# nikisalli/nightmare_rl

Measured on AMD Instinct MI355X. Metric: env-steps/sec at N parallel Nightmare-v3 envs, 1/2/4/8 MI355X, higher is better.
Workload: dtype f32; 1 GPU; 4096 Nightmare-v3 envs per GPU, random-action rollout U(-1,1)^18, full step(): 2 x 8 ms substeps (18-DoF dynamics + floor contact, PGS x3 + noslip x4) + obs/reward/termination/reset; envs_per_gpu=4096, decimation=2

## Files before the change

nightmare_rl_amd/csrc/nm_core.h:

```cpp
#pragma once
#include <type_traits>
#include <stddef.h>

#include "simt.h"

#ifdef NM_MEASURE
#define NM_ABLATE(mask) (mask)
#else
#define NM_ABLATE(mask) 0
#endif
namespace nm {
using namespace simt;

constexpr int kNQ = 25, kNV = 24, kNU = 18, kNLEG = 6, kNCOL = 7, kNSENS = 13, kNOBS = 66, kNREW = 16;
constexpr int kLinkN = 25;
constexpr int kLegN = 3 * kLinkN;
constexpr int kBaseN = 10;
constexpr int kColN = 24;
constexpr int kMaxCon = 16;
constexpr int kMaxRow = 4 * kMaxCon;
constexpr int kMaxConBig = 44;
constexpr int kBigSlots = (4 * kMaxConBig + NM_WAVE - 1) / NM_WAVE;
constexpr int kJRow = 16;
enum { R_ACTION_RATE, R_ANG_VEL_XY, R_BASE_HEIGHT, R_BODY_CONTACT, R_DEFAULT_POS, R_DOF_ACC, R_DOF_VEL, R_FEET_AIR_TIME, R_FEET_CONTACT,
       R_LIN_VEL_Z, R_ORIENTATION, R_STAND_STILL, R_TORQUES, R_TRACK_ANG, R_TRACK_LIN, R_TERMINATION };

template <class real> struct Model {
  const real* hullv;
  const real* hullnv;
  real legc[kNLEG * kLegN];
  real basec[kBaseN];
  real colc[kNCOL * kColN];
  real footc[kNLEG * 4];
  real qpos0[kNQ];
  int maxnbr;
  int link_rot_id[3];
  real total_mass;
  real h, kv, ctrl_max, grav, mu;
  real solref_K, solref_B, si_d0, si_dmax, si_width, si_mid, si_power;
  real pgs_scale, pgs_tol, noslip_tol, tol_planemesh;
  int pgs_iters, noslip_iters, mpr_iters;
  real mpr_tol;
  real dt, p_gain, clip_obs, obs_lin, obs_ang, obs_dofpos, obs_dofvel, max_lin_x, max_ang, term_force, sigma, max_ep_len, default_pos[3];
  float action_scale, clip_actions;
  int resample_every;
  real rew_scale[kNREW];
  real ep_len_s;
  int rew_extra;
  int tibia_mode, body_mode;
  int collide_batch_min;
  real tibia_max, body_max, base_h_target, max_contact_force;
};

template <class real> struct Args {
  int N;
  uint64_t seed;
  int64_t env_offset;
  real *qpos, *qvel, *qwarm;
  real *dofpos, *dofvel, *act, *cmd, *epsum;
  real* feetair;
  int* feetflags;
  int64_t* eplen;
  uint32_t* rngctr;
  int* hullcache;
  const float* actions;
  const real* cmd_u;
  float *obs, *rew, *timeout_now;
  float* ret_acc;
  int64_t* done;
  real* stat_sum;
  int* stat_cnt;
  int* wave_done;
  int *nto, *to_list;
  int *nprev, *to_prev;
  unsigned long long* to_owner;
  float *ep_stats, *time_outs;
  long long* counters;
  real* dbg;
  int nsub;
  int nxcd;
  int physics_only;
  int ablate;
  const real* noise_vec;
  const real* noise_u;
  uint64_t noise_step;
  real* rec;
  int rec_env;
};
constexpr int kTicketGroup = 64, kTicketStride = 32, kTicketTop = 0;
constexpr uint64_t kNoiseKey = 0x4E4F495345ull;
constexpr int kDbgN = 256;

template <class real> struct Sh {
  real qpos[28], qvel[24], warm[24], ctrl[20];
  real Rb[9], wv[6];
  real anc[kNU * 3], axs[kNU * 3];
  real colR[kNCOL * 9], colp[kNCOL * 3];
  real Minv[kNLEG * 6], W[kNLEG * 18], Lb[15], Dbi[6];
  real MinvH[kNLEG * 6], WH[kNLEG * 18], LbH[15], DbiH[6];
  real qas[24], qfs[24], qfc[24];
  real vv[24];
  real sens[16], cvb[6];
  real bh[2];
  real mbb[36], sc[36];
  real legtmp[kNLEG * 66];
  NM_FN real* cpos() { return legtmp; }
  NM_FN real* cnrm() { return legtmp + 3 * kMaxConBig; }
  NM_FN real* cdist() { return legtmp + 6 * kMaxConBig; }
  NM_FN int* cleg() { return reinterpret_cast<int*>(legtmp + 7 * kMaxConBig); }
  NM_FN int* cleg1() { return reinterpret_cast<int*>(legtmp + 8 * kMaxConBig); }
  real efc_f[kMaxRow];
#ifdef NM_DEBUG_SOLVER
  real dbg_b[kMaxRow], dbg_a[kMaxRow], dbg_f0[kMaxRow];
#endif
  int ncon, nwarn, it_pgs, it_noslip, anypair;
  int nhop;
  int ntog;
  real eact[kNU], epact[kNU], epdv[kNU];
  real ecmd[4], eepsum[kNREW];
  int eplen_lo, eplen_hi;
  unsigned ectr;
  int cstart[8], ccnt[8];
  real sink[NM_WAVE];
  int hcache[8];
};

static_assert(kNLEG * 66 >= 9 * kMaxConBig, "contact list must fit the leg staging area");
template <class real, int G> struct ShW {
  Sh<real> e[G];
  alignas(16) real jrow[kMaxRow * kJRow];
};
#define NM_OFS(field) ((int)(offsetof(Sh<real>, field) / sizeof(real)))
#define NM_IOFS(field) ((int)(offsetof(Sh<real>, field) / sizeof(int)))

template <class A, class B, class C> NM_FN void cross3(A* r, const B* a, const C* b) {
  A x = a[1] * b[2] - a[2] * b[1], y = a[2] * b[0] - a[0] * b[2], z = a[0] * b[1] - a[1] * b[0];
  r[0] = x; r[1] = y; r[2] = z;
}
template <class A, class B, class C> NM_FN A dot3(const B* a, const C* b) { return a[0] * b[0] + a[1] * b[1] + a[2] * b[2]; }
template <class A, class B, class C> NM_FN void matvec3(A* r, const B* m, const C* v) {
  A x = m[0] * v[0] + m[1] * v[1] + m[2] * v[2], y = m[3] * v[0] + m[4] * v[1] + m[5] * v[2], z = m[6] * v[0] + m[7] * v[1] + m[8] * v[2];
  r[0] = x; r[1] = y; r[2] = z;
}
template <class A, class B, class C> NM_FN void matvec3_fma(A* r, const B* m, const C* v) {
  A x = vfma(A(m[2]), A(v[2]), vfma(A(m[1]), A(v[1]), A(m[0]) * A(v[0])));
  A y = vfma(A(m[5]), A(v[2]), vfma(A(m[4]), A(v[1]), A(m[3]) * A(v[0])));
  A z = vfma(A(m[8]), A(v[2]), vfma(A(m[7]), A(v[1]), A(m[6]) * A(v[0])));
  r[0] = x; r[1] = y; r[2] = z;
}
template <class A, class B, class C> NM_FN void matmul3(A* r, const B* a, const C* b) {
#pragma unroll
  for (int i = 0; i < 3; i++)
#pragma unroll
    for (int j = 0; j < 3; j++) r[3 * i + j] = a[3 * i] * b[j] + a[3 * i + 1] * b[3 + j] + a[3 * i + 2] * b[6 + j];
}
template <class A, class B, class C> NM_FN void inert_mul(A* r, const B* i, const C* v) {
  r[0] = i[0] * v[0] + i[3] * v[1] + i[4] * v[2] - i[8] * v[4] + i[7] * v[5];
  r[1] = i[3] * v[0] + i[1] * v[1] + i[5] * v[2] + i[8] * v[3] - i[6] * v[5];
  r[2] = i[4] * v[0] + i[5] * v[1] + i[2] * v[2] - i[7] * v[3] + i[6] * v[4];
  r[3] = i[8] * v[1] - i[7] * v[2] + i[9] * v[3];
  r[4] = i[6] * v[2] - i[8] * v[0] + i[9] * v[4];
  r[5] = i[7] * v[0] - i[6] * v[1] + i[9] * v[5];
}
template <class A, class B, class C> NM_FN void cross_motion(A* r, const B* vel, const C* v) {
  A a[3], b[3], c[3];
  cross3(a, vel, v); cross3(b, vel, v + 3); cross3(c, vel + 3, v);
  r[0] = a[0]; r[1] = a[1]; r[2] = a[2]; r[3] = b[0] + c[0]; r[4] = b[1] + c[1]; r[5] = b[2] + c[2];
}
template <class A, class B, class C> NM_FN void cross_force(A* r, const B* vel, const C* f) {
  A a[3], b[3], c[3];
  cross3(a, vel, f); cross3(b, vel + 3, f + 3); cross3(c, vel, f + 3);
  r[0] = a[0] + b[0]; r[1] = a[1] + b[1]; r[2] = a[2] + b[2]; r[3] = c[0]; r[4] = c[1]; r[5] = c[2];
}
template <class A, class B, class C> NM_FN A dot6(const B* a, const C* b) {
  return a[0] * b[0] + a[1] * b[1] + a[2] * b[2] + a[3] * b[3] + a[4] * b[4] + a[5] * b[5];
}
template <class real> NM_FN real lanesum6(const V<real>& x) {
  return ((rdlane(x, 0) + rdlane(x, 1)) + (rdlane(x, 2) + rdlane(x, 3))) + (rdlane(x, 4) + rdlane(x, 5));
}
template <class X, class real> NM_FN void spatial_inertia(X* I10, const X* R, const X* Ib, const X* d, X m, real) {
  X T[9];
#pragma unroll
  for (int i = 0; i < 3; i++) {
    T[3 * i + 0] = R[3 * i] * Ib[0] + R[3 * i + 1] * Ib[3] + R[3 * i + 2] * Ib[4];
    T[3 * i + 1] = R[3 * i] * Ib[3] + R[3 * i + 1] * Ib[1] + R[3 * i + 2] * Ib[5];
    T[3 * i + 2] = R[3 * i] * Ib[4] + R[3 * i + 1] * Ib[5] + R[3 * i + 2] * Ib[2];
  }
  X xx = T[0] * R[0] + T[1] * R[1] + T[2] * R[2], yy = T[3] * R[3] + T[4] * R[4] + T[5] * R[5], zz = T[6] * R[6] + T[7] * R[7] + T[8] * R[8];
  X xy = T[0] * R[3] + T[1] * R[4] + T[2] * R[5], xz = T[0] * R[6] + T[1] * R[7] + T[2] * R[8], yz = T[3] * R[6] + T[4] * R[7] + T[5] * R[8];
  I10[0] = xx + m * (d[1] * d[1] + d[2] * d[2]);
  I10[1] = yy + m * (d[0] * d[0] + d[2] * d[2]);
  I10[2] = zz + m * (d[0] * d[0] + d[1] * d[1]);
  I10[3] = xy - m * d[0] * d[1];
  I10[4] = xz - m * d[0] * d[2];
  I10[5] = yz - m * d[1] * d[2];
  I10[6] = m * d[0]; I10[7] = m * d[1]; I10[8] = m * d[2];
  I10[9] = m;
}
template <class X, class real> NM_FN void ldl3(X* r, const X* a, real one) {
  X i2 = vrcp(a[5]);
  X l21 = a[4] * i2, l20 = a[2] * i2;
  X m11 = a[3] - l21 * a[4], m01 = a[1] - l21 * a[2], m00 = a[0] - l20 * a[2];
  X i1 = vrcp(m11);
  X l10 = m01 * i1;
  X d0 = m00 - l10 * m01;
  r[0] = l21; r[1] = l20; r[2] = l10; r[3] = i2; r[4] = i1; r[5] = vrcp(d0);
}
template <class X, class Y> NM_FN void ldl3_solve(X* x, const X* f, const Y* y) {
  X y2 = y[2];
  X y1 = y[1] - f[0] * y2;
  X y0 = y[0] - f[1] * y2 - f[2] * y1;
  X x0 = y0 * f[5];
  X x1 = y1 * f[4] - f[2] * x0;
  x[2] = y2 * f[3] - f[0] * x1 - f[1] * x0;
  x[1] = x1; x[0] = x0;
}
template <class X, class real, class Acc> NM_FN void ldl6(Acc S, X* L, X* Dinv, real one) {
  X Lf[36], D[6];
#pragma unroll
  for (int j = 0; j < 6; j++) {
    X d = S(j, j);
#pragma unroll
    for (int k = 0; k < j; k++) d = d - Lf[6 * j + k] * Lf[6 * j + k] * D[k];
    D[j] = d;
    X di = vrcp(d);
    Dinv[j] = di;
#pragma unroll
    for (int i = j + 1; i < 6; i++) {
      X s = S(j, i);
#pragma unroll
      for (int k = 0; k < j; k++) s = s - Lf[6 * i + k] * Lf[6 * j + k] * D[k];
      Lf[6 * i + j] = s * di;
    }
  }
  int n = 0;
#pragma unroll
  for (int i = 1; i < 6; i++)
#pragma unroll
    for (int j = 0; j < i; j++) L[n++] = Lf[6 * i + j];
}
template <class LT, class X> NM_FN void ldl6_solve(const LT* L, const LT* Dinv, X* x) {
  int n = 0;
#pragma unroll
  for (int i = 1; i < 6; i++)
#pragma unroll
    for (int j = 0; j < i; j++) x[i] = x[i] - L[n++] * x[j];
#pragma unroll
  for (int i = 0; i < 6; i++) x[i] = x[i] * Dinv[i];
#pragma unroll
  for (int i = 5; i >= 1; i--) {
    n = i * (i - 1) / 2;
#pragma unroll
    for (int j = 0; j < i; j++) x[j] = x[j] - L[n + j] * x[i];
  }
}

NM_FN uint32_t rand_u24_bits(uint64_t seed, uint64_t genv, uint32_t ctr) {
  uint64_t x = seed + 0x9E3779B97F4A7C15ull * (genv + 1) + 0xD1B54A32D192ED03ull * (uint64_t)ctr;
  x ^= x >> 30; x *= 0xBF58476D1CE4E5B9ull;
  x ^= x >> 27; x *= 0x94D049BB133111EBull;
  x ^= x >> 31;
  return (uint32_t)(x >> 40);
}

#ifndef NM_EMUL
template <class T> NM_FN void nm_consume(T x) { asm volatile("" ::"v"(x) : "memory"); }
#endif

#if defined(NM_STAMPS) && !defined(NM_EMUL)
__device__ unsigned long long g_stamps[16];
NM_FN void nm_stamp(int k) {
  __shared__ unsigned long long tl, acc[16];
#ifdef NM_STAMPS_B
  asm volatile("s_waitcnt vmcnt(0) lgkmcnt(0)" ::: "memory");
#endif
  unsigned long long n = __builtin_amdgcn_s_memtime();
  if (NM_TID == 0) {
    if (k < 0) for (int i = 0; i < 16; i++) acc[i] = 0;
    else acc[k] += n - tl;
    if (k == 10) for (int i = 0; i < 16; i++) atomicAdd(&g_stamps[i], acc[i]);
    tl = n;
  }
}
#else
NM_FN void nm_stamp(int) {}
#endif
#ifdef NM_STAMPS_B
#define NM_ESTAMP(k)
#define NM_BSTAMP(k) nm_stamp(k)
#else
#define NM_ESTAMP(k) nm_stamp(k)
#define NM_BSTAMP(k)
#endif

constexpr int kLinkTmp = 22;

template <class real> NM_FN V<real> legsum(const V<real>& x, const VB& isleg) {
  return gsum8(sel(isleg, x, V<real>(real(0))));
}

template <class real, int G> NM_FN void stage_smooth(ShW<real, G>& w, const Model<real>& M, bool last) {
  typedef V<real> vr;
  real* lds = reinterpret_cast<real*>(&w.e[0]);
  static_assert((G & (G - 1)) == 0 && 2 * G <= 8, "lane groups: G envs x 2 factorisations");
  const V<int> lane0 = opaque_lane();
  const V<int> sub = lane0 & 7, grp = lane0 >> 3;
  const V<int> leg = vmin(sub, V<int>(5)), eo = (grp & (G - 1)) * (int)(sizeof(Sh<real>) / sizeof(real));
  const VB pass1 = (grp & G) != 0;
  const VB isleg = sub < V<int>(6);
#define LDG(field, i) ldsv(lds, eo + (NM_OFS(field) + (i)))
  const VB st_all = VB(true), st_leg = VB(true);
#define STG(field, i, val) stsv(lds, eo + (NM_OFS(field) + (i)), val, st_all)
#define LDL(field, idx) ldsv(lds, eo + (idx) + NM_OFS(field))
#define STL(field, idx, val) stsv(lds, eo + (idx) + NM_OFS(field), val, st_leg)
  const V<int> slot = leg * (3 * kLinkTmp);

  vr Rb[9];
  {
    vr qw = LDG(qpos, 3), qx = LDG(qpos, 4), qy = LDG(qpos, 5), qz = LDG(qpos, 6);
    {
      const vr in_ = vrcp(vsqrt(qw * qw + qx * qx + qy * qy + qz * qz));
      qw = qw * in_; qx = qx * in_; qy = qy * in_; qz = qz * in_;
      STG(qpos, 3, qw); STG(qpos, 4, qx); STG(qpos, 5, qy); STG(qpos, 6, qz);
    }
    vr q00 = qw * qw, q01 = qw * qx, q02 = qw * qy, q03 = qw * qz, q11 = qx * qx, q12 = qx * qy, q13 = qx * qz, q22 = qy * qy,
       q23 = qy * qz, q33 = qz * qz;
    Rb[0] = q00 + q11 - q22 - q33; Rb[4] = q00 - q11 + q22 - q33; Rb[8] = q00 - q11 - q22 + q33;
    Rb[1] = real(2) * (q12 - q03); Rb[2] = real(2) * (q13 + q02); Rb[3] = real(2) * (q12 + q03);
    Rb[5] = real(2) * (q23 - q01); Rb[6] = real(2) * (q13 - q02); Rb[7] = real(2) * (q23 + q01);
  }
  vr vb[6], ab[6];
  {
    vr wl[3] = {LDG(qvel, 3), LDG(qvel, 4), LDG(qvel, 5)};
    matvec3(vb, Rb, wl);
    vb[3] = LDG(qvel, 0); vb[4] = LDG(qvel, 1); vb[5] = LDG(qvel, 2);
    vr t[3];
    cross3(t, vb + 3, vb);
    ab[0] = ab[1] = ab[2] = vr(real(0));
    ab[3] = t[0]; ab[4] = t[1]; ab[5] = t[2] + M.grav;
  }
#pragma unroll
  for (int j = 0; j < 9; j++) { STG(colR, j, Rb[j]); STG(Rb, j, Rb[j]); }
#pragma unroll
  for (int j = 0; j < 3; j++) STG(colp, j, vr(real(0)));
#pragma unroll
  for (int j = 0; j < 6; j++) STG(wv, j, vb[j]);

  const V<int> mylink = (grp >> (G == 1 ? 0 : (G == 2 ? 1 : 2))) & 3;
  const VB isbase = mylink == 3;
#ifndef NM_NO_ROLE_ROT
  {
    const V<int> lk = vmin(mylink, V<int>(2));
    const V<int> cbr = leg * kLegN + lk * kLinkN;
    const vr ax[3] = {ldsv(M.legc, cbr + 12), ldsv(M.legc, cbr + 13), ldsv(M.legc, cbr + 14)};
    vr s_, co;
    vsincos(LDL(qpos, leg * 3 + lk + 7), &s_, &co);
    const vr oc = vr(real(1)) - co;
    vr Rl[9];
    Rl[0] = co + oc * ax[0] * ax[0]; Rl[1] = oc * ax[0] * ax[1] - s_ * ax[2]; Rl[2] = oc * ax[0] * ax[2] + s_ * ax[1];
    Rl[3] = oc * ax[0] * ax[1] + s_ * ax[2]; Rl[4] = co + oc * ax[1] * ax[1]; Rl[5] = oc * ax[1] * ax[2] - s_ * ax[0];
    Rl[6] = oc * ax[0] * ax[2] - s_ * ax[1]; Rl[7] = oc * ax[1] * ax[2] + s_ * ax[0]; Rl[8] = co + oc * ax[2] * ax[2];
#pragma unroll
    for (int j = 0; j < 9; j++) STL(legtmp, leg * 27 + lk * 9 + j, Rl[j]);
    wave_sync();
  }
#endif
  vr mcom[3] = {vr(real(0)), vr(real(0)), vr(real(0))};
// ... 1888 lines not shown
        noslip_pair_prepare<real>(r.f[k], shfl_xor1(r.f[k]), r.small[k], lo, hi);
        const vr dg = g - shfl_xor1(g);
        vr d = noslip_pair_delta(dg, r.invK1[k], lo, hi);
        const vr change = noslip_pair_cost(d, r.hK1[k], dg);
        const VB bad = noslip_pair_bad<real>(change);
        d = sel(bad, vr(real(0)), d);
        const real d0 = rdlane(d, 2 * pp), d1 = rdlane(d, 2 * pp + 1);
        improvement -= rdlane(sel(bad, vr(real(0)), change), 2 * pp);
        r.f[k] = sel((lane >> 1) == pp, r.f[k] + d, r.f[k]);
        real jb[6], jl[3], jm[3];
#pragma unroll
        for (int j = 0; j < 6; j++) jb[j] = rdlane(r.Jb[k][j], 2 * pp) * d0 + rdlane(r.Jb[k][j], 2 * pp + 1) * d1;
#pragma unroll
        for (int j = 0; j < 3; j++) {
          jl[j] = rdlane(r.Jl[k][j], 2 * pp) * d0 + rdlane(r.Jl[k][j], 2 * pp + 1) * d1;
          jm[j] = rdlane(r.Jm[k][j], 2 * pp) * d0 + rdlane(r.Jm[k][j], 2 * pp + 1) * d1;
        }
        big_update_v(sh, jb, jl, jm, rdlane(r.L[k], 2 * pp), rdlane(r.L1[k], 2 * pp));
      }
    }
    sh.it_noslip = iter + 1;
    if (improvement * M.pgs_scale < M.noslip_tol) break;
  }
  big_jtf(sh, r);
  stsv(sh.efc_f, lane, r.f[0], lane < kMaxRow);
  if (last) {
    vr s_all[kNLEG], s_foot[kNLEG], s_base = vr(real(0));
#pragma unroll
    for (int l = 0; l < kNLEG; l++) { s_all[l] = vr(real(0)); s_foot[l] = vr(real(0)); }
#pragma unroll
    for (int k = 0; k < kBigSlots; k++) {
      const V<int> row = lane + NM_WAVE * k;
      const V<int> c = sel(r.act[k], row >> 2, V<int>(0));
      vr cp[3] = {ldsv(sh.cpos(), c * 3), ldsv(sh.cpos(), c * 3 + 1), ldsv(sh.cpos(), c * 3 + 2)};
      vr nrm[3] = {ldsv(sh.cnrm(), c * 3), ldsv(sh.cnrm(), c * 3 + 1), ldsv(sh.cnrm(), c * 3 + 2)};
      vr nf = r.f[k] + shfl_xor1(r.f[k]);
      nf = nf + shfl_xor2(nf);
      auto foot_hit = [&](const V<int>& Lx, real sgn) {
        vr ft[3], fr, sp[3], Rt[9];
#pragma unroll
        for (int j = 0; j < 3; j++) sp[j] = ldsv(M.footc, Lx * 4 + j);
        fr = ldsv(M.footc, Lx * 4 + 3);
#pragma unroll
        for (int j = 0; j < 9; j++) Rt[j] = ldsv(sh.colR, (Lx + 1) * 9 + j);
        matvec3(ft, Rt, sp);
#pragma unroll
        for (int j = 0; j < 3; j++) ft[j] = ft[j] + ldsv(sh.colp, (Lx + 1) * 3 + j);
        vr dif[3] = {cp[0] - ft[0], cp[1] - ft[1], cp[2] - ft[2]};
        vr b2 = sgn * (nrm[0] * dif[0] + nrm[1] * dif[1] + nrm[2] * dif[2]);
        vr cc = dif[0] * dif[0] + dif[1] * dif[1] + dif[2] * dif[2] - fr * fr;
        vr det = b2 * b2 - cc;
        vr sq = vsqrt(vmax(det, vr(real(0))));
        return !(det < vr(real(1e-15))) & (((-b2 - sq) >= vr(real(0))) | ((-b2 + sq) >= vr(real(0))));
      };
      const VB hit = foot_hit(vmax(r.L[k], V<int>(0)), real(-1)), hit1 = foot_hit(vmax(r.L1[k], V<int>(0)), real(1));
      const VB head = r.act[k] & ((lane & 3) == 0) & (nf > vr(real(0)));
#pragma unroll
      for (int l = 0; l < kNLEG; l++) {
        s_all[l] += sel(head & ((r.L[k] == l) | (r.L1[k] == l)), nf, vr(real(0)));
        s_foot[l] += sel(head & (((r.L[k] == l) & hit) | ((r.L1[k] == l) & hit1)), nf, vr(real(0)));
      }
      s_base += sel(head & (r.L[k] < 0), nf, vr(real(0)));
    }
#pragma unroll
    for (int l = 0; l < kNLEG; l++) { sh.sens[l] = wsum<real>(s_all[l]); sh.sens[6 + l] = wsum<real>(s_foot[l]); }
    sh.sens[12] = wsum<real>(s_base);
  }
  wave_sync();
}
template <class real> NM_COLD void floor_frames(Sh<real>& sh) {
  const V<int> lane = lane_id();
  const int nfloor = uniform(sh.cstart[7]);
  const VB on = lane < nfloor;
  const V<int> c = sel(on, lane, V<int>(0));
  stsv(sh.cleg1(), c, V<int>(-1), on);
  stsv(sh.cnrm(), c * 3, V<real>(real(0)), on);
  stsv(sh.cnrm(), c * 3 + 1, V<real>(real(0)), on);
  stsv(sh.cnrm(), c * 3 + 2, V<real>(real(1)), on);
  wave_sync();
}
template <class real> NM_FN void stage_constraint(Sh<real>& sh, real* jrow, const Model<real>& M, bool last, bool nosweep = false) {
  if (uniform(sh.ncon) > kMaxCon) { floor_frames(sh); stage_constraint_big<real>(sh, M, last, nosweep); }
  else if (uniform(sh.anypair) != 0) { floor_frames(sh); stage_constraint_pairs<real>(sh, jrow, M, last, nosweep); }
  else stage_constraint_body<real, false>(sh, jrow, M, last, nosweep);
}

template <class real, int G> NM_FN void stage_integrate(ShW<real, G>& w, const Model<real>& M) {
  typedef V<real> vr;
  real* lds = reinterpret_cast<real*>(&w.e[0]);
  const V<int> lane0 = opaque_lane();
  const V<int> sub = lane0 & 7, grp = lane0 >> 3;
  const V<int> leg = vmin(sub, V<int>(5)), eo = (grp & (G - 1)) * (int)(sizeof(Sh<real>) / sizeof(real));
  const VB pass1 = (grp & G) != 0;
  const VB isleg = sub < V<int>(6);
#define LDG(field, i) ldsv(lds, eo + (NM_OFS(field) + (i)))
#define LDL(field, idx) ldsv(lds, eo + (idx) + NM_OFS(field))
  constexpr int kFacH = NM_OFS(MinvH) - NM_OFS(Minv);
  static_assert(NM_OFS(WH) - NM_OFS(W) == kFacH && NM_OFS(LbH) - NM_OFS(Lb) == kFacH && NM_OFS(DbiH) - NM_OFS(Dbi) == kFacH, "factor blocks");
  static_assert(sizeof(Sh<real>::mbb) / sizeof(real) >= 24 && sizeof(Sh<real>::sc) / sizeof(real) >= 28 && sizeof(Sh<real>::vv) / sizeof(real) >= 24, "junk rows");
  const V<int> eoF = eo + sel(pass1, V<int>(kFacH), V<int>(0));
  vr xl[3], xb[6];
  {
    vr y[3], t[3], Mi[6];
#pragma unroll
    for (int k = 0; k < 3; k++) y[k] = LDL(qfc, leg * 3 + (6 + k)) + sel(pass1, LDL(qfs, leg * 3 + (6 + k)), vr(real(0)));
#pragma unroll
    for (int j = 0; j < 6; j++) Mi[j] = ldsv(lds, eoF + leg * 6 + (NM_OFS(Minv) + j));
    ldl3_solve(t, Mi, y);
#pragma unroll
    for (int j = 0; j < 6; j++) {
      vr wy = ldsv(lds, eoF + leg * 18 + (NM_OFS(W) + j)) * y[0] + ldsv(lds, eoF + leg * 18 + (NM_OFS(W) + 6 + j)) * y[1] +
              ldsv(lds, eoF + leg * 18 + (NM_OFS(W) + 12 + j)) * y[2];
      xb[j] = LDG(qfc, j) - legsum<real>(wy, isleg) + sel(pass1, LDG(qfs, j), vr(real(0)));
    }
    {
      vr L[15], Di[6];
#pragma unroll
      for (int j = 0; j < 15; j++) L[j] = ldsv(lds, eoF + (NM_OFS(Lb) + j));
#pragma unroll
      for (int j = 0; j < 6; j++) Di[j] = ldsv(lds, eoF + (NM_OFS(Dbi) + j));
      ldl6_solve(L, Di, xb);
    }
#pragma unroll
    for (int k = 0; k < 3; k++) {
      vr x = t[k];
#pragma unroll
      for (int j = 0; j < 6; j++) x = x - ldsv(lds, eoF + leg * 18 + (NM_OFS(W) + 6 * k + j)) * xb[j];
      xl[k] = x;
    }
  }
  vr qacc_l[3], qacc_b[6];
#pragma unroll
  for (int k = 0; k < 3; k++) qacc_l[k] = xl[k] + LDL(qas, leg * 3 + (6 + k));
#pragma unroll
  for (int j = 0; j < 6; j++) qacc_b[j] = xb[j] + LDG(qas, j);
  const vr* qint_l = xl; const vr* qint_b = xb;
  VB badl = (visbad(qacc_l[0]) | visbad(qacc_l[1]) | visbad(qacc_l[2])) & isleg;
#pragma unroll
  for (int j = 0; j < 6; j++) badl = badl | visbad(qacc_b[j]);
  const VB gbad = gsum8(sel(badl, V<int>(1), V<int>(0))) > 0;
  const VB okl = VB(true), okb = VB(true);
  wave_sync();
  vr nv[6];
#pragma unroll
  for (int j = 0; j < 6; j++) nv[j] = LDG(qvel, j) + M.h * qint_b[j];
  vr np_[3], nq[4];
#pragma unroll
  for (int j = 0; j < 3; j++) np_[j] = LDG(qpos, j) + M.h * nv[j];
  {
    vr n = vsqrt(nv[3] * nv[3] + nv[4] * nv[4] + nv[5] * nv[5]);
    VB rot = !(n < vr(real(1e-15)));
    vr ns = sel(rot, n, vr(real(1)));
    vr ang = M.h * n, sn, cs;
    vsincos(real(0.5) * ang, &sn, &cs);
    rot = rot & (ang != vr(real(0)));
    const vr isn = vrcp(ns) * sn;
    vr qr[4] = {sel(rot, cs, vr(real(1))), sel(rot, nv[3] * isn, vr(real(0))), sel(rot, nv[4] * isn, vr(real(0))),
                sel(rot, nv[5] * isn, vr(real(0)))};
    vr a[4] = {LDG(qpos, 3), LDG(qpos, 4), LDG(qpos, 5), LDG(qpos, 6)};
    vr t[4] = {a[0] * qr[0] - a[1] * qr[1] - a[2] * qr[2] - a[3] * qr[3], a[0] * qr[1] + a[1] * qr[0] + a[2] * qr[3] - a[3] * qr[2],
               a[0] * qr[2] - a[1] * qr[3] + a[2] * qr[0] + a[3] * qr[1], a[0] * qr[3] + a[1] * qr[2] - a[2] * qr[1] + a[3] * qr[0]};
    vr nn = vsqrt(t[0] * t[0] + t[1] * t[1] + t[2] * t[2] + t[3] * t[3]);
#pragma unroll
    for (int j = 0; j < 4; j++) nq[j] = t[j] * vrcp(nn);
  }
  vr jq[3], jv[3];
#pragma unroll
  for (int k = 0; k < 3; k++) {
    jv[k] = LDL(qvel, leg * 3 + (6 + k)) + M.h * qint_l[k];
    jq[k] = LDL(qpos, leg * 3 + (7 + k)) + M.h * jv[k];
  }
  wave_sync();
  const V<int> eoV = eo + sel(pass1, V<int>(NM_OFS(qvel)), V<int>(NM_OFS(mbb)));
  const V<int> eoP = eo + sel(pass1, V<int>(NM_OFS(qpos)), V<int>(NM_OFS(sc)));
  const V<int> eoW = eo + sel(pass1, V<int>(NM_OFS(vv)), V<int>(NM_OFS(warm)));
#pragma unroll
  for (int j = 0; j < 6; j++) {
    stsv(lds, eoV + j, nv[j], okb);
    stsv(lds, eoW + j, qacc_b[j], okb);
  }
#pragma unroll
  for (int j = 0; j < 3; j++) stsv(lds, eoP + j, np_[j], okb);
#pragma unroll
  for (int j = 0; j < 4; j++) stsv(lds, eoP + (3 + j), nq[j], okb);
#pragma unroll
  for (int k = 0; k < 3; k++) {
    stsv(lds, eoV + leg * 3 + (6 + k), jv[k], okl);
    stsv(lds, eoP + leg * 3 + (7 + k), jq[k], okl);
    stsv(lds, eoW + leg * 3 + (6 + k), qacc_l[k], okl);
  }
  wave_sync();
  for (int e = 0; e < G; e++) {
    if (rdlane(sel(gbad, V<int>(1), V<int>(0)), 8 * e) != 0) {
      Sh<real>& sh = w.e[e];
      const V<int> lane = opaque_lane();
      sh.nwarn += 1;
      vr q0 = ldsv(M.qpos0, sel(lane < kNQ, lane, V<int>(0)));
      real vz = -M.grav * M.h;
      q0 = sel(lane == 2, q0 + vz * M.h, q0);
      stsv(sh.qpos, lane, q0, lane < kNQ);
      stsv(sh.qvel, lane, sel(lane == 2, vr(vz), vr(real(0))), lane < kNV);
      stsv(sh.warm, lane, sel(lane == 2, vr(-M.grav), vr(real(0))), lane < kNV);
      stsv(sh.ctrl, lane, real(0), lane < kNU);
      wave_sync();
    }
  }
#undef LDG
#undef LDL
}

template <class real> NM_FN void reset_data(Sh<real>& sh, const Model<real>& M) {
  const V<int> lane = opaque_lane();
  stsv(sh.qpos, lane, ldsv(M.qpos0, sel(lane < kNQ, lane, V<int>(0))), lane < kNQ);
  stsv(sh.qvel, lane, real(0), lane < kNV);
  stsv(sh.warm, lane, real(0), lane < kNV);
  stsv(sh.ctrl, lane, real(0), lane < kNU);
  wave_sync();
}

#ifndef NM_PRIO
#define NM_PRIO 3
#endif
#if !defined(NM_EMUL)
NM_FN void nm_set_priority(int load) {
  if (load >= NM_PRIO + 4) __builtin_amdgcn_s_setprio(3);
  else if (load >= NM_PRIO + 2) __builtin_amdgcn_s_setprio(2);
  else if (load >= NM_PRIO) __builtin_amdgcn_s_setprio(1);
  else __builtin_amdgcn_s_setprio(0);
}
#else
inline void nm_set_priority(int) {}
#endif

template <class real, int G> NM_FN void substep(ShW<real, G>& w, const Model<real>& M, bool last, int* dropped, int ablate) {
  const V<int> lane = opaque_lane();
  if constexpr (G == 2) {
    constexpr int kSR = (int)(sizeof(Sh<real>) / sizeof(real));
    real* rbw = reinterpret_cast<real*>(&w.e[0]);
    const V<int> hl = lane & 31, ho = (lane >> 5) * kSR;
    {
      const VB bad = (visbad(ldsv(rbw, ho + (sel(hl < kNQ, hl, V<int>(0)) + NM_OFS(qpos)))) & (hl < kNQ)) |
                     (visbad(ldsv(rbw, ho + (sel(hl < kNV, hl, V<int>(0)) + NM_OFS(qvel)))) & (hl < kNV));
      const uint64_t bm = ballot(bad);
      if (bm) {
#pragma unroll
        for (int e = 0; e < 2; e++)
          if ((bm >> (32 * e)) & 0xffffffffull) { w.e[e].nwarn += 1; reset_data(w.e[e], M); }
      }
    }
  } else {
    for (int e = 0; e < G; e++) {
      Sh<real>& sh = w.e[e];
      {
        VB bad = (visbad(ldsv(sh.qpos, sel(lane < kNQ, lane, V<int>(0)))) & (lane < kNQ)) |
                 (visbad(ldsv(sh.qvel, sel(lane < kNV, lane, V<int>(0)))) & (lane < kNV));
        if (wany(bad)) { sh.nwarn += 1; reset_data(sh, M); }
      }
    }
  }
  wave_sync();
  nm_stamp(1);
  if (!(ablate & 8)) stage_smooth(w, M, last);
  nm_stamp(2);
  for (int e = 0; e < G; e++) {
    Sh<real>& sh = w.e[e];
    if (!(ablate & 1)) { Rings<real> rg; collide_rings(sh, M, rg); stage_collide(sh, M, dropped, rg, G != 2 && !(ablate & 16)); }
    else { sh.ncon = 0; sh.anypair = 0; wave_sync(); }
  }
  if constexpr (G == 2) {
    if (!(ablate & 1) && !(ablate & 16)) stage_collide_pairs2(w, M, dropped);
  }
  for (int e = 0; e < G; e++)
    if (ablate & 4) { w.e[e].ncon = 0; w.e[e].anypair = 0; wave_sync(); }
  bool together = false;
  if constexpr (G == 2) {
    const int n0 = uniform(w.e[0].ncon), n1 = uniform(w.e[1].ncon);
    nm_set_priority(n0 + n1);
    together = n0 + n1 >= 1 && n0 <= kMaxCon2 && n1 <= kMaxCon2 && uniform(w.e[0].anypair) == 0 && uniform(w.e[1].anypair) == 0 && !(ablate & 32);
    if (!last) w.e[1].ntog = n0 * 64 + n1;
    if (together) {
#ifdef NM_EMUL
      nm_emul_together() += 1;
#endif
      w.e[0].ntog += 1;
      stage_constraint2(w, M, last, (ablate & 2) != 0);
      nm_stamp(8);
    }
  }
  if (!together)
    for (int e = 0; e < G; e++) {
      stage_constraint(w.e[e], w.jrow, M, last, (ablate & 2) != 0);
      nm_stamp(8);
    }
  stage_integrate(w, M);
  nm_stamp(9);
}


template <class real> NM_FN void env_load(Sh<real>& sh, const Model<real>& M, const Args<real>& A, int env) {
  typedef V<real> vr;
  const V<int> lane = opaque_lane();
  const VB l18 = lane < kNU;
  const V<int> l18c = sel(l18, lane, V<int>(0));
  const vr q_in = gldv(A.qpos, sel(lane < kNQ, lane, V<int>(0)) + env * kNQ);
  const vr v_in = gldv(A.qvel, sel(lane < kNV, lane, V<int>(0)) + env * kNV);
  const vr w_in = gldv(A.qwarm, sel(lane < kNV, lane, V<int>(0)) + env * kNV);
  const V<int> hc_in = gldv(A.hullcache, sel(lane < 8, lane, V<int>(0)) + env * 8);
  const V<float> a_in = gldv(A.actions, l18c + env * kNU);
  vr cmd_in = vr(real(0)), eps_in = vr(real(0)), prev_act = vr(real(0)), prev_dofvel = vr(real(0)), dofpos_old = vr(real(0));
  int64_t ep = 0;
  uint32_t ctr_in = 0;
  if (!A.physics_only) {
    cmd_in = gldv(A.cmd, sel(lane < 3, lane, V<int>(0)) + env * 3);
    eps_in = gldv(A.epsum, sel(lane < kNREW, lane, V<int>(0)) + env * kNREW);
    ep = gld1(A.eplen, env);
    ctr_in = gld1(A.rngctr, env);
    prev_act = gldv(A.act, l18c + env * kNU);
    prev_dofvel = gldv(A.dofvel, l18c + env * kNU);
    dofpos_old = gldv(A.dofpos, l18c + env * kNU);
  }
  stsv(sh.qpos, lane, q_in, lane < kNQ);
  stsv(sh.qvel, lane, v_in, lane < kNV);
  stsv(sh.warm, lane, w_in, lane < kNV);
  stsv(sh.hcache, lane, sel(lane == 0, hc_in & V<int>(0xffff), hc_in), lane < 8);
  sh.nwarn = 0;
  sh.nhop = 0;
  sh.ntog = 0;
  V<float> af = a_in * M.action_scale;
  af = vmin(vmax(af, V<float>(-M.clip_actions)), V<float>(M.clip_actions));
  vr act;
  vr defp;
  {
    V<int> m3 = lane % 3;
    defp = sel(m3 == 1, vr(M.default_pos[1]), sel(m3 == 0, vr(M.default_pos[0]), vr(M.default_pos[2])));
  }
#ifdef NM_EMUL
  for (int i = 0; i < NM_WAVE; i++) act.v[i] = (real)af.v[i];
#else
  act = (real)af;
#endif
  if (!A.physics_only) {
    stsv(sh.ecmd, lane, cmd_in, lane < 3);
    stsv(sh.eepsum, lane, eps_in, lane < kNREW);
    sh.eplen_lo = (int)(uint32_t)(ep & 0xffffffffll);
    sh.eplen_hi = (int)(ep >> 32);
    sh.ectr = ctr_in;
    stsv(sh.ctrl, lane, ((act - defp) - dofpos_old) * M.p_gain, l18);
  } else {
    wave_sync();
    stsv(sh.ctrl, lane, ((act - defp) - ldsv(sh.qpos, l18c + 7)) * M.p_gain, l18);
  }
  stsv(sh.eact, lane, act, l18); stsv(sh.epact, lane, prev_act, l18); stsv(sh.epdv, lane, prev_dofvel, l18);
  wave_sync();
}

template <class real> NM_FN void env_debug(Sh<real>& sh, const Args<real>& A, int env, int dropped) {
  const V<int> lane = opaque_lane();
  {
    real* dbg = A.dbg + (size_t)env * kDbgN;
    gstv(dbg, lane, ldsv(sh.qas, sel(lane < 24, lane, V<int>(0))), lane < 24);
    gstv(dbg, lane + 24, ldsv(sh.qfs, sel(lane < 24, lane, V<int>(0))), lane < 24);
    gstv(dbg, lane + 48, ldsv(sh.qfc, sel(lane < 24, lane, V<int>(0))), lane < 24);
    gstv(dbg, lane + 72, ldsv(sh.sens, sel(lane < 13, lane, V<int>(0))), lane < 13);
    gstv(dbg, lane + 88, ldsv(sh.cvb, sel(lane < 6, lane, V<int>(0))), lane < 6);
    gstv(dbg, lane + 96, ldsv(sh.cdist(), sel(lane < kMaxCon, lane, V<int>(0))), lane < kMaxCon);
    gstv(dbg, lane + 112, ldsv(sh.cpos(), sel(lane < 3 * kMaxCon, lane, V<int>(0))), lane < 3 * kMaxCon);
    gstv(dbg, V<int>(160), to_real<real>(sh.ncon), lane == 0);
    gstv(dbg, V<int>(161), to_real<real>(sh.nwarn), lane == 0);
    gstv(dbg, V<int>(162), to_real<real>(dropped), lane == 0);
    gstv(dbg, lane + 165, ldsv(sh.cnrm(), sel(lane < 6, lane, V<int>(0))), lane < 6);
    gstv(dbg, lane + 150, to_real<real>(ldsv(sh.hcache, sel(lane < 7, lane, V<int>(0)))), lane < 7);
    gstv(dbg, V<int>(158), to_real<real>(sh.hcache[7]), lane == 0);
    gstv(dbg, V<int>(159), to_real<real>(sh.nhop), lane == 0);
    gstv(dbg, V<int>(157), to_real<real>(sh.anypair), lane == 0);
    gstv(dbg, V<int>(156), to_real<real>(sh.ntog), lane == 0);
    gstv(dbg, V<int>(163), to_real<real>(sh.it_pgs), lane == 0);
    gstv(dbg, V<int>(164), to_real<real>(sh.it_noslip), lane == 0);
    gstv(dbg, lane + 176, ldsv(sh.efc_f, lane), lane < kMaxRow);
#ifdef NM_DEBUG_SOLVER
    gstv(dbg, lane + 240, ldsv(sh.dbg_b, sel(lane < 4, lane, V<int>(0))), lane < 4);
    gstv(dbg, lane + 244, ldsv(sh.dbg_a, sel(lane < 4, lane, V<int>(0))), lane < 4);
    gstv(dbg, lane + 248, ldsv(sh.dbg_f0, sel(lane < 4, lane, V<int>(0))), lane < 4);
#endif
  }
}

template <class real> NM_FN void env_finish(Sh<real>& sh, const Model<real>& M, const Args<real>& A, int env,
                                            int dropped, bool live) {
  typedef V<real> vr;
  if (!live) return;
  const V<int> lane = opaque_lane();
  const VB l18 = lane < kNU;
  const V<int> l18c = sel(l18, lane, V<int>(0));
  const vr act = ldsv(sh.eact, l18c), prev_act = ldsv(sh.epact, l18c), prev_dofvel = ldsv(sh.epdv, l18c);
  vr defp;
  {
    V<int> m3 = lane % 3;
    defp = sel(m3 == 1, vr(M.default_pos[1]), sel(m3 == 0, vr(M.default_pos[0]), vr(M.default_pos[2])));
  }
  {
    const V<int> hc = ldsv(sh.hcache, sel(lane < 8, lane, V<int>(0)));
    const vr q = ldsv(sh.qpos, sel(lane < kNQ, lane, V<int>(0))), v = ldsv(sh.qvel, sel(lane < kNV, lane, V<int>(0))),
             w = ldsv(sh.warm, sel(lane < kNV, lane, V<int>(0)));
    gstv(A.hullcache, lane + env * 8, hc, lane < 8);
    gstv(A.qpos, lane + env * kNQ, q, lane < kNQ);
    gstv(A.qvel, lane + env * kNV, v, lane < kNV);
    gstv(A.qwarm, lane + env * kNV, w, lane < kNV);
  }
  if (A.rec && env == A.rec_env) {
    gstv(A.rec, lane, ldsv(sh.qpos, sel(lane < kNQ, lane, V<int>(0))), lane < kNQ);
    gstv(A.rec, lane + kNQ, ldsv(sh.qvel, sel(lane < kNV, lane, V<int>(0))), lane < kNV);
    gstv(A.rec, V<int>(kNQ + kNV), to_real<real>(sh.nwarn), lane == 0);
  }
  if (A.dbg) env_debug(sh, A, env, dropped);
  if ((dropped | sh.nwarn) && A.stat_cnt) {
#ifdef NM_EMUL
    A.stat_cnt[1] += dropped; A.stat_cnt[2] += sh.nwarn;
#else
    if (NM_TID == 0) { nm_consume(atomicAdd(A.stat_cnt + 1, dropped)); nm_consume(atomicAdd(A.stat_cnt + 2, sh.nwarn)); }
#endif
  }
  if (A.physics_only) return;
  NM_ESTAMP(11);

  int64_t eplen = (((int64_t)sh.eplen_hi << 32) | (int64_t)(uint32_t)sh.eplen_lo) + 1;
  real bq[4] = {sh.qpos[3], -sh.qpos[4], -sh.qpos[5], -sh.qpos[6]};
  auto rot = [&](real* r, const real* v) {
    real tx = real(2) * (bq[2] * v[2] - bq[3] * v[1]), ty = real(2) * (bq[3] * v[0] - bq[1] * v[2]), tz = real(2) * (bq[1] * v[1] - bq[2] * v[0]);
    r[0] = v[0] + bq[0] * tx + (bq[2] * tz - bq[3] * ty);
    r[1] = v[1] + bq[0] * ty + (bq[3] * tx - bq[1] * tz);
    r[2] = v[2] + bq[0] * tz + (bq[1] * ty - bq[2] * tx);
  };
  real blv[3], bav[3], pg[3];
  {
    real lin[3] = {sh.cvb[3], sh.cvb[4], sh.cvb[5]}, ang[3] = {sh.cvb[0], sh.cvb[1], sh.cvb[2]}, gv[3] = {real(0), real(0), -M.grav};
    rot(blv, lin); rot(bav, ang); rot(pg, gv);
  }
  vr dofpos = ldsv(sh.qpos, l18c + 7), dofvel = ldsv(sh.qvel, l18c + 6);
  real tib[6], feet[6], body = sh.sens[12];
#pragma unroll
  for (int l = 0; l < 6; l++) {
    feet[l] = sh.sens[6 + l];
    tib[l] = feet[l] == real(0) ? sh.sens[l] : real(0);
  }
  real cmd[3] = {sh.ecmd[0], sh.ecmd[1], sh.ecmd[2]};
  uint32_t ctr = sh.ectr;
  auto resample = [&](int which) {
    real ux, uy;
    if (A.cmd_u) { ux = gld1(A.cmd_u, env * 4 + 2 * which); uy = gld1(A.cmd_u, env * 4 + 2 * which + 1); }
    else {
      ux = (real)rand_u24_bits(A.seed, (uint64_t)(A.env_offset + env), ctr) * real(1.0 / 16777216.0);
      uy = (real)rand_u24_bits(A.seed, (uint64_t)(A.env_offset + env), ctr + 1) * real(1.0 / 16777216.0);
      ctr += 2;
    }
    cmd[0] = ux * real(2) * M.max_lin_x - M.max_lin_x;
    cmd[1] = real(0);
    cmd[2] = uy * real(2) * M.max_ang - M.max_ang;
    real keep = vsqrt(cmd[0] * cmd[0] + cmd[1] * cmd[1]) > real(0.02) ? real(1) : real(0);
    cmd[0] = cmd[0] * keep; cmd[1] = cmd[1] * keep;
  };
  {
    bool due;
    if (eplen >= 0 && eplen < (1 << 22)) {
      const int e32 = (int)eplen, R = M.resample_every;
      const int q = (int)((float)e32 / (float)R);
      const int r = e32 - q * R;
      due = r == 0 || r == R || r == -R;
    } else due = eplen % M.resample_every == 0;
    if (due) resample(0);
  }
  bool time_out = (real)eplen > M.max_ep_len;
  bool reset = time_out;
  {
    real fm = feet[0];
#pragma unroll
    for (int l = 1; l < 6; l++) fm = vmax(fm, feet[l]);
    reset = reset | (fm > M.term_force);
    if ((M.tibia_mode == 2) | (M.body_mode == 2)) {
      real tm = tib[0];
#pragma unroll
      for (int l = 1; l < 6; l++) tm = vmax(tm, tib[l]);
      if (M.tibia_mode == 2) reset = reset | (tm > M.tibia_max);
      if (M.body_mode == 2) reset = reset | (body > M.body_max);
    }
    real nrm = vsqrt(pg[0] * pg[0] + pg[1] * pg[1] + pg[2] * pg[2]);
    if (sizeof(real) == 8) reset = reset | (vacos(-pg[2] / nrm) > real(1.0471975511965976));
    else reset = reset | (-pg[2] / nrm <= real(0.5));
  }
  NM_ESTAMP(12);
  vr epsum[1];
  V<int> l8c = sel(lane < kNREW, lane, V<int>(0));
  epsum[0] = ldsv(sh.eepsum, l8c);
  if (reset) {
    gstv(A.qpos, lane + env * kNQ, ldsv(M.qpos0, sel(lane < kNQ, lane, V<int>(0))), lane < kNQ);
    gstv(A.qvel, lane + env * kNV, real(0), lane < kNV);
    resample(1);
    eplen = 0;
#ifdef NM_EMUL
    for (int k = 0; k < kNREW; k++) A.stat_sum[k] += epsum[0].v[k];
    A.stat_cnt[0] += 1;
#else
    if (NM_TID < kNREW) nm_consume(atomicAdd(A.stat_sum + NM_TID, epsum[0]));
    if (NM_TID == 0) {
      nm_consume(atomicAdd(A.stat_cnt, 1));
      if (time_out && A.to_list) nm_consume(atomicExch(A.to_list + atomicAdd(A.nto, 1), env));
    }
#endif
    epsum[0] = vr(real(0));
  }
  NM_ESTAMP(13);
  real rt[kNREW];
#pragma unroll
  for (int k = 0; k < kNREW; k++) rt[k] = real(0);
  {
    vr da = prev_act - act;
    rt[R_ACTION_RATE] = wsum<real>(sel(l18, da * da, vr(real(0)))) * M.rew_scale[R_ACTION_RATE];
    real sumt = ((tib[0] + tib[1]) + (tib[2] + tib[3])) + (tib[4] + tib[5]);
    if ((M.tibia_mode != 1) | (M.body_mode != 1)) {
      sumt = M.tibia_mode == 1 ? sumt : real(0);
      body = M.body_mode == 1 ? body : real(0);
    }
    rt[R_BODY_CONTACT] = (sumt + body) * M.rew_scale[R_BODY_CONTACT];
    vr dp = dofpos - defp;
    rt[R_DEFAULT_POS] = wsum<real>(sel(l18, dp * dp, vr(real(0)))) * M.rew_scale[R_DEFAULT_POS];
    vr acc = (dofvel - prev_dofvel) / M.dt;
    rt[R_DOF_ACC] = wsum<real>(sel(l18, acc * acc, vr(real(0)))) * M.rew_scale[R_DOF_ACC];
    rt[R_ORIENTATION] = (pg[0] * pg[0] + pg[1] * pg[1]) * M.rew_scale[R_ORIENTATION];
    real ea = (cmd[2] - bav[2]) * (cmd[2] - bav[2]);
    rt[R_TRACK_ANG] = vexp(-ea / M.sigma) * M.rew_scale[R_TRACK_ANG];
    real el = (cmd[0] - blv[0]) * (cmd[0] - blv[0]) + (cmd[1] - blv[1]) * (cmd[1] - blv[1]);
    rt[R_TRACK_LIN] = vexp(-el / M.sigma) * M.rew_scale[R_TRACK_LIN];
    rt[R_TERMINATION] = (reset && !time_out) ? M.rew_scale[R_TERMINATION] : real(0);
    if (M.rew_extra) {
      rt[R_ANG_VEL_XY] = (bav[0] * bav[0] + bav[1] * bav[1]) * M.rew_scale[R_ANG_VEL_XY];
      real dh = sh.bh[0] - M.base_h_target;
      rt[R_BASE_HEIGHT] = dh * dh * M.rew_scale[R_BASE_HEIGHT];
      rt[R_DOF_VEL] = wsum<real>(sel(l18, dofvel * dofvel, vr(real(0)))) * M.rew_scale[R_DOF_VEL];
      rt[R_LIN_VEL_Z] = blv[2] * blv[2] * M.rew_scale[R_LIN_VEL_Z];
      real still = vsqrt(cmd[0] * cmd[0] + cmd[1] * cmd[1]) < real(0.01) ? real(1) : real(0);
      rt[R_STAND_STILL] = wsum<real>(sel(l18, vabs(dp), vr(real(0)))) * still * M.rew_scale[R_STAND_STILL];
      const VB l6 = lane < kNLEG;
      const V<int> l6c = sel(l6, lane, V<int>(0));
      const vr ff = ldsv(sh.sens, l6c + 6);
      vr over = sel(ff > vr(M.max_contact_force), ff - M.max_contact_force, vr(real(0)));
      rt[R_FEET_CONTACT] = wsum<real>(sel(l6, over * over, vr(real(0)))) * M.rew_scale[R_FEET_CONTACT];
      if (M.rew_scale[R_FEET_AIR_TIME] != real(0)) {
        vr air = gldv(A.feetair, l6c + env * kNLEG);
        const V<int> fl = V<int>(gld1(A.feetflags, env));
        if (reset) air = vr(real(0));
        const VB contact = ff > vr(real(1));
        const VB filt = contact | (((fl >> l6c) & 1) != 0);
        const VB lastf = ((fl >> (l6c + kNLEG)) & 1) != 0;
        air = air + M.dt;
        air = sel(filt == lastf, air, vr(real(0)));
        const vr single = sel(air > vr(real(1)), air - real(1), vr(real(0))) + sel(air < vr(real(0.5)), real(0.5) - air, vr(real(0)));
        rt[R_FEET_AIR_TIME] = wsum<real>(sel(l6, single * single, vr(real(0)))) * M.rew_scale[R_FEET_AIR_TIME];
        gstv(A.feetair, l6c + env * kNLEG, air, l6);
        const int nf = (int)(ballot(l6 & contact) | (ballot(l6 & filt) << kNLEG));
#ifdef NM_EMUL
        A.feetflags[env] = nf;
#else
        if (NM_TID == 0) gst1(A.feetflags, env, nf);
#endif
      }
    }
  }
  real rew = real(0);
#pragma unroll
  for (int k = 0; k < kNREW; k++) rew = rew + rt[k];
  {
    vr add = vr(real(0));
#pragma unroll
    for (int k = 0; k < kNREW; k++) add = wrlane(add, rt[k], k);
    gstv(A.epsum, lane + env * kNREW, epsum[0] + add, lane < kNREW);
  }
  NM_ESTAMP(14);
  {
    real head[12] = {blv[0] * M.obs_lin, blv[1] * M.obs_lin, blv[2] * M.obs_lin, bav[0] * M.obs_ang, bav[1] * M.obs_ang, bav[2] * M.obs_ang,
                     pg[0], pg[1], pg[2], cmd[0] * M.obs_lin, cmd[1] * M.obs_lin, cmd[2] * M.obs_ang};
    vr o = vr(real(0));
#pragma unroll
    for (int k = 0; k < 12; k++) o = wrlane(o, head[k], k);
    auto put = [&](const vr& x0, const V<int>& idx, const VB& m) {
      vr x = x0;
      if (A.noise_vec) {
        auto nz = [&](int k) {
          real u = A.noise_u ? gld1(A.noise_u, (size_t)env * kNOBS + k)
                             : (real)rand_u24_bits(A.seed + kNoiseKey, (uint64_t)(A.env_offset + env), (uint32_t)(A.noise_step * kNOBS + k)) * real(1.0 / 16777216.0);
          return (real(2) * u - real(1)) * gld1(A.noise_vec, k);
        };
#ifdef NM_EMUL
        for (int i = 0; i < NM_WAVE; i++) if (m.v[i]) x.v[i] = x.v[i] + nz(idx.v[i]);
#else
        if (m) x = x + nz(idx);
#endif
      }
      vr cx = vmin(vmax(x, vr(-M.clip_obs)), vr(M.clip_obs));
#ifdef NM_EMUL
      for (int i = 0; i < NM_WAVE; i++) if (m.v[i]) A.obs[(size_t)env * kNOBS + idx.v[i]] = (float)cx.v[i];
#else
      if (m) gst1(A.obs, (size_t)env * kNOBS + idx, (float)cx);
#endif
    };
    put(o, lane, lane < 12);
    put((dofpos - defp) * M.obs_dofpos, lane + 12, l18);
    put(dofvel * M.obs_dofvel, lane + 30, l18);
    put(act, lane + 48, l18);
  }
  NM_ESTAMP(15);
  gstv(A.dofpos, lane + env * kNU, dofpos, l18);
  gstv(A.dofvel, lane + env * kNU, dofvel, l18);
  gstv(A.act, lane + env * kNU, act, l18);
  {
    vr cv = sel(lane == 0, vr(cmd[0]), sel(lane == 1, vr(cmd[1]), vr(cmd[2])));
    gstv(A.cmd, lane + env * 3, cv, lane < 3);
  }
#ifdef NM_EMUL
  const bool lane0 = true;
#else
  const bool lane0 = NM_TID == 0;
#endif
  if (lane0) {
    gst1(A.eplen, env, eplen);
    gst1(A.rngctr, env, ctr);
    gst1(A.rew, env, (float)rew);
    if (A.ret_acc) gadd1(A.ret_acc, env, (float)rew);
    gst1(A.done, env, (int64_t)(reset ? 1 : 0));
    gst1(A.timeout_now, env, time_out ? 1.0f : 0.0f);
  }
}

struct NoMid { NM_FN void operator()() const {} NM_FN void operator()(int) const {} };
template <class real, class Mid> NM_FN void env_load2(ShW<real, 2>& w, const Model<real>& M, const Args<real>& A, int wave, Mid&& mid) {
  typedef V<real> vr;
  constexpr int kSR = (int)(sizeof(Sh<real>) / sizeof(real)), kSI = (int)(sizeof(Sh<real>) / sizeof(int));
  const V<int> lane = opaque_lane();
  const V<int> h = lane >> 5, hl = lane & 31;
  const V<int> env0 = h + wave * 2;
  const V<int> env = sel(env0 < V<int>(A.N), env0, V<int>(A.N - 1));
  real* rb = reinterpret_cast<real*>(&w.e[0]);
  int* ib = reinterpret_cast<int*>(&w.e[0]);
  const V<int> ho = h * kSR, hoi = h * kSI;
  const VB l18 = hl < kNU;
  const V<int> l18c = sel(l18, hl, V<int>(0));
  const vr q_in = gldv(A.qpos, sel(hl < kNQ, hl, V<int>(0)) + env * kNQ);
  const vr v_in = gldv(A.qvel, sel(hl < kNV, hl, V<int>(0)) + env * kNV);
  const vr w_in = gldv(A.qwarm, sel(hl < kNV, hl, V<int>(0)) + env * kNV);
  const V<int> hc_in = gldv(A.hullcache, sel(hl < 8, hl, V<int>(0)) + env * 8);
  const V<float> a_in = gldv(A.actions, l18c + env * kNU);
  vr cmd_in = vr(real(0)), eps_in = vr(real(0)), prev_act = vr(real(0)), prev_dofvel = vr(real(0)), dofpos_old = vr(real(0));
#ifndef NM_EMUL
  int64_t ep = 0;
  uint32_t ctr_in = 0;
#endif
  if (!A.physics_only) {
    cmd_in = gldv(A.cmd, sel(hl < 3, hl, V<int>(0)) + env * 3);
    eps_in = gldv(A.epsum, sel(hl < kNREW, hl, V<int>(0)) + env * kNREW);
#ifndef NM_EMUL
    ep = gld1(A.eplen, (size_t)env);
    ctr_in = gld1(A.rngctr, (size_t)env);
#endif
    prev_act = gldv(A.act, l18c + env * kNU);
    prev_dofvel = gldv(A.dofvel, l18c + env * kNU);
    dofpos_old = gldv(A.dofpos, l18c + env * kNU);
  }
  mid();
  stsv(rb, ho + (hl + NM_OFS(qpos)), q_in, hl < kNQ);
  stsv(rb, ho + (hl + NM_OFS(qvel)), v_in, hl < kNV);
  stsv(rb, ho + (hl + NM_OFS(warm)), w_in, hl < kNV);
  stsv(ib, hoi + (hl + NM_IOFS(hcache)), sel(hl == 0, hc_in & V<int>(0xffff), hc_in), hl < 8);
  nm_set_priority((rdlane(hc_in, 0) >> 16) + (rdlane(hc_in, 32) >> 16));
  w.e[0].nwarn = 0; w.e[1].nwarn = 0;
  w.e[0].nhop = 0; w.e[1].nhop = 0;
  w.e[0].ntog = 0; w.e[1].ntog = 0;
  V<float> af = a_in * M.action_scale;
  af = vmin(vmax(af, V<float>(-M.clip_actions)), V<float>(M.clip_actions));
  vr act;
  vr defp;
  {
    V<int> m3 = hl % 3;
    defp = sel(m3 == 1, vr(M.default_pos[1]), sel(m3 == 0, vr(M.default_pos[0]), vr(M.default_pos[2])));
  }
#ifdef NM_EMUL
  for (int i = 0; i < NM_WAVE; i++) act.v[i] = (real)af.v[i];
#else
  act = (real)af;
#endif
  if (!A.physics_only) {
    stsv(rb, ho + (hl + NM_OFS(ecmd)), cmd_in, hl < 3);
    stsv(rb, ho + (hl + NM_OFS(eepsum)), eps_in, hl < kNREW);
#ifdef NM_EMUL
    for (int hh = 0; hh < 2; hh++) {
      const int e = env.v[32 * hh];
      const int64_t ep = A.eplen[e];
      w.e[hh].eplen_lo = (int)(uint32_t)(ep & 0xffffffffll);
      w.e[hh].eplen_hi = (int)(ep >> 32);
      w.e[hh].ectr = A.rngctr[e];
    }
#else
    stsv(ib, hoi + NM_IOFS(eplen_lo), (int)(uint32_t)(ep & 0xffffffffll), hl == 0);
    stsv(ib, hoi + NM_IOFS(eplen_hi), (int)(ep >> 32), hl == 0);
    stsv(ib, hoi + NM_IOFS(ectr), (int)ctr_in, hl == 0);
#endif
    stsv(rb, ho + (hl + NM_OFS(ctrl)), ((act - defp) - dofpos_old) * M.p_gain, l18);
  } else {
    wave_sync();
    stsv(rb, ho + (hl + NM_OFS(ctrl)), ((act - defp) - ldsv(rb, ho + (l18c + (7 + NM_OFS(qpos))))) * M.p_gain, l18);
  }
  stsv(rb, ho + (hl + NM_OFS(eact)), act, l18); stsv(rb, ho + (hl + NM_OFS(epact)), prev_act, l18); stsv(rb, ho + (hl + NM_OFS(epdv)), prev_dofvel, l18);
  wave_sync();
}

template <class real, class Pub> NM_FN void env_finish2(ShW<real, 2>& w, const Model<real>& M, const Args<real>& A, int wave, int dropped, Pub&& published) {
  typedef V<real> vr;
  constexpr int kSR = (int)(sizeof(Sh<real>) / sizeof(real)), kSI = (int)(sizeof(Sh<real>) / sizeof(int));
  const V<int> lane = opaque_lane();
  const V<int> h = lane >> 5, hl = lane & 31;
  const VB h1 = h != 0;
  const V<int> env = h + wave * 2;
  const VB live = env < V<int>(A.N);
  const V<int> envc = sel(live, env, V<int>(A.N - 1));
  const bool lives[2] = {wave * 2 < A.N, wave * 2 + 1 < A.N};
  const real* rb = reinterpret_cast<const real*>(&w.e[0]);
  const int* ib = reinterpret_cast<const int*>(&w.e[0]);
  const V<int> ho = h * kSR, hoi = h * kSI;
#define SHR(field, idx) ldsv(rb, ho + ((idx) + NM_OFS(field)))
#define SHI(field, idx) ldsv(ib, hoi + ((idx) + NM_IOFS(field)))
  const VB l18 = hl < kNU;
  const V<int> l18c = sel(l18, hl, V<int>(0));
  const vr act = SHR(eact, l18c), prev_act = SHR(epact, l18c), prev_dofvel = SHR(epdv, l18c);
  vr defp;
  {
    V<int> m3 = hl % 3;
    defp = sel(m3 == 1, vr(M.default_pos[1]), sel(m3 == 0, vr(M.default_pos[0]), vr(M.default_pos[2])));
  }
  const V<int> nwarn = SHI(nwarn, V<int>(0));
  {
    V<int> hc = SHI(hcache, sel(hl < 8, hl, V<int>(0)));
    hc = sel(hl == 0, hc | (SHI(ncon, V<int>(0)) << 16), hc);
    const vr q = SHR(qpos, sel(hl < kNQ, hl, V<int>(0))), v = SHR(qvel, sel(hl < kNV, hl, V<int>(0))), wq = SHR(warm, sel(hl < kNV, hl, V<int>(0)));
    gstv(A.hullcache, hl + env * 8, hc, live & (hl < 8));
    gstv(A.qpos, hl + env * kNQ, q, live & (hl < kNQ));
    gstv(A.qvel, hl + env * kNV, v, live & (hl < kNV));
    gstv(A.qwarm, hl + env * kNV, wq, live & (hl < kNV));
    if (A.rec) {
      const VB r = live & (env == V<int>(A.rec_env));
      gstv(A.rec, hl, q, r & (hl < kNQ));
      gstv(A.rec, hl + kNQ, v, r & (hl < kNV));
      gstv(A.rec, V<int>(kNQ + kNV), to_real<real>(nwarn), r & (hl == 0));
    }
  }
  if (A.dbg) {
    if (lives[0]) env_debug(w.e[0], A, wave * 2, dropped);
    if (lives[1]) env_debug(w.e[1], A, wave * 2 + 1, 0);
  }
  if (A.stat_cnt && (dropped != 0 || wany(live & (nwarn != 0)))) {
#ifdef NM_EMUL
    A.stat_cnt[1] += dropped;
    for (int hh = 0; hh < 2; hh++) if (lives[hh]) A.stat_cnt[2] += nwarn.v[32 * hh];
#else
    if (NM_TID == 0 && dropped) nm_consume(atomicAdd(A.stat_cnt + 1, dropped));
    if (hl == 0 && live && nwarn) nm_consume(atomicAdd(A.stat_cnt + 2, nwarn));
#endif
  }
  if (A.physics_only) return;
  if (NM_ABLATE(A.ablate) & 128) return;
  NM_ESTAMP(11);

  int64_t ep[2];
  uint32_t ctr[2];
#pragma unroll
  for (int hh = 0; hh < 2; hh++) {
    ep[hh] = (((int64_t)w.e[hh].eplen_hi << 32) | (int64_t)(uint32_t)w.e[hh].eplen_lo) + 1;
    ctr[hh] = w.e[hh].ectr;
  }
  vr bq[4] = {SHR(qpos, V<int>(3)), -SHR(qpos, V<int>(4)), -SHR(qpos, V<int>(5)), -SHR(qpos, V<int>(6))};
  auto rot = [&](vr* r, const vr* v) {
    vr tx = real(2) * (bq[2] * v[2] - bq[3] * v[1]), ty = real(2) * (bq[3] * v[0] - bq[1] * v[2]), tz = real(2) * (bq[1] * v[1] - bq[2] * v[0]);
    r[0] = v[0] + bq[0] * tx + (bq[2] * tz - bq[3] * ty);
    r[1] = v[1] + bq[0] * ty + (bq[3] * tx - bq[1] * tz);
    r[2] = v[2] + bq[0] * tz + (bq[1] * ty - bq[2] * tx);
  };
  vr blv[3], bav[3], pg[3];
  {
    vr lin[3] = {SHR(cvb, V<int>(3)), SHR(cvb, V<int>(4)), SHR(cvb, V<int>(5))}, ang[3] = {SHR(cvb, V<int>(0)), SHR(cvb, V<int>(1)), SHR(cvb, V<int>(2))};
    vr gv[3] = {vr(real(0)), vr(real(0)), vr(-M.grav)};
    rot(blv, lin); rot(bav, ang); rot(pg, gv);
  }
  vr dofpos = SHR(qpos, l18c + 7), dofvel = SHR(qvel, l18c + 6);
  vr tib[6], feet[6], body = SHR(sens, V<int>(12));
#pragma unroll
  for (int l = 0; l < 6; l++) {
    feet[l] = SHR(sens, V<int>(6 + l));
    tib[l] = sel(feet[l] == vr(real(0)), SHR(sens, V<int>(l)), vr(real(0)));
  }
  vr cmd[3] = {SHR(ecmd, V<int>(0)), SHR(ecmd, V<int>(1)), SHR(ecmd, V<int>(2))};
  auto resample = [&](int hh, int which) {
    const int e = wave * 2 + hh;
    real ux, uy;
    if (A.cmd_u) { ux = gld1(A.cmd_u, (size_t)(e * 4 + 2 * which)); uy = gld1(A.cmd_u, (size_t)(e * 4 + 2 * which + 1)); }
    else {
      ux = (real)rand_u24_bits(A.seed, (uint64_t)(A.env_offset + e), ctr[hh]) * real(1.0 / 16777216.0);
      uy = (real)rand_u24_bits(A.seed, (uint64_t)(A.env_offset + e), ctr[hh] + 1) * real(1.0 / 16777216.0);
      ctr[hh] += 2;
    }
    real c0 = ux * real(2) * M.max_lin_x - M.max_lin_x, c1 = real(0), c2 = uy * real(2) * M.max_ang - M.max_ang;
    real keep = vsqrt(c0 * c0 + c1 * c1) > real(0.02) ? real(1) : real(0);
    c0 = c0 * keep; c1 = c1 * keep;
    const VB mine = hh ? h1 : !h1;
    cmd[0] = sel(mine, vr(c0), cmd[0]); cmd[1] = sel(mine, vr(c1), cmd[1]); cmd[2] = sel(mine, vr(c2), cmd[2]);
  };
  bool tos[2];
#pragma unroll
  for (int hh = 0; hh < 2; hh++) {
    bool due;
    if (ep[hh] >= 0 && ep[hh] < (1 << 22)) {
      const int e32 = (int)ep[hh], R = M.resample_every;
      const int q = (int)((float)e32 / (float)R);
      const int r = e32 - q * R;
      due = r == 0 || r == R || r == -R;
    } else due = ep[hh] % M.resample_every == 0;
    if (due && lives[hh]) resample(hh, 0);
    tos[hh] = (real)ep[hh] > M.max_ep_len;
  }
  const VB time_out = (h1 & VB(tos[1])) | (!h1 & VB(tos[0]));
  VB reset = time_out;
  {
    vr fm = feet[0];
#pragma unroll
    for (int l = 1; l < 6; l++) fm = vmax(fm, feet[l]);
    reset = reset | (fm > vr(M.term_force));
    if ((M.tibia_mode == 2) | (M.body_mode == 2)) {
      vr tm = tib[0];
#pragma unroll
      for (int l = 1; l < 6; l++) tm = vmax(tm, tib[l]);
      if (M.tibia_mode == 2) reset = reset | (tm > vr(M.tibia_max));
      if (M.body_mode == 2) reset = reset | (body > vr(M.body_max));
    }
    vr nrm = vsqrt(pg[0] * pg[0] + pg[1] * pg[1] + pg[2] * pg[2]);
    if (sizeof(real) == 8) reset = reset | (vacos(-pg[2] / nrm) > vr(real(1.0471975511965976)));
    else reset = reset | ((-pg[2] / nrm) <= vr(real(0.5)));
  }
  NM_ESTAMP(12);
  vr epsum = SHR(eepsum, sel(hl < kNREW, hl, V<int>(0)));
  const VB resetL = reset & live;
  const uint64_t rmask = ballot(resetL);
  if (rmask) {
    gstv(A.qpos, hl + env * kNQ, ldsv(M.qpos0, sel(hl < kNQ, hl, V<int>(0))), resetL & (hl < kNQ));
    gstv(A.qvel, hl + env * kNV, real(0), resetL & (hl < kNV));
#pragma unroll
    for (int hh = 0; hh < 2; hh++)
      if ((rmask >> (32 * hh)) & 1) { resample(hh, 1); ep[hh] = 0; }
#ifdef NM_EMUL
    for (int hh = 0; hh < 2; hh++)
      if ((rmask >> (32 * hh)) & 1) {
        for (int k = 0; k < kNREW; k++) A.stat_sum[k] += epsum.v[32 * hh + k];
        A.stat_cnt[0] += 1;
      }
#else
    if (resetL && hl < kNREW) nm_consume(atomicAdd(A.stat_sum + hl, epsum));
    if (resetL && hl == 0) {
      nm_consume(atomicAdd(A.stat_cnt, 1));
      if (time_out && A.to_list) nm_consume(atomicExch(A.to_list + atomicAdd(A.nto, 1), env));
    }
#endif
    epsum = sel(resetL, vr(real(0)), epsum);
  }
  published(0);
  NM_ESTAMP(13);
  vr rt[kNREW];
#pragma unroll
  for (int k = 0; k < kNREW; k++) rt[k] = vr(real(0));
  {
    vr da = prev_act - act;
    rt[R_ACTION_RATE] = hsum32(sel(l18, da * da, vr(real(0)))) * M.rew_scale[R_ACTION_RATE];
    vr sumt = ((tib[0] + tib[1]) + (tib[2] + tib[3])) + (tib[4] + tib[5]);
    if ((M.tibia_mode != 1) | (M.body_mode != 1)) {
      sumt = M.tibia_mode == 1 ? sumt : vr(real(0));
      body = M.body_mode == 1 ? body : vr(real(0));
    }
    rt[R_BODY_CONTACT] = (sumt + body) * M.rew_scale[R_BODY_CONTACT];
    vr dp = dofpos - defp;
    rt[R_DEFAULT_POS] = hsum32(sel(l18, dp * dp, vr(real(0)))) * M.rew_scale[R_DEFAULT_POS];
    vr acc = (dofvel - prev_dofvel) / M.dt;
    rt[R_DOF_ACC] = hsum32(sel(l18, acc * acc, vr(real(0)))) * M.rew_scale[R_DOF_ACC];
    rt[R_ORIENTATION] = (pg[0] * pg[0] + pg[1] * pg[1]) * M.rew_scale[R_ORIENTATION];
    vr ea = (cmd[2] - bav[2]) * (cmd[2] - bav[2]);
    rt[R_TRACK_ANG] = vexp(-ea / M.sigma) * M.rew_scale[R_TRACK_ANG];
    vr el = (cmd[0] - blv[0]) * (cmd[0] - blv[0]) + (cmd[1] - blv[1]) * (cmd[1] - blv[1]);
    rt[R_TRACK_LIN] = vexp(-el / M.sigma) * M.rew_scale[R_TRACK_LIN];
    rt[R_TERMINATION] = sel(reset & !time_out, vr(M.rew_scale[R_TERMINATION]), vr(real(0)));
    if (M.rew_extra) {
      rt[R_ANG_VEL_XY] = (bav[0] * bav[0] + bav[1] * bav[1]) * M.rew_scale[R_ANG_VEL_XY];
      vr dh = SHR(bh, V<int>(0)) - M.base_h_target;
      rt[R_BASE_HEIGHT] = dh * dh * M.rew_scale[R_BASE_HEIGHT];
      rt[R_DOF_VEL] = hsum32(sel(l18, dofvel * dofvel, vr(real(0)))) * M.rew_scale[R_DOF_VEL];
      rt[R_LIN_VEL_Z] = blv[2] * blv[2] * M.rew_scale[R_LIN_VEL_Z];
      vr still = sel(vsqrt(cmd[0] * cmd[0] + cmd[1] * cmd[1]) < vr(real(0.01)), vr(real(1)), vr(real(0)));
      rt[R_STAND_STILL] = hsum32(sel(l18, vabs(dp), vr(real(0)))) * still * M.rew_scale[R_STAND_STILL];
      const VB l6 = hl < kNLEG;
      const V<int> l6c = sel(l6, hl, V<int>(0));
      const vr ff = SHR(sens, l6c + 6);
      vr over = sel(ff > vr(M.max_contact_force), ff - M.max_contact_force, vr(real(0)));
      rt[R_FEET_CONTACT] = hsum32(sel(l6, over * over, vr(real(0)))) * M.rew_scale[R_FEET_CONTACT];
      if (M.rew_scale[R_FEET_AIR_TIME] != real(0)) {
        vr air = gldv(A.feetair, l6c + envc * kNLEG);
        const V<int> fl = gldv(A.feetflags, envc);
        air = sel(reset, vr(real(0)), air);
        const VB contact = ff > vr(real(1));
        const VB filt = contact | (((fl >> l6c) & 1) != 0);
        const VB lastf = ((fl >> (l6c + kNLEG)) & 1) != 0;
        air = air + M.dt;
        air = sel(filt == lastf, air, vr(real(0)));
        const vr single = sel(air > vr(real(1)), air - real(1), vr(real(0))) + sel(air < vr(real(0.5)), real(0.5) - air, vr(real(0)));
        rt[R_FEET_AIR_TIME] = hsum32(sel(l6, single * single, vr(real(0)))) * M.rew_scale[R_FEET_AIR_TIME];
        gstv(A.feetair, l6c + env * kNLEG, air, live & l6);
        const uint64_t bc = ballot(l6 & contact), bf = ballot(l6 & filt);
        const int nf0 = (int)((bc & 63) | ((bf & 63) << kNLEG)), nf1 = (int)(((bc >> 32) & 63) | (((bf >> 32) & 63) << kNLEG));
        gstv(A.feetflags, env, sel(h1, V<int>(nf1), V<int>(nf0)), live & (hl == 0));
      }
    }
  }
  vr rew = vr(real(0));
#pragma unroll
  for (int k = 0; k < kNREW; k++) rew = rew + rt[k];
  {
    vr add = vr(real(0));
#pragma unroll
    for (int k = 0; k < kNREW; k++) add = sel(hl == k, rt[k], add);
    gstv(A.epsum, hl + env * kNREW, epsum + add, live & (hl < kNREW));
  }
  published(1);
  NM_ESTAMP(14);
  if (!(NM_ABLATE(A.ablate) & 256)) {
    vr head[12] = {blv[0] * M.obs_lin, blv[1] * M.obs_lin, blv[2] * M.obs_lin, bav[0] * M.obs_ang, bav[1] * M.obs_ang, bav[2] * M.obs_ang,
                   pg[0], pg[1], pg[2], cmd[0] * M.obs_lin, cmd[1] * M.obs_lin, cmd[2] * M.obs_ang};
    vr o = vr(real(0));
#pragma unroll
    for (int k = 0; k < 12; k++) o = sel(hl == k, head[k], o);
    auto put = [&](const vr& x0, const V<int>& idx, const VB& m0) {
      const VB m = m0 & live;
      vr x = x0;
      if (A.noise_vec) {
        auto nz = [&](int k, int e) {
          real u = A.noise_u ? gld1(A.noise_u, (size_t)e * kNOBS + k)
                             : (real)rand_u24_bits(A.seed + kNoiseKey, (uint64_t)(A.env_offset + e), (uint32_t)(A.noise_step * kNOBS + k)) * real(1.0 / 16777216.0);
          return (real(2) * u - real(1)) * gld1(A.noise_vec, (size_t)k);
        };
#ifdef NM_EMUL
        for (int i = 0; i < NM_WAVE; i++) if (m.v[i]) x.v[i] = x.v[i] + nz(idx.v[i], env.v[i]);
#else
        if (m) x = x + nz(idx, env);
#endif
      }
      vr cx = vmin(vmax(x, vr(-M.clip_obs)), vr(M.clip_obs));
#ifdef NM_EMUL
      for (int i = 0; i < NM_WAVE; i++) if (m.v[i]) A.obs[(size_t)env.v[i] * kNOBS + idx.v[i]] = (float)cx.v[i];
#else
      if (m) gst1(A.obs, (size_t)env * kNOBS + idx, (float)cx);
#endif
    };
    put(o, hl, hl < 12);
    put((dofpos - defp) * M.obs_dofpos, hl + 12, l18);
    put(dofvel * M.obs_dofvel, hl + 30, l18);
    put(act, hl + 48, l18);
  }
  NM_ESTAMP(15);
  gstv(A.dofpos, hl + env * kNU, dofpos, live & l18);
  gstv(A.dofvel, hl + env * kNU, dofvel, live & l18);
  gstv(A.act, hl + env * kNU, act, live & l18);
  {
    vr cv = sel(hl == 0, cmd[0], sel(hl == 1, cmd[1], cmd[2]));
    gstv(A.cmd, hl + env * 3, cv, live & (hl < 3));
  }
#ifdef NM_EMUL
  for (int hh = 0; hh < 2; hh++)
    if (lives[hh]) {
      const int e = wave * 2 + hh, l0 = 32 * hh;
      A.eplen[e] = ep[hh]; A.rngctr[e] = ctr[hh]; A.rew[e] = (float)rew.v[l0];
      if (A.ret_acc) A.ret_acc[e] += (float)rew.v[l0];
      A.done[e] = (int64_t)(reset.v[l0] ? 1 : 0); A.timeout_now[e] = time_out.v[l0] ? 1.0f : 0.0f;
    }
#else
  if (hl == 0 && live) {
    gst1(A.eplen, (size_t)env, h1 ? ep[1] : ep[0]);
    gst1(A.rngctr, (size_t)env, h1 ? ctr[1] : ctr[0]);
    gst1(A.rew, (size_t)env, (float)rew);
    if (A.ret_acc) gadd1(A.ret_acc, (size_t)env, (float)rew);
    gst1(A.done, (size_t)env, (int64_t)(reset ? 1 : 0));
    gst1(A.timeout_now, (size_t)env, time_out ? 1.0f : 0.0f);
  }
#endif
#undef SHR
#undef SHI
}

template <class real, int G, class Mid = NoMid, class Pub = NoMid>
NM_FN void wave_step(ShW<real, G>& w, const Model<real>& M, const Args<real>& A, int wave, Mid&& mid = Mid(), Pub&& published = Pub()) {
  nm_stamp(-1);
  if constexpr (G == 2) {
    env_load2(w, M, A, wave, mid);
  } else {
    mid();
#pragma unroll
    for (int e = 0; e < G; e++) {
      int env = wave * G + e;
      env_load(w.e[e], M, A, env < A.N ? env : A.N - 1);
    }
  }
  nm_stamp(0);
  int dropped = 0;
  if (NM_ABLATE(A.ablate) & 1024) return;
  if (!(NM_ABLATE(A.ablate) & 2048))
  for (int s = 0; s < A.nsub; s++) substep(w, M, s == A.nsub - 1, &dropped, NM_ABLATE(A.ablate));
  if constexpr (G == 2) {
    env_finish2(w, M, A, wave, dropped, published);
  } else {
#pragma unroll
    for (int e = 0; e < G; e++) {
      int env = wave * G + e;
      env_finish(w.e[e], M, A, env, e == 0 ? dropped : 0, env < A.N);
    }
  }
  nm_stamp(10);
}

}
```

nightmare_rl_amd/csrc/nm_hip.hip:

```cpp
#include <hip/hip_runtime.h>

#include <cstdio>
#include <cstdlib>
#include <cstring>
#include <string>
#include <vector>

#include "../../include/nightmare_hip.h"
#include "nm_host_model.h"
#include "nm_rollout.h"

static thread_local std::string g_err;
static int fail(const std::string& m) { g_err = m; return 1; }
#define HIPCHK(x)                                                                                        \
  do {                                                                                                   \
    hipError_t e_ = (x);                                                                                 \
    if (e_ != hipSuccess) return fail(std::string(#x) + ": " + hipGetErrorString(e_));                  \
  } while (0)

#ifndef NM_WAVES_PER_SIMD
#define NM_WAVES_PER_SIMD 2
#endif
#ifndef NM_ENVS_PER_WAVE
#define NM_ENVS_PER_WAVE 2
#endif
template <class real> __device__ __noinline__ void step_tail(const nm::Args<real>& A, real ep_len_s) {
  const int lane = NM_TID;
#define TAIL_LD(p) __hip_atomic_load(p, __ATOMIC_RELAXED, __HIP_MEMORY_SCOPE_AGENT)
  const int cnt = TAIL_LD(A.stat_cnt);
  const int c1 = TAIL_LD(A.stat_cnt + 1), c2 = TAIL_LD(A.stat_cnt + 2);
  const real ssum = TAIL_LD(A.stat_sum + (lane < nm::kNREW ? lane : 0));
  const int n = TAIL_LD(A.nto);
  const int np = TAIL_LD(A.nprev);
  const bool to_full = A.time_outs && TAIL_LD(A.to_owner) != (unsigned long long)(uintptr_t)A.time_outs;
  const long long k0 = lane == 0 ? A.counters[0] : 0, k1 = lane == 0 ? A.counters[1] : 0;
  if (cnt > 0) {
    if (lane < nm::kNREW && A.ep_stats) A.ep_stats[lane] = (float)(ssum / (real)cnt / ep_len_s);
    if (A.time_outs) {
      const int e_new = lane < n ? TAIL_LD(A.to_list + lane) : -1;
      const int e_old = (!to_full && lane < np) ? A.to_prev[lane] : -1;
      if (to_full) {
        for (int i = lane; i < A.N; i += 64) A.time_outs[i] = 0.f;
      } else {
        if (e_old >= 0) A.time_outs[e_old] = 0.f;
        for (int j = lane + 64; j < np; j += 64) A.time_outs[A.to_prev[j]] = 0.f;
      }
      asm volatile("s_waitcnt vmcnt(0)" ::: "memory");
      if (e_new >= 0) { A.time_outs[e_new] = 1.f; A.to_prev[lane] = e_new; }
      for (int j = lane + 64; j < n; j += 64) {
        const int e = TAIL_LD(A.to_list + j);
        A.time_outs[e] = 1.f;
        A.to_prev[j] = e;
      }
      if (lane == 0) { *A.nprev = n; *A.to_owner = (unsigned long long)(uintptr_t)A.time_outs; }
    }
  }
#undef TAIL_LD
  if (lane < nm::kNREW) A.stat_sum[lane] = real(0);
  if (lane == 0) {
    A.counters[0] = k0 + c1;
    A.counters[1] = k1 + c2;
    A.stat_cnt[0] = 0; A.stat_cnt[1] = 0; A.stat_cnt[2] = 0; A.stat_cnt[3] = 0;
    *A.nto = 0;
    A.wave_done[nm::kTicketTop] = 0;
  }
}

#ifdef NM_WG_WAVES
constexpr int kWG = NM_WG_WAVES;
#else
constexpr int kWG = 1;
#endif
template <class real, int G>
__global__ void __launch_bounds__(64 * (sizeof(real) == 8 ? 1 : kWG), NM_WAVES_PER_SIMD) k_env_step(const nm::Model<real>* __restrict__ Mp, nm::Args<real> A) {
  constexpr int kWG = sizeof(real) == 8 ? 1 : ::kWG;
  __shared__ nm::ShW<real, G> shs[kWG];
  __shared__ nm::Model<real> Ms;
  __shared__ nm::Args<real> As;
  nm::ShW<real, G>& sh = shs[kWG == 1 ? 0 : (int)(threadIdx.x >> 6)];
  int wave = blockIdx.x;
#ifndef NM_NO_XCD_MAP
  {
    const int nwx = (int)gridDim.x >> 3;
    if (A.nxcd == 8 && wave < (nwx << 3)) wave = (wave & 7) * nwx + (wave >> 3);
  }
#endif
  if (kWG > 1) wave = wave * kWG + (int)(threadIdx.x >> 6);
#ifdef NM_MEASURE
  if (A.ablate & 512) return;
#endif
  const unsigned long long t_start = A.dbg ? __builtin_amdgcn_s_memtime() : 0ull;
  if (kWG == 1 || threadIdx.x < 64) As = A;
  __syncthreads();
  if (wave * G >= A.N) return;
  auto copy_model = [&]() {
    const uint32_t* src = reinterpret_cast<const uint32_t*>(Mp);
    uint32_t* dst = reinterpret_cast<uint32_t*>(&Ms);
    constexpr int kWords = (int)(sizeof(nm::Model<real>) / 4);
    uint32_t tmp[(kWords + 63) / 64];
#pragma unroll
    for (int k = 0; k < (kWords + 63) / 64; k++) { const int i = NM_TID + 64 * k; tmp[k] = i < kWords ? src[i] : 0u; }
    if (kWG == 1 || threadIdx.x < 64) {
#pragma unroll
      for (int k = 0; k < (kWords + 63) / 64; k++) { const int i = NM_TID + 64 * k; if (i < kWords) dst[i] = tmp[k]; }
    }
    __syncthreads();
  };
  const int nw = (As.N + G - 1) / G, grp = wave / nm::kTicketGroup, ngrp = (nw + nm::kTicketGroup - 1) / nm::kTicketGroup;
  const int gsize = min(nm::kTicketGroup, nw - grp * nm::kTicketGroup);
  int ticket = 0, top = 0;
  int stage = 0;
  bool closes_group = false;
  auto draw = [&](int phase) {
#ifdef NM_NO_TICKETS
    stage = 2; (void)phase; return;
#endif
    if (phase == 0) {
      if (NM_TID == 0) ticket = atomicAdd(As.wave_done + (grp + 1) * nm::kTicketStride, 1);
      stage = 1;
    } else {
      closes_group = __builtin_amdgcn_readfirstlane(ticket) == gsize - 1;
      if (closes_group && NM_TID == 0) {
        As.wave_done[(grp + 1) * nm::kTicketStride] = 0;
        top = atomicAdd(As.wave_done + nm::kTicketTop, 1);
      }
      stage = 2;
    }
  };
  nm::wave_step<real, G>(sh, Ms, As, wave, copy_model, draw);
  if (As.dbg && NM_TID == 0) {
    const unsigned long long t_end = __builtin_amdgcn_s_memtime();
    real* d = As.dbg + (size_t)(wave * G) * nm::kDbgN + 250;
    d[0] = (real)(unsigned)(t_start & 0xFFFFFF); d[1] = (real)(unsigned)((t_start >> 24) & 0xFFFFFF);
    d[2] = (real)(unsigned)(t_end & 0xFFFFFF); d[3] = (real)(unsigned)((t_end >> 24) & 0xFFFFFF);
    d[4] = (real)(__builtin_amdgcn_s_getreg(4 | (0 << 6) | (15 << 11)) & 0xFFFF);
    d[5] = (real)(__builtin_amdgcn_s_getreg(20 | (0 << 6) | (3 << 11)) & 0xF);
  }
  if (As.physics_only) return;
  if (stage < 1) draw(0);
  if (stage < 2) draw(1);
  if (!closes_group) return;
  if (__builtin_amdgcn_readfirstlane(top) != ngrp - 1) return;
#ifndef NM_SKIP_TAIL2
  step_tail<real>(As, Ms.ep_len_s);
#endif
}


template <class real>
__global__ void k_reset(nm::Model<real> M, nm::Args<real> A, const int32_t* ids, int n) {
  int j = blockIdx.x * blockDim.x + threadIdx.x;
  if (j >= n) return;
  int env = ids ? ids[j] : j;
  for (int k = 0; k < nm::kNQ; k++) A.qpos[env * nm::kNQ + k] = M.qpos0[k];
  for (int k = 0; k < nm::kNV; k++) A.qvel[env * nm::kNV + k] = real(0);
  real ux, uy;
  uint32_t ctr = A.rngctr[env];
  if (A.cmd_u) { ux = A.cmd_u[env * 4 + 2]; uy = A.cmd_u[env * 4 + 3]; }
  else {
    ux = (real)nm::rand_u24_bits(A.seed, (uint64_t)(A.env_offset + env), ctr) * real(1.0 / 16777216.0);
    uy = (real)nm::rand_u24_bits(A.seed, (uint64_t)(A.env_offset + env), ctr + 1) * real(1.0 / 16777216.0);
    ctr += 2;
  }
  real c0 = ux * real(2) * M.max_lin_x - M.max_lin_x, c2 = uy * real(2) * M.max_ang - M.max_ang;
  real keep = sqrt(c0 * c0) > real(0.02) ? real(1) : real(0);
  A.cmd[env * 3] = c0 * keep; A.cmd[env * 3 + 1] = real(0); A.cmd[env * 3 + 2] = c2;
  A.rngctr[env] = ctr;
  A.eplen[env] = 0;
  for (int k = 0; k < nm::kNLEG; k++) A.feetair[env * nm::kNLEG + k] = real(0);
  for (int k = 0; k < nm::kNREW; k++) {
    atomicAdd(A.stat_sum + k, A.epsum[env * nm::kNREW + k]);
    A.epsum[env * nm::kNREW + k] = real(0);
  }
  atomicAdd(A.stat_cnt, 1);
}

template <class real>
__global__ void k_finalize(int N, real* stat_sum, int* stat_cnt, float* ep_stats, const float* timeout_now, float* time_outs,
                           real ep_len_s, long long* counters) {
  __shared__ int cnt;
  if (threadIdx.x == 0) cnt = stat_cnt[0];
  __syncthreads();
  if (cnt > 0) {
    if (threadIdx.x < nm::kNREW && ep_stats) ep_stats[threadIdx.x] = (float)(stat_sum[threadIdx.x] / (real)cnt / ep_len_s);
    if (time_outs && timeout_now)
      for (int i = threadIdx.x; i < N; i += blockDim.x) time_outs[i] = timeout_now[i];
  }
  __syncthreads();
  if (threadIdx.x < nm::kNREW) stat_sum[threadIdx.x] = real(0);
  if (threadIdx.x == 0) {
    stat_cnt[0] = 0;
    counters[0] += stat_cnt[1];
    counters[1] += stat_cnt[2];
    counters[2] += stat_cnt[3];
    stat_cnt[1] = 0;
    stat_cnt[2] = 0;
    stat_cnt[3] = 0;
  }
}

struct nm_env {
  int N = 0, device = 0, dtype = 0;
  virtual ~nm_env() {}
  virtual int reset(const int32_t* ids, int n, int64_t* eplen, float* ep_stats, hipStream_t s) = 0;
  virtual int step(const float* actions, int64_t* eplen, float* obs, float* rew, int64_t* done, float* time_outs, float* ep_stats,
                   int physics_only, hipStream_t s) = 0;
  virtual int get_state(double* qpos, double* qvel, double* qw) = 0;
  virtual int set_state(const double* qpos, const double* qvel, const double* qw) = 0;
  virtual int get_buffers(double* dp, double* dv, double* act, double* cmd, double* es) = 0;
  virtual int set_buffers(const double* dp, const double* dv, const double* act, const double* cmd, const double* es) = 0;
  virtual int set_cmd_u(const double* u) = 0;
  virtual int get_feet(double* air, unsigned char* last, unsigned char* filt) = 0;
  virtual int set_feet(const double* air, const unsigned char* last, const unsigned char* filt) = 0;
  virtual int counters(int64_t* out) = 0;
  virtual void set_dbg(void* p) = 0;
  virtual void set_ret_acc(float* p) = 0;
  virtual int invalidate_time_outs(hipStream_t s) = 0;
  virtual int rollout(const nm_rollout_args* r, int act, hipStream_t s) = 0;
  virtual int rollout_act(const float* flat, const float* obs, uint64_t seed, const int64_t* iter_dev, int step, int act, float* actions, float* logp, float* values,
                          float* mu, float* sigma, float* obs_store, hipStream_t s) = 0;
  virtual int profiling(int on, double* sum_ms, int64_t* count) = 0;
  virtual void set_ablate(int m) = 0;
  virtual int set_noise(const double* vec) = 0;
  virtual int set_noise_u(const double* u) = 0;
  virtual int set_record(int idx) = 0;
  virtual int get_record(double* qpos, double* qvel, int32_t* nbad) = 0;
  virtual int play(const nm_play_args* r, int act, hipStream_t s) = 0;
  virtual int get_log(int first, int count, double* rows) = 0;
  virtual int get_log_dones(int first, int count, unsigned char* dones) = 0;
};

template <class real> struct Env : nm_env {
  nmhost::Tables<real> T;
  nm::Model<real> M;
  nm::Args<real> A;
  std::vector<void*> allocs;
  real* cmd_u_dev = nullptr;
  bool cmd_u_on = false;
  float* timeout_now = nullptr;
  int32_t* ids_dev = nullptr;
  long long* counters_dev = nullptr;
  nm::Model<real>* M_dev = nullptr;
  real* noise_vec_dev = nullptr;
  real* noise_u_dev = nullptr;
  bool noise_on = false, noise_u_on = false;
  uint64_t noise_step = 0;
  real* rec_dev = nullptr;
  int rec_env = -1;
  real* rec_log = nullptr;
  int rec_log_cap = 0, rec_log_rows = 0;
  unsigned char* rec_done = nullptr;
  bool rec_done_valid = false;
  const real* rec_last = nullptr;
  bool prof_on = false;
  std::vector<std::pair<hipEvent_t, hipEvent_t>> prof_ev;
  size_t prof_used = 0;

  char* slab = nullptr;
  size_t slab_size = 0, slab_used = 0;
  int slab_init(size_t bytes) {
    slab_size = (bytes + (2u << 20) - 1) & ~(size_t)((2u << 20) - 1);
    HIPCHK(hipMalloc((void**)&slab, slab_size));
    HIPCHK(hipMemset(slab, 0, slab_size));
    allocs.push_back(slab);
    return 0;
  }
  template <class X> int dalloc(X** p, size_t n) {
    const size_t bytes = (n * sizeof(X) + 255) & ~(size_t)255;
    if (slab && slab_used + bytes <= slab_size) {
      *p = (X*)(slab + slab_used);
      slab_used += bytes;
      return 0;
    }
    HIPCHK(hipMalloc((void**)p, n * sizeof(X)));
    HIPCHK(hipMemset(*p, 0, n * sizeof(X)));
    allocs.push_back(*p);
    return 0;
  }
  template <class X> int upload(const X** p, const std::vector<X>& v) {
    X* d;
    if (dalloc(&d, v.size())) return 1;
    HIPCHK(hipMemcpy(d, v.data(), v.size() * sizeof(X), hipMemcpyHostToDevice));
    *p = d;
    return 0;
  }
  int init(const nmhost::EnvConfig& cfg, int n, int dev, uint64_t seed, int64_t off) {
    N = n; device = dev; dtype = sizeof(real) == 8;
    HIPCHK(hipSetDevice(dev));
    T.build();
    memset(&M, 0, sizeof M);
    memset(&A, 0, sizeof A);
    T.fill_scalars(M, cfg);
#ifdef NM_MEASURE
    if (const char* e = getenv("NM_MEASURE_PGS_ITERS")) M.pgs_iters = atoi(e);
    if (const char* e = getenv("NM_MEASURE_NOSLIP_ITERS")) M.noslip_iters = atoi(e);
#endif
    if (slab_init((T.hullv.size() + T.hullnv.size()) * sizeof(real) + (size_t)n * 300 * sizeof(real) + (size_t)n * 64 + (1u << 20))) return 1;
    if (upload(&M.hullv, T.hullv) || upload(&M.hullnv, T.hullnv)) return 1;
    A.N = N; A.seed = seed; A.env_offset = off; A.nsub = cfg.decimation;
    {
      int nx = 0;
      if (hipDeviceGetAttribute(&nx, hipDeviceAttributeNumberOfXccs, dev) != hipSuccess) { (void)hipGetLastError(); nx = 0; }
      A.nxcd = nx;
    }
    size_t n_ = (size_t)N;
    if (dalloc(&A.qpos, n_ * 25) || dalloc(&A.qvel, n_ * 24) || dalloc(&A.qwarm, n_ * 24) || dalloc(&A.dofpos, n_ * 18) ||
        dalloc(&A.dofvel, n_ * 18) || dalloc(&A.act, n_ * 18) || dalloc(&A.cmd, n_ * 3) || dalloc(&A.epsum, n_ * nm::kNREW) || dalloc(&A.feetair, n_ * nm::kNLEG) || dalloc(&A.feetflags, n_) ||
        dalloc(&A.rngctr, n_) || dalloc(&A.hullcache, n_ * 8) || dalloc(&A.stat_sum, nm::kNREW) || dalloc(&A.stat_cnt, 4) || dalloc(&cmd_u_dev, n_ * 4) ||
        dalloc(&timeout_now, n_) || dalloc(&ids_dev, n_) || dalloc(&counters_dev, 4) || dalloc(&A.wave_done, ((n_ + nm::kTicketGroup - 1) / nm::kTicketGroup + 2) * nm::kTicketStride) || dalloc(&A.nto, 1) || dalloc(&A.to_list, n_) || dalloc(&A.nprev, 1) || dalloc(&A.to_prev, n_) || dalloc(&A.to_owner, 1))
      return 1;
    if (dalloc(&M_dev, 1)) return 1;
    HIPCHK(hipMemcpy(M_dev, &M, sizeof M, hipMemcpyHostToDevice));
    std::vector<real> q0(n_ * 25);
    for (size_t i = 0; i < n_; i++)
      for (int k = 0; k < 25; k++) q0[i * 25 + k] = T.qpos0[k];
    HIPCHK(hipMemcpy(A.qpos, q0.data(), q0.size() * sizeof(real), hipMemcpyHostToDevice));
    return 0;
  }
  ~Env() override {
    (void)hipSetDevice(device);
    (void)hipDeviceSynchronize();
    for (auto& ev : prof_ev) { (void)hipEventDestroy(ev.first); (void)hipEventDestroy(ev.second); }
    for (void* p : allocs) (void)hipFree(p);
  }
  int finalize(float* ep_stats, float* time_outs, hipStream_t s) {
    hipLaunchKernelGGL(k_finalize<real>, dim3(1), dim3(1024), 0, s, N, A.stat_sum, A.stat_cnt, ep_stats, timeout_now, time_outs, M.ep_len_s,
                       counters_dev);
    HIPCHK(hipGetLastError());
    return 0;
  }
  int reset(const int32_t* ids, int n, int64_t* eplen, float* ep_stats, hipStream_t s) override {
    HIPCHK(hipSetDevice(device));
    if (!eplen) return fail("nm_reset: episode_length_dev is NULL");
    const int32_t* idp = nullptr;
    if (ids) {
      if (n <= 0) return 0;
      for (int i = 0; i < n; i++)
        if (ids[i] < 0 || ids[i] >= N) return fail("nm_reset: env id out of range");
      HIPCHK(hipMemcpyAsync(ids_dev, ids, sizeof(int32_t) * n, hipMemcpyHostToDevice, s));
      HIPCHK(hipStreamSynchronize(s));
      idp = ids_dev;
    } else n = N;
    nm::Args<real> a = A;
    a.eplen = eplen;
    a.cmd_u = cmd_u_on ? cmd_u_dev : nullptr;
    hipLaunchKernelGGL(k_reset<real>, dim3((n + 255) / 256), dim3(256), 0, s, M, a, idp, n);
    HIPCHK(hipGetLastError());
    return finalize(ep_stats, nullptr, s);
  }
  int step(const float* actions, int64_t* eplen, float* obs, float* rew, int64_t* done, float* time_outs, float* ep_stats, int physics_only,
           hipStream_t s) override {
    HIPCHK(hipSetDevice(device));
    if (!actions) return fail("nm_step: actions_dev is NULL");
    if (!physics_only && (!eplen || !obs || !rew || !done)) return fail("nm_step: NULL output pointer");
    nm::Args<real> a = A;
    a.actions = actions; a.eplen = eplen; a.obs = obs; a.rew = rew; a.done = done; a.timeout_now = timeout_now;
    a.cmd_u = cmd_u_on ? cmd_u_dev : nullptr;
    a.physics_only = physics_only;
    a.ep_stats = ep_stats; a.time_outs = time_outs; a.counters = counters_dev;
    if (!physics_only) {
      a.noise_vec = noise_on ? noise_vec_dev : nullptr;
      a.noise_u = noise_on && noise_u_on ? noise_u_dev : nullptr;
      a.noise_step = noise_step++;
      a.rec = rec_env >= 0 ? rec_dev : nullptr;
      a.rec_env = rec_env;
      if (rec_env >= 0) rec_last = rec_dev;
    }
    hipEvent_t e0 = nullptr, e1 = nullptr;
    if (prof_on) {
      if (prof_used == prof_ev.size()) {
        HIPCHK(hipEventCreate(&e0));
        HIPCHK(hipEventCreate(&e1));
        prof_ev.push_back({e0, e1});
      }
      e0 = prof_ev[prof_used].first; e1 = prof_ev[prof_used].second;
      prof_used++;
      HIPCHK(hipEventRecord(e0, s));
    }
    constexpr int G = sizeof(real) == 8 ? 1 : NM_ENVS_PER_WAVE;
    constexpr int W = sizeof(real) == 8 ? 1 : kWG;
    hipLaunchKernelGGL((k_env_step<real, G>), dim3((N + G * W - 1) / (G * W)), dim3(64 * W), 0, s, (const nm::Model<real>*)M_dev, a);
    HIPCHK(hipGetLastError());
    if (prof_on) HIPCHK(hipEventRecord(e1, s));
    return 0;
  }
  int d2h(const real* dev, double* host, size_t n) {
    if (!host) return 0;
    std::vector<real> tmp(n);
    HIPCHK(hipMemcpy(tmp.data(), dev, n * sizeof(real), hipMemcpyDeviceToHost));
    for (size_t i = 0; i < n; i++) host[i] = (double)tmp[i];
    return 0;
  }
  int h2d(real* dev, const double* host, size_t n) {
    if (!host) return 0;
    std::vector<real> tmp(n);
    for (size_t i = 0; i < n; i++) tmp[i] = (real)host[i];
    HIPCHK(hipMemcpy(dev, tmp.data(), n * sizeof(real), hipMemcpyHostToDevice));
    return 0;
  }
  int get_state(double* qpos, double* qvel, double* qw) override {
    HIPCHK(hipSetDevice(device));
    HIPCHK(hipDeviceSynchronize());
    return d2h(A.qpos, qpos, (size_t)N * 25) || d2h(A.qvel, qvel, (size_t)N * 24) || d2h(A.qwarm, qw, (size_t)N * 24);
  }
  int set_state(const double* qpos, const double* qvel, const double* qw) override {
    HIPCHK(hipSetDevice(device));
    HIPCHK(hipDeviceSynchronize());
    return h2d(A.qpos, qpos, (size_t)N * 25) || h2d(A.qvel, qvel, (size_t)N * 24) || h2d(A.qwarm, qw, (size_t)N * 24);
  }
  int get_buffers(double* dp, double* dv, double* act, double* cmd, double* es) override {
    HIPCHK(hipSetDevice(device));
    HIPCHK(hipDeviceSynchronize());
    return d2h(A.dofpos, dp, (size_t)N * 18) || d2h(A.dofvel, dv, (size_t)N * 18) || d2h(A.act, act, (size_t)N * 18) ||
           d2h(A.cmd, cmd, (size_t)N * 3) || d2h(A.epsum, es, (size_t)N * nm::kNREW);
  }
  int set_buffers(const double* dp, const double* dv, const double* act, const double* cmd, const double* es) override {
    HIPCHK(hipSetDevice(device));
    HIPCHK(hipDeviceSynchronize());
    return h2d(A.dofpos, dp, (size_t)N * 18) || h2d(A.dofvel, dv, (size_t)N * 18) || h2d(A.act, act, (size_t)N * 18) ||
           h2d(A.cmd, cmd, (size_t)N * 3) || h2d(A.epsum, es, (size_t)N * nm::kNREW);
  }
  int get_feet(double* air, unsigned char* last, unsigned char* filt) override {
    HIPCHK(hipSetDevice(device));
    HIPCHK(hipDeviceSynchronize());
    if (d2h(A.feetair, air, (size_t)N * 6)) return 1;
    std::vector<int> fl(N);
    HIPCHK(hipMemcpy(fl.data(), A.feetflags, sizeof(int) * N, hipMemcpyDeviceToHost));
    for (int i = 0; i < N; i++)
      for (int k = 0; k < 6; k++) {
        if (last) last[i * 6 + k] = (fl[i] >> k) & 1;
        if (filt) filt[i * 6 + k] = (fl[i] >> (6 + k)) & 1;
      }
    return 0;
  }
  int set_feet(const double* air, const unsigned char* last, const unsigned char* filt) override {
    HIPCHK(hipSetDevice(device));
    HIPCHK(hipDeviceSynchronize());
    if (h2d(A.feetair, air, (size_t)N * 6)) return 1;
    if (last || filt) {
      std::vector<int> fl(N);
      HIPCHK(hipMemcpy(fl.data(), A.feetflags, sizeof(int) * N, hipMemcpyDeviceToHost));
      for (int i = 0; i < N; i++)
        for (int k = 0; k < 6; k++) {
          if (last) fl[i] = (fl[i] & ~(1 << k)) | ((last[i * 6 + k] ? 1 : 0) << k);
          if (filt) fl[i] = (fl[i] & ~(1 << (6 + k))) | ((filt[i * 6 + k] ? 1 : 0) << (6 + k));
        }
      HIPCHK(hipMemcpy(A.feetflags, fl.data(), sizeof(int) * N, hipMemcpyHostToDevice));
    }
    return 0;
  }
  int set_cmd_u(const double* u) override {
    HIPCHK(hipSetDevice(device));
    HIPCHK(hipDeviceSynchronize());
    cmd_u_on = u != nullptr;
    return h2d(cmd_u_dev, u, (size_t)N * 4);
  }
  int counters(int64_t* out) override {
    HIPCHK(hipSetDevice(device));
    HIPCHK(hipDeviceSynchronize());
    long long c[3];
    HIPCHK(hipMemcpy(c, counters_dev, sizeof c, hipMemcpyDeviceToHost));
    std::vector<int> hc((size_t)N * 8);
    HIPCHK(hipMemcpy(hc.data(), A.hullcache, hc.size() * sizeof(int), hipMemcpyDeviceToHost));
    long long fb = 0;
    for (int i = 0; i < N; i++) fb += hc[(size_t)i * 8 + 7];
    out[0] = c[0]; out[1] = c[1]; out[2] = fb;
    return 0;
  }
  int set_noise(const double* vec) override {
    HIPCHK(hipSetDevice(device));
    HIPCHK(hipDeviceSynchronize());
    noise_on = vec != nullptr;
    if (vec && !noise_vec_dev && dalloc(&noise_vec_dev, NM_NUM_OBS)) return 1;
    return vec ? h2d(noise_vec_dev, vec, NM_NUM_OBS) : 0;
  }
  int set_noise_u(const double* u) override {
    HIPCHK(hipSetDevice(device));
    HIPCHK(hipDeviceSynchronize());
    noise_u_on = u != nullptr;
    if (u && !noise_u_dev && dalloc(&noise_u_dev, (size_t)N * NM_NUM_OBS)) return 1;
    return u ? h2d(noise_u_dev, u, (size_t)N * NM_NUM_OBS) : 0;
  }
  int set_record(int idx) override {
    HIPCHK(hipSetDevice(device));
    HIPCHK(hipDeviceSynchronize());
    if (idx >= N) return fail("nm_set_state_record: env index out of range");
    if (idx >= 0 && !rec_dev && dalloc(&rec_dev, 64)) return 1;
    rec_env = idx < 0 ? -1 : idx;
    rec_last = nullptr; rec_log_rows = 0; rec_done_valid = false;
    return 0;
  }
  int get_record(double* qpos, double* qvel, int32_t* nbad) override {
    HIPCHK(hipSetDevice(device));
    if (rec_env < 0) return fail("nm_get_state_record: recording is off (nm_set_state_record)");
    if (!rec_last) return fail("nm_get_state_record: no step has been recorded yet");
    HIPCHK(hipDeviceSynchronize());
    double tmp[50];
    if (d2h(rec_last, tmp, 50)) return 1;
    if (qpos) for (int i = 0; i < 25; i++) qpos[i] = tmp[i];
    if (qvel) for (int i = 0; i < 24; i++) qvel[i] = tmp[25 + i];
    if (nbad) *nbad = (int32_t)tmp[49];
    return 0;
  }

  int get_log(int first, int count, double* rows) override {
    HIPCHK(hipSetDevice(device));
    if (rec_env < 0) return fail("nm_get_state_log: recording is off (nm_set_state_record)");
    if (first < 0 || count < 0 || first + count > rec_log_rows) return fail("nm_get_state_log: rows outside the last K-step launch");
    if (count == 0) return 0;
    if (!rows) return fail("nm_get_state_log: rows_host is NULL");
    HIPCHK(hipDeviceSynchronize());
    return d2h(rec_log + (size_t)first * nmr::kRecRow, rows, (size_t)count * nmr::kRecRow);
  }
  int get_log_dones(int first, int count, unsigned char* dones) override {
    HIPCHK(hipSetDevice(device));
    if (rec_env < 0) return fail("nm_get_state_log_dones: recording is off (nm_set_state_record)");
    if (!rec_done_valid) return fail("nm_get_state_log_dones: the last K-step launch was not nm_play (nm_rollout files the flags in its dones rows)");
    if (first < 0 || count < 0 || first + count > rec_log_rows) return fail("nm_get_state_log_dones: steps outside the last K-step launch");
    if (count == 0) return 0;
    if (!dones) return fail("nm_get_state_log_dones: dones_host is NULL");
    HIPCHK(hipDeviceSynchronize());
    HIPCHK(hipMemcpy(dones, rec_done + first, (size_t)count, hipMemcpyDeviceToHost));
    return 0;
  }
  int log_rows(int K, real** out) {
    *out = nullptr;
    if (rec_env < 0) return 0;
    if (K > rec_log_cap) {
      if (dalloc(&rec_log, (size_t)roll_cap * nmr::kRecRow) || dalloc(&rec_done, (size_t)roll_cap)) return 1;
      rec_log_cap = roll_cap;
    }
    rec_log_rows = K;
    rec_done_valid = false;
    rec_last = rec_log + (size_t)(K - 1) * nmr::kRecRow;
    *out = rec_log;
    return 0;
  }
  int roll_reserve(int K) {
    if (K > roll_cap) {
      const int cap = (K + 127) & ~127;
      if (dalloc(&roll_sum, (size_t)cap * nm::kNREW) || dalloc(&roll_cnt, (size_t)cap * 4)) return 1;
      if (!roll_to && dalloc(&roll_to, (size_t)N)) return 1;
      roll_cap = cap;
    }
    return 0;
  }
  float *roll_wp = nullptr, *roll_bp = nullptr;
  real* roll_sum = nullptr;
  int *roll_cnt = nullptr, *roll_to = nullptr;
  int roll_cap = 0;
  typedef nmr::RefShape RS;
  int roll_pack(const float* flat, hipStream_t s) {
    if (!roll_wp && (dalloc(&roll_wp, (size_t)RS::nfrag() * 256) || dalloc(&roll_bp, (size_t)RS::nbias()))) return 1;
    if (nmr::launch_pack(flat, roll_wp, roll_bp, s)) return fail("nm_rollout: packing the policy failed to launch");
    return 0;
  }
  int rollout_act(const float* flat, const float* obs, uint64_t seed, const int64_t* iter_dev, int step, int act, float* actions, float* logp, float* values,
                  float* mu, float* sigma, float* obs_store, hipStream_t s) override {
    HIPCHK(hipSetDevice(device));
    if (!flat || !obs || !iter_dev || !actions || !logp || !values || !mu || !sigma) return fail("nm_rollout_act: NULL pointer");
    if (roll_pack(flat, s)) return 1;
    nmr::ActOut o{actions, logp, values, mu, sigma, obs_store};
    if (nmr::launch_act(roll_wp, roll_bp, flat + RS::stdoff(), obs, N, seed, iter_dev, step, o, act, s)) return fail("nm_rollout_act: launch failed");
    return 0;
  }
  int rollout(const nm_rollout_args* r, int act, hipStream_t s) override {
    HIPCHK(hipSetDevice(device));
    if constexpr (sizeof(real) == 8 || NM_ENVS_PER_WAVE != 2) {
      return fail("nm_rollout: the fused rollout runs on the fp32 kernel (two envs per wave) only");
    } else {
      if (!r) return fail("nm_rollout: args is NULL");
      const int K = r->steps;
      if (K < 1 || K > 4096) return fail("nm_rollout: steps must be in 1..4096");
      if ((double)K > (double)M.max_ep_len) return fail("nm_rollout: more steps than an episode has (an env may time out once per rollout)");
      if (!r->params_flat_dev || !r->iter_dev || !r->obs0_dev || !r->obs_final_dev || !r->episode_length_dev || !r->rew_dev || !r->done_dev || !r->s_obs ||
          !r->s_actions || !r->s_logp || !r->s_values || !r->s_mu || !r->s_sigma || !r->s_rewards || !r->s_dones || !r->cur_ret || !r->cur_len || !r->fin3)
        return fail("nm_rollout: NULL pointer");
      if (r->n_ep < 0 || r->n_ep > nm::kNREW || (r->n_ep > 0 && (!r->ep_idx_dev || !r->ep_acc_dev || !r->ep_stats_dev))) return fail("nm_rollout: bad episode-statistics arguments");
      real* log = nullptr;
      if (roll_reserve(K) || log_rows(K, &log)) return 1;
      if (roll_pack(r->params_flat_dev, s)) return 1;
      nm::Args<real> a = A;
      a.actions = nullptr; a.eplen = r->episode_length_dev; a.obs = r->obs_final_dev; a.rew = r->rew_dev; a.done = r->done_dev; a.timeout_now = timeout_now;
      a.cmd_u = cmd_u_on ? cmd_u_dev : nullptr;
      a.physics_only = 0;
      a.ep_stats = nullptr; a.time_outs = nullptr; a.counters = counters_dev;
      a.to_list = nullptr;
      a.noise_vec = noise_on ? noise_vec_dev : nullptr;
      a.noise_u = noise_on && noise_u_on ? noise_u_dev : nullptr;
      a.noise_step = noise_step;
      noise_step += (uint64_t)K;
      a.rec = log; a.rec_env = log ? rec_env : -1; a.dbg = nullptr; a.ret_acc = nullptr;
      nmr::RollArgs R;
      R.K = K; R.wp = (const nmr::f32x4*)roll_wp; R.bp = roll_bp; R.stdv = r->params_flat_dev + RS::stdoff();
      R.seed = r->seed; R.iter_dev = r->iter_dev; R.obs0 = r->obs0_dev; R.obs_final = r->obs_final_dev;
      R.s_obs = r->s_obs; R.s_actions = r->s_actions; R.s_logp = r->s_logp; R.s_values = r->s_values; R.s_mu = r->s_mu; R.s_sigma = r->s_sigma;
      R.s_rewards = r->s_rewards; R.s_dones = r->s_dones; R.cur_ret = r->cur_ret; R.cur_len = r->cur_len; R.fin3 = r->fin3;
      R.st_sum = roll_sum; R.st_cnt = roll_cnt; R.to_step = roll_to;
      R.last_values = r->last_values_dev;
      R.rec_log = log;
      R.wave_clock = A.dbg ? reinterpret_cast<unsigned long long*>(A.dbg) : nullptr;
      nmr::TailArgs ta{N, K, roll_sum, roll_cnt, roll_to, r->ep_stats_dev, r->time_outs_dev, M.ep_len_s, counters_dev, r->bootstrap_time_outs ? r->gamma : -1.0f, r->s_values, r->s_rewards,
                       r->ep_idx_dev, r->n_ep, r->ep_acc_dev, A.to_owner};
      if (nmr::launch_rollout(M_dev, a, R, ta, act, s)) return fail("nm_rollout: launch failed");
      return 0;
    }
  }
  float* play_scratch = nullptr;
  int play(const nm_play_args* r, int act, hipStream_t s) override {
    HIPCHK(hipSetDevice(device));
    if constexpr (sizeof(real) == 8 || NM_ENVS_PER_WAVE != 2) {
      return fail("nm_play: the play kernel runs on the fp32 kernel (two envs per wave) only");
    } else {
      if (!r) return fail("nm_play: args is NULL");
      const int K = r->steps;
      if (K < 1 || K > 4096) return fail("nm_play: steps must be in 1..4096 (longer runs: consecutive launches)");
      if (!r->params_flat_dev || !r->iter_dev || !r->obs0_dev || !r->obs_dev || !r->actions_dev || !r->episode_length_dev || !r->rew_dev || !r->done_dev)
        return fail("nm_play: NULL pointer");
      if (r->n_ep < 0 || r->n_ep > nm::kNREW || (r->n_ep > 0 && (!r->ep_idx_dev || !r->ep_acc_dev || !r->ep_stats_dev))) return fail("nm_play: bad episode-statistics arguments");
      if ((r->cur_ret == nullptr) != (r->cur_len == nullptr) || (r->ret_sum == nullptr) != (r->ret_cnt == nullptr))
        return fail("nm_play: cur_ret / cur_len and ret_sum / ret_cnt come in pairs");
      real* log = nullptr;
      if (roll_reserve(K) || log_rows(K, &log)) return 1;
      if (!play_scratch && dalloc(&play_scratch, (size_t)N * 4 + 4)) return 1;
      if (roll_pack(r->params_flat_dev, s)) return 1;
      nm::Args<real> a = A;
      a.actions = r->actions_dev; a.eplen = r->episode_length_dev; a.obs = r->obs_dev; a.rew = r->rew_dev; a.done = r->done_dev; a.timeout_now = timeout_now;
      a.cmd_u = cmd_u_on ? cmd_u_dev : nullptr;
      a.physics_only = 0;
      a.ep_stats = nullptr; a.time_outs = nullptr; a.counters = counters_dev;
      a.to_list = nullptr;
      a.noise_vec = noise_on ? noise_vec_dev : nullptr;
      a.noise_u = noise_on && noise_u_on ? noise_u_dev : nullptr;
      a.noise_step = noise_step;
      noise_step += (uint64_t)K;
      a.rec = log; a.rec_env = log ? rec_env : -1; a.dbg = nullptr; a.ret_acc = nullptr;
      nmr::PlayArgs P;
      P.K = K; P.deterministic = r->deterministic != 0;
      P.wp = (const nmr::f32x4*)roll_wp; P.bp = roll_bp; P.stdv = r->params_flat_dev + RS::stdoff();
      P.seed = r->seed; P.iter_dev = r->iter_dev; P.step0 = r->step0;
      P.obs0 = r->obs0_dev; P.obs = r->obs_dev; P.actions = r->actions_dev;
      const size_t n_ = (size_t)N;
      P.cur_ret = r->cur_ret ? r->cur_ret : play_scratch; P.cur_len = r->cur_len ? r->cur_len : play_scratch + n_;
      P.ret_sum = r->ret_sum ? r->ret_sum : play_scratch + 2 * n_; P.ret_cnt = r->ret_cnt ? r->ret_cnt : play_scratch + 3 * n_;
      P.fin3 = r->fin3 ? r->fin3 : play_scratch + 4 * n_;
      P.st_sum = roll_sum; P.st_cnt = roll_cnt; P.to_step = roll_to;
      P.rec_log = log; P.rec_done = log ? rec_done : nullptr; P.rec_env = rec_env;
      rec_done_valid = log != nullptr;
      nmr::TailArgs ta{N, K, roll_sum, roll_cnt, roll_to, r->ep_stats_dev, r->time_outs_dev, M.ep_len_s, counters_dev, -1.0f, nullptr, nullptr,
                       r->ep_idx_dev, r->n_ep, r->ep_acc_dev, A.to_owner};
      if (nmr::launch_play(M_dev, a, P, ta, act, s)) return fail("nm_play: launch failed");
      return 0;
    }
  }
  void set_dbg(void* p) override { A.dbg = (real*)p; }
  void set_ret_acc(float* p) override { A.ret_acc = p; }
  int invalidate_time_outs(hipStream_t s) override {
    HIPCHK(hipSetDevice(device));
    HIPCHK(hipMemsetAsync(A.to_owner, 0, sizeof(unsigned long long), s));
    return 0;
  }
  void set_ablate(int m) override { A.ablate = m; }
  int profiling(int on, double* sum_ms, int64_t* count) override {
    HIPCHK(hipSetDevice(device));
    HIPCHK(hipDeviceSynchronize());
    double sum = 0;
    for (size_t i = 0; i < prof_used; i++) {
      float ms = 0;
      HIPCHK(hipEventElapsedTime(&ms, prof_ev[i].first, prof_ev[i].second));
      sum += ms;
    }
    if (sum_ms) *sum_ms = sum;
    if (count) *count = (int64_t)prof_used;
    prof_used = 0;
    prof_on = on != 0;
    return 0;
  }
};

static const char* kRewardNames[NM_NUM_REWARDS] = {"action_rate", "ang_vel_xy", "base_height", "body_contact_forces", "default_position", "dof_acc",
                                                   "dof_vel", "feet_air_time", "feet_contact_forces", "lin_vel_z", "orientation", "stand_still",
                                                   "torques", "tracking_ang_vel", "tracking_lin_vel", "termination"};
static_assert(NM_NUM_REWARDS == nm::kNREW, "reward table size");
extern "C" {
const char* nm_last_error(void) { return g_err.c_str(); }
int nm_policy_set_error(const char* m) { return fail(m); }
const char* nm_reward_name(int i) { return (i >= 0 && i < NM_NUM_REWARDS) ? kRewardNames[i] : ""; }
void nm_default_config(nm_config* c) {
  nmhost::EnvConfig d;
  c->decimation = d.decimation; c->p_gain = d.p_gain; c->action_scale = d.action_scale;
  for (int i = 0; i < 3; i++) c->default_pos[i] = d.default_pos[i];
  c->clip_actions = d.clip_actions; c->clip_observations = d.clip_observations;
  c->obs_lin_vel = d.obs_lin_vel; c->obs_ang_vel = d.obs_ang_vel; c->obs_dof_pos = d.obs_dof_pos; c->obs_dof_vel = d.obs_dof_vel;
  c->episode_length_s = d.episode_length_s; c->resampling_time = d.resampling_time;
  c->max_lin_vel_x = d.max_lin_vel_x; c->max_ang_vel = d.max_ang_vel;
  c->termination_contact_force = d.termination_contact_force; c->tracking_sigma = d.tracking_sigma;
  for (int i = 0; i < NM_NUM_REWARDS; i++) c->reward_scales[i] = d.rew_scales[i];
  c->tibia_contact_mode = d.tibia_contact_mode; c->tibia_max_contact_force = d.tibia_max_contact_force;
  c->body_contact_mode = d.body_contact_mode; c->body_max_contact_force = d.body_max_contact_force;
  c->base_height_target = d.base_height_target; c->max_contact_force = d.max_contact_force;
}
int nm_create(const nm_config* cfg, int32_t num_envs, int32_t device, uint64_t seed, int64_t env_id_offset, int32_t dtype, nm_env** out) {
  if (!out) return fail("nm_create: out is NULL");
  *out = nullptr;
  if (num_envs <= 0) return fail("nm_create: num_envs must be positive");
  int ndev = 0;
  if (hipGetDeviceCount(&ndev) != hipSuccess || ndev == 0)
    return fail("nm_create: no HIP device available (this backend has no CPU path)");
  if (device < 0 || device >= ndev) return fail("nm_create: bad device index");
  nmhost::EnvConfig c;
  if (cfg) {
    if (cfg->decimation < 1) return fail("nm_create: decimation must be >= 1");
    if (!(cfg->episode_length_s > 0)) return fail("nm_create: episode_length_s must be positive");
    if ((int)(cfg->resampling_time / (NM_TIMESTEP * cfg->decimation)) < 1) return fail("nm_create: resampling_time must be at least one env step (dt)");
    if (cfg->tibia_contact_mode < 0 || cfg->tibia_contact_mode > 2 || cfg->body_contact_mode < 0 || cfg->body_contact_mode > 2)
      return fail("nm_create: contact modes are 0 (ignore), 1 (penalise) or 2 (terminate)");
    c.decimation = cfg->decimation; c.p_gain = cfg->p_gain; c.action_scale = cfg->action_scale;
    for (int i = 0; i < 3; i++) c.default_pos[i] = cfg->default_pos[i];
    c.clip_actions = cfg->clip_actions; c.clip_observations = cfg->clip_observations;
    c.obs_lin_vel = cfg->obs_lin_vel; c.obs_ang_vel = cfg->obs_ang_vel; c.obs_dof_pos = cfg->obs_dof_pos; c.obs_dof_vel = cfg->obs_dof_vel;
    c.episode_length_s = cfg->episode_length_s; c.resampling_time = cfg->resampling_time;
    c.max_lin_vel_x = cfg->max_lin_vel_x; c.max_ang_vel = cfg->max_ang_vel;
    c.termination_contact_force = cfg->termination_contact_force; c.tracking_sigma = cfg->tracking_sigma;
    for (int i = 0; i < NM_NUM_REWARDS; i++) c.rew_scales[i] = cfg->reward_scales[i];
    c.tibia_contact_mode = cfg->tibia_contact_mode; c.tibia_max_contact_force = cfg->tibia_max_contact_force;
    c.body_contact_mode = cfg->body_contact_mode; c.body_max_contact_force = cfg->body_max_contact_force;
    c.base_height_target = cfg->base_height_target; c.max_contact_force = cfg->max_contact_force;
  }
  nm_env* e;
  int rc;
  if (dtype == NM_DTYPE_F64) { auto* p = new Env<double>(); rc = p->init(c, num_envs, device, seed, env_id_offset); e = p; }
  else if (dtype == NM_DTYPE_F32) { auto* p = new Env<float>(); rc = p->init(c, num_envs, device, seed, env_id_offset); e = p; }
  else return fail("nm_create: dtype must be NM_DTYPE_F32 or NM_DTYPE_F64");
  if (rc) { delete e; return 1; }
  *out = e;
  return 0;
}
int nm_destroy(nm_env* env) { delete env; return 0; }
int32_t nm_num_envs(const nm_env* env) { return env ? env->N : 0; }
int32_t nm_dtype(const nm_env* env) { return env ? env->dtype : -1; }
#define NEED(e) if (!(e)) return fail("null nm_env")
int nm_reset(nm_env* env, const int32_t* ids, int32_t n, int64_t* eplen, float* ep_stats, void* stream) {
  NEED(env); return env->reset(ids, n, eplen, ep_stats, (hipStream_t)stream);
}
int nm_step(nm_env* env, const float* actions, int64_t* eplen, float* obs, float* rew, int64_t* done, float* time_outs, float* ep_stats,
            void* stream) {
  NEED(env); return env->step(actions, eplen, obs, rew, done, time_outs, ep_stats, 0, (hipStream_t)stream);
}
int nm_step_physics(nm_env* env, const float* actions, void* stream) {
  NEED(env); return env->step(actions, nullptr, nullptr, nullptr, nullptr, nullptr, nullptr, 1, (hipStream_t)stream);
}
int nm_get_state(nm_env* env, double* qpos, double* qvel, double* qw) { NEED(env); return env->get_state(qpos, qvel, qw); }
int nm_set_state(nm_env* env, const double* qpos, const double* qvel, const double* qw) { NEED(env); return env->set_state(qpos, qvel, qw); }
int nm_get_buffers(nm_env* env, double* dp, double* dv, double* act, double* cmd, double* es) { NEED(env); return env->get_buffers(dp, dv, act, cmd, es); }
int nm_set_buffers(nm_env* env, const double* dp, const double* dv, const double* act, const double* cmd, const double* es) {
  NEED(env); return env->set_buffers(dp, dv, act, cmd, es);
}
int nm_get_feet_state(nm_env* env, double* air, unsigned char* last, unsigned char* filt) { NEED(env); return env->get_feet(air, last, filt); }
int nm_set_feet_state(nm_env* env, const double* air, const unsigned char* last, const unsigned char* filt) { NEED(env); return env->set_feet(air, last, filt); }
int nm_set_command_uniforms(nm_env* env, const double* u) { NEED(env); return env->set_cmd_u(u); }
int nm_get_counters(nm_env* env, int64_t* out2) { NEED(env); return env->counters(out2); }
int nm_set_debug_buffer(nm_env* env, void* dbg) { NEED(env); env->set_dbg(dbg); return 0; }
int nm_set_return_accumulator(nm_env* env, float* acc) { NEED(env); env->set_ret_acc(acc); return 0; }
int nm_invalidate_time_outs(nm_env* env, void* stream) { NEED(env); return env->invalidate_time_outs((hipStream_t)stream); }
int nm_rollout_supported(const int32_t* actor_dims, const int32_t* critic_dims, int32_t n_layers) {
  return nm_rollout_supported_act(actor_dims, critic_dims, n_layers, NM_ACT_ELU);
}
int nm_rollout_supported_act(const int32_t* actor_dims, const int32_t* critic_dims, int32_t n_layers, int32_t activation) {
// ... 60 lines not shown
```

nightmare_rl_amd/csrc/simt.h:

```cpp
#pragma once
#include <stdint.h>

#define NM_WAVE 64

#ifndef NM_EMUL
#include <hip/hip_runtime.h>
#define NM_FN __device__ __forceinline__
#define NM_COLD __device__ __noinline__
namespace simt {
template <class T> using V = T;
using VB = bool;

#ifdef NM_WG_WAVES
#define NM_TID ((int)(threadIdx.x & 63))
#else
#define NM_TID ((int)threadIdx.x)
#endif
NM_FN int lane_id() { return NM_TID; }
template <class T> NM_FN T sel(bool c, T a, T b) { return c ? a : b; }
NM_FN float vsqrt(float x) { return sqrtf(x); }
NM_FN double vsqrt(double x) { return sqrt(x); }
NM_FN float vabs(float x) { return fabsf(x); }
NM_FN double vabs(double x) { return fabs(x); }
NM_FN float vmax(float a, float b) { return fmaxf(a, b); }
NM_FN double vmax(double a, double b) { return fmax(a, b); }
NM_FN float vmin(float a, float b) { return fminf(a, b); }
NM_FN double vmin(double a, double b) { return fmin(a, b); }
NM_FN int vmin(int a, int b) { return a < b ? a : b; }
NM_FN int vmax(int a, int b) { return a > b ? a : b; }
NM_FN void vsincos(float x0, float* s, float* c) {
  const float x = fminf(fmaxf(x0, -4194304.0f), 4194304.0f);
  const float k = rintf(x * 0.636619772f);
  float r = fmaf(-k, 1.5707963705062866f, x);
  r = fmaf(-k, -4.371139000186241e-8f, r);
  const float r2 = r * r;
  const float ps = fmaf(r * r2, fmaf(r2, fmaf(r2, -1.9515295891e-4f, 8.3321608736e-3f), -1.6666654611e-1f), r);
  const float pc = fmaf(r2 * r2, fmaf(r2, fmaf(r2, 2.443315711809948e-5f, -1.388731625493765e-3f), 4.166664568298827e-2f), fmaf(r2, -0.5f, 1.0f));
  const int n = (int)k;
  const float sa = (n & 1) ? pc : ps, ca = (n & 1) ? ps : pc;
  *s = (n & 2) ? -sa : sa;
  *c = ((n + 1) & 2) ? -ca : ca;
}
NM_FN void vsincos(double x, double* s, double* c) { sincos(x, s, c); }
NM_FN float vexp(float x) { return expf(x); }
NM_FN double vexp(double x) { return exp(x); }
NM_FN float vacos(float x) { return acosf(x); }
NM_FN double vacos(double x) { return acos(x); }
NM_FN float vpow(float x, float p) { return powf(x, p); }
NM_FN double vpow(double x, double p) { return pow(x, p); }
NM_FN bool visbad(float x) { return !(fabsf(x) <= 1e10f); }
NM_FN bool visbad(double x) { return !(fabs(x) <= 1e10); }
template <class T> NM_FN T to_real(int i) { return (T)i; }
template <class T, class S> NM_FN T vcvt(S x) { return (T)x; }
NM_FN float vrcp(float x) { return __builtin_amdgcn_rcpf(x); }
NM_FN double vrcp(double x) { return 1.0 / x; }

NM_FN float vfma(float a, float b, float c) { return __builtin_fmaf(a, b, c); }
NM_FN double vfma(double a, double b, double c) { return __builtin_fma(a, b, c); }
NM_FN float sel_mask(uint64_t m, float a, float b) {
  float r;
  asm("v_cndmask_b32_e64 %0, %1, %2, %3" : "=v"(r) : "v"(b), "v"(a), "s"(m));
  return r;
}
NM_FN double sel_mask(uint64_t m, double a, double b) {
  int rl, rh;
  asm("v_cndmask_b32_e64 %0, %2, %3, %6\n\tv_cndmask_b32_e64 %1, %4, %5, %6" : "=&v"(rl), "=v"(rh)
      : "v"(__double2loint(b)), "v"(__double2loint(a)), "v"(__double2hiint(b)), "v"(__double2hiint(a)), "s"(m));
  return __hiloint2double(rh, rl);
}
NM_FN uint64_t mask_shl(uint64_t m, int k) { m <<= k; asm("" : "+s"(m)); return m; }
template <int I> NM_FN float fma_half_lane(float a, float x, float g, bool h1);
template <int I> NM_FN double fma_half_lane(double a, double x, double g, bool h1);
NM_FN int rdlane(int x, int l) { return __builtin_amdgcn_readlane(x, l); }
NM_FN float rdlane(float x, int l) { return __int_as_float(__builtin_amdgcn_readlane(__float_as_int(x), l)); }
NM_FN double rdlane(double x, int l) {
  int lo = __builtin_amdgcn_readlane(__double2loint(x), l), hi = __builtin_amdgcn_readlane(__double2hiint(x), l);
  return __hiloint2double(hi, lo);
}
template <int I> NM_FN float fma_half_lane(float a, float x, float g, bool h1) {
  const float s0 = rdlane(x, I), s1 = rdlane(x, 32 + I);
  return vfma(a, h1 ? s1 : s0, g);
}
template <int I> NM_FN double fma_half_lane(double a, double x, double g, bool h1) {
  const double s0 = rdlane(x, I), s1 = rdlane(x, 32 + I);
  return vfma(a, h1 ? s1 : s0, g);
}
template <class T> NM_FN T wrlane(T x, T v, int l) {
  int ln = NM_TID;
  asm volatile("" : "+v"(ln));
  return ln == l ? v : x;
}
NM_FN int opaque_lane() { int ln = NM_TID; asm volatile("" : "+v"(ln)); return ln; }
template <class T> NM_FN T uniform(T x) { return rdlane(x, 0); }
NM_FN bool uniform(bool x) { return __builtin_amdgcn_readfirstlane((int)x) != 0; }
#define NM_DPP_QUAD_XOR1 0xB1
#define NM_DPP_QUAD_XOR2 0x4E
#define NM_DPP_HALF_MIRROR 0x141
#define NM_DPP_ROW_MIRROR 0x140
template <int CTRL> NM_FN int dpp(int x) { return __builtin_amdgcn_mov_dpp(x, CTRL, 0xF, 0xF, true); }
template <int CTRL> NM_FN float dpp(float x) { return __int_as_float(dpp<CTRL>(__float_as_int(x))); }
template <int CTRL> NM_FN double dpp(double x) { return __hiloint2double(dpp<CTRL>(__double2hiint(x)), dpp<CTRL>(__double2loint(x))); }
template <int P, class T> NM_FN T quad(T x) { return dpp<P>(x); }
template <class T> NM_FN T shfl_xor1(T x) { return dpp<NM_DPP_QUAD_XOR1>(x); }
template <class T> NM_FN T shfl_xor2(T x) { return dpp<NM_DPP_QUAD_XOR2>(x); }
template <class T> NM_FN T wsum8(T x) {
  x = x + dpp<NM_DPP_QUAD_XOR1>(x);
  x = x + dpp<NM_DPP_QUAD_XOR2>(x);
  x = x + dpp<NM_DPP_HALF_MIRROR>(x);
  return rdlane(x, 0);
}
template <class T> NM_FN T gsum8(T x) {
  x = x + dpp<NM_DPP_QUAD_XOR1>(x);
  x = x + dpp<NM_DPP_QUAD_XOR2>(x);
  x = x + dpp<NM_DPP_HALF_MIRROR>(x);
  return x;
}
template <class T> NM_FN T wsum(T x) {
  x = x + dpp<NM_DPP_QUAD_XOR1>(x);
  x = x + dpp<NM_DPP_QUAD_XOR2>(x);
  x = x + dpp<NM_DPP_HALF_MIRROR>(x);
  x = x + dpp<NM_DPP_ROW_MIRROR>(x);
  return (rdlane(x, 0) + rdlane(x, 16)) + (rdlane(x, 32) + rdlane(x, 48));
}
template <class T> NM_FN T hsum32(T x) {
  x = x + dpp<NM_DPP_QUAD_XOR1>(x);
  x = x + dpp<NM_DPP_QUAD_XOR2>(x);
  x = x + dpp<NM_DPP_HALF_MIRROR>(x);
  x = x + dpp<NM_DPP_ROW_MIRROR>(x);
  const T s0 = rdlane(x, 0) + rdlane(x, 16), s1 = rdlane(x, 32) + rdlane(x, 48);
  return (NM_TID & 32) ? s1 : s0;
}
NM_FN bool wany(bool c) { return __ballot(c) != 0ull; }
NM_FN int lane_rank(uint64_t m) { return (int)__builtin_amdgcn_mbcnt_hi((uint32_t)(m >> 32), __builtin_amdgcn_mbcnt_lo((uint32_t)m, 0u)); }
NM_FN int popc64(uint64_t m) { return __popcll(m); }
NM_FN uint64_t ballot(bool c) { return __ballot(c); }
NM_FN bool in_mask(uint64_t m) { return __builtin_amdgcn_inverse_ballot_w64(m); }
template <class T> NM_FN void order_after(int& a, const T& dep) { asm volatile("" : "+v"(a) : "v"(dep)); }
template <class T> NM_FN void wargmax(T val, int idx, T* best, int* ibest) {
#define NM_AM_STEP(CTRL)                                                   \
  {                                                                        \
    T ov = dpp<CTRL>(val);                                                 \
    int oi = dpp<CTRL>(idx);                                               \
    bool take = (ov > val) | ((ov == val) & (oi < idx));                   \
    val = take ? ov : val;                                                 \
    idx = take ? oi : idx;                                                 \
  }
  NM_AM_STEP(NM_DPP_QUAD_XOR1) NM_AM_STEP(NM_DPP_QUAD_XOR2) NM_AM_STEP(NM_DPP_HALF_MIRROR) NM_AM_STEP(NM_DPP_ROW_MIRROR)
#undef NM_AM_STEP
  T bv = rdlane(val, 0);
  int bi = rdlane(idx, 0);
#pragma unroll
  for (int r = 16; r < 64; r += 16) {
    T ov = rdlane(val, r);
    int oi = rdlane(idx, r);
    bool take = (ov > bv) | ((ov == bv) & (oi < bi));
    bv = take ? ov : bv;
    bi = take ? oi : bi;
  }
  *best = bv;
  *ibest = bi;
}
template <class T> NM_FN void wmaxfirst(T val, T* best, int* lane_of_best) {
  T m = val;
  m = vmax(m, dpp<NM_DPP_QUAD_XOR1>(m));
  m = vmax(m, dpp<NM_DPP_QUAD_XOR2>(m));
  m = vmax(m, dpp<NM_DPP_HALF_MIRROR>(m));
  m = vmax(m, dpp<NM_DPP_ROW_MIRROR>(m));
  const T b = vmax(vmax(rdlane(m, 0), rdlane(m, 16)), vmax(rdlane(m, 32), rdlane(m, 48)));
  *best = b;
  *lane_of_best = (int)__builtin_ctzll(__ballot(val == b));
}
template <class T> NM_FN T ldsv(const T* a, int i) { return a[i]; }
template <class T> NM_FN void stsv(T* a, int i, T v, bool m) { if (m) a[i] = v; }
template <class T, class S> NM_FN void stsu(T* a, int i, T v, bool m, S* sink) {
  T* p = m ? a + i : reinterpret_cast<T*>(sink) + NM_TID;
  *p = v;
}
#define NM_GLOBAL(T) __attribute__((address_space(1))) T
typedef float nm_f4 __attribute__((ext_vector_type(4)));
typedef double nm_d4 __attribute__((ext_vector_type(4)));
template <class T> NM_FN T gldv(const T* p, int i) { return ((const NM_GLOBAL(T)*)p)[i]; }
template <class T> NM_FN void gstv(T* p, int i, T v, bool m) { if (m) ((NM_GLOBAL(T)*)p)[i] = v; }
template <class T> NM_FN T gld1(const T* p, size_t i) { return ((const NM_GLOBAL(T)*)p)[i]; }
template <class T> NM_FN void gst1(T* p, size_t i, T v) { ((NM_GLOBAL(T)*)p)[i] = v; }
NM_FN void gadd1(float* p, size_t i, float v) { __builtin_amdgcn_global_atomic_fadd_f32((NM_GLOBAL(float)*)p + i, v); }
NM_FN void gld3(const float* p, int i, float* o) { const nm_f4 t = *(const NM_GLOBAL(nm_f4)*)((const NM_GLOBAL(float)*)p + i); o[0] = t.x; o[1] = t.y; o[2] = t.z; }
NM_FN void gld3(const double* p, int i, double* o) { const nm_d4 t = *(const NM_GLOBAL(nm_d4)*)((const NM_GLOBAL(double)*)p + i); o[0] = t.x; o[1] = t.y; o[2] = t.z; }
NM_FN void gld4(const float* p, int i, float* o) { const nm_f4 t = *(const NM_GLOBAL(nm_f4)*)((const NM_GLOBAL(float)*)p + i); o[0] = t.x; o[1] = t.y; o[2] = t.z; o[3] = t.w; }
NM_FN void gld4(const double* p, int i, double* o) { const nm_d4 t = *(const NM_GLOBAL(nm_d4)*)((const NM_GLOBAL(double)*)p + i); o[0] = t.x; o[1] = t.y; o[2] = t.z; o[3] = t.w; }
NM_FN int to_int(float x) { return (int)x; }
NM_FN int to_int(double x) { return (int)x; }
NM_FN void wave_sync() {
  __builtin_amdgcn_fence(__ATOMIC_RELEASE, "wavefront");
  __builtin_amdgcn_wave_barrier();
  __builtin_amdgcn_fence(__ATOMIC_ACQUIRE, "wavefront");
}
NM_FN void sched_fence() { __builtin_amdgcn_sched_barrier(0); }
}

#else
#include <cmath>
#include <cstring>
#define NM_FN inline
#define NM_COLD inline
namespace simt {
template <class T> struct V {
  T v[NM_WAVE];
  V() {}
  V(T s) { for (int i = 0; i < NM_WAVE; i++) v[i] = s; }
#define NM_BIN(op)                                                                                   \
  friend V operator op(const V& a, const V& b) { V r; for (int i = 0; i < NM_WAVE; i++) r.v[i] = a.v[i] op b.v[i]; return r; }
  NM_BIN(+) NM_BIN(-) NM_BIN(*) NM_BIN(/) NM_BIN(%) NM_BIN(&) NM_BIN(|) NM_BIN(>>) NM_BIN(<<)
#undef NM_BIN
#define NM_CMP(op)                                                                                      \
  friend V<bool> operator op(const V& a, const V& b) { V<bool> r; for (int i = 0; i < NM_WAVE; i++) r.v[i] = a.v[i] op b.v[i]; return r; }
  NM_CMP(<) NM_CMP(>) NM_CMP(<=) NM_CMP(>=) NM_CMP(==) NM_CMP(!=)
#undef NM_CMP
  friend V operator-(const V& a) { V r; for (int i = 0; i < NM_WAVE; i++) r.v[i] = -a.v[i]; return r; }
  friend V operator!(const V& a) { V r; for (int i = 0; i < NM_WAVE; i++) r.v[i] = !a.v[i]; return r; }
  V& operator+=(const V& b) { for (int i = 0; i < NM_WAVE; i++) v[i] += b.v[i]; return *this; }
  V& operator-=(const V& b) { for (int i = 0; i < NM_WAVE; i++) v[i] -= b.v[i]; return *this; }
  V& operator*=(const V& b) { for (int i = 0; i < NM_WAVE; i++) v[i] *= b.v[i]; return *this; }
};
using VB = V<bool>;

NM_FN V<int> lane_id() { V<int> r; for (int i = 0; i < NM_WAVE; i++) r.v[i] = i; return r; }
#define NM_SEL(T)                                                                                              \
  NM_FN V<T> sel(const VB& c, const V<T>& a, const V<T>& b) { V<T> r; for (int i = 0; i < NM_WAVE; i++) r.v[i] = c.v[i] ? a.v[i] : b.v[i]; return r; } \
  NM_FN T sel(bool c, T a, T b) { return c ? a : b; }
NM_SEL(float) NM_SEL(double) NM_SEL(int)
#undef NM_SEL
#define NM_MAP1(name, expr)                                                                                   \
  NM_FN V<float> name(const V<float>& a) { V<float> r; for (int i = 0; i < NM_WAVE; i++) { float x = a.v[i]; r.v[i] = expr; } return r; } \
  NM_FN V<double> name(const V<double>& a) { V<double> r; for (int i = 0; i < NM_WAVE; i++) { double x = a.v[i]; r.v[i] = expr; } return r; } \
  NM_FN float name(float x) { return expr; }                                                                  \
  NM_FN double name(double x) { return expr; }
NM_MAP1(vsqrt, std::sqrt(x)) NM_MAP1(vabs, std::fabs(x)) NM_MAP1(vexp, std::exp(x)) NM_MAP1(vacos, std::acos(x))
#undef NM_MAP1
#define NM_MAP2(name, expr, T)                                                                               \
  NM_FN V<T> name(const V<T>& a, const V<T>& b) { V<T> r; for (int i = 0; i < NM_WAVE; i++) { T x = a.v[i], y = b.v[i]; r.v[i] = expr; } return r; } \
  NM_FN T name(T x, T y) { return expr; }
NM_MAP2(vmax, (x > y ? x : y), float) NM_MAP2(vmax, (x > y ? x : y), double) NM_MAP2(vmax, (x > y ? x : y), int)
NM_MAP2(vmin, (x < y ? x : y), float) NM_MAP2(vmin, (x < y ? x : y), double) NM_MAP2(vmin, (x < y ? x : y), int)
NM_MAP2(vpow, std::pow(x, y), float) NM_MAP2(vpow, std::pow(x, y), double)
#undef NM_MAP2
template <class T> NM_FN void vsincos(const V<T>& x, V<T>* s, V<T>* c) { for (int i = 0; i < NM_WAVE; i++) { s->v[i] = std::sin(x.v[i]); c->v[i] = std::cos(x.v[i]); } }
NM_FN void vsincos(float x, float* s, float* c) { *s = std::sin(x); *c = std::cos(x); }
NM_FN void vsincos(double x, double* s, double* c) { *s = std::sin(x); *c = std::cos(x); }
template <class T> NM_FN VB visbad(const V<T>& a) { VB r; for (int i = 0; i < NM_WAVE; i++) r.v[i] = !(std::fabs(a.v[i]) <= (T)1e10); return r; }
NM_FN bool visbad(float x) { return !(std::fabs(x) <= 1e10f); }
NM_FN bool visbad(double x) { return !(std::fabs(x) <= 1e10); }
template <class T> NM_FN V<T> to_real(const V<int>& a) { V<T> r; for (int i = 0; i < NM_WAVE; i++) r.v[i] = (T)a.v[i]; return r; }
template <class T> NM_FN T to_real(int a) { return (T)a; }
template <class T> NM_FN V<T> vrcp(const V<T>& a) { V<T> r; for (int i = 0; i < NM_WAVE; i++) r.v[i] = (T)1 / a.v[i]; return r; }
NM_FN float vrcp(float x) { return 1.0f / x; }
NM_FN double vrcp(double x) { return 1.0 / x; }
template <class T, class S> NM_FN V<T> vcvt(const V<S>& a) { V<T> r; for (int i = 0; i < NM_WAVE; i++) r.v[i] = (T)a.v[i]; return r; }

template <class T> NM_FN V<T> vfma(const V<T>& a, const V<T>& b, const V<T>& c) { return a * b + c; }
NM_FN float vfma(float a, float b, float c) { return a * b + c; }
NM_FN double vfma(double a, double b, double c) { return a * b + c; }
template <class T> NM_FN V<T> sel_mask(uint64_t m, const V<T>& a, const V<T>& b) {
  V<T> r;
  for (int i = 0; i < NM_WAVE; i++) r.v[i] = ((m >> i) & 1ull) ? a.v[i] : b.v[i];
  return r;
}
NM_FN uint64_t mask_shl(uint64_t m, int k) { return m << k; }
template <int I, class T> NM_FN V<T> fma_half_lane(const V<T>& a, const V<T>& x, const V<T>& g, const VB&) {
  V<T> r;
  for (int i = 0; i < NM_WAVE; i++) r.v[i] = a.v[i] * x.v[(i & 32) + I] + g.v[i];
  return r;
}
template <class T> NM_FN T rdlane(const V<T>& x, int l) { return x.v[l]; }
template <class T> NM_FN T rdlane(T x, int) { return x; }
template <class T> NM_FN V<T> wrlane(V<T> x, T v, int l) { x.v[l] = v; return x; }
NM_FN V<int> opaque_lane() { return lane_id(); }
template <class T> NM_FN T uniform(const V<T>& x) { return x.v[0]; }
template <class T> NM_FN T uniform(T x) { return x; }
template <class T> NM_FN V<T> shfl_xor(const V<T>& x, int m) { V<T> r; for (int i = 0; i < NM_WAVE; i++) r.v[i] = x.v[i ^ m]; return r; }
template <int P, class T> NM_FN V<T> quad(const V<T>& x) { V<T> r; for (int i = 0; i < NM_WAVE; i++) r.v[i] = x.v[(i & ~3) | ((P >> (2 * (i & 3))) & 3)]; return r; }
template <class T> NM_FN V<T> shfl_xor1(const V<T>& x) { return shfl_xor(x, 1); }
template <class T> NM_FN V<T> shfl_xor2(const V<T>& x) { return shfl_xor(x, 2); }
template <class T> NM_FN V<T> half_mirror(const V<T>& x) { V<T> r; for (int i = 0; i < NM_WAVE; i++) r.v[i] = x.v[(i & ~7) | (7 - (i & 7))]; return r; }
template <class T> NM_FN V<T> row_mirror(const V<T>& x) { V<T> r; for (int i = 0; i < NM_WAVE; i++) r.v[i] = x.v[(i & ~15) | (15 - (i & 15))]; return r; }
template <class T> NM_FN V<T> gsum8(V<T> x) {
  x = x + shfl_xor(x, 1); x = x + shfl_xor(x, 2); x = x + half_mirror(x);
  return x;
}
template <class T> NM_FN T wsum8(V<T> x) {
  x = x + shfl_xor(x, 1); x = x + shfl_xor(x, 2); x = x + half_mirror(x);
  return x.v[0];
}
template <class T> NM_FN T wsum(V<T> x) {
  x = x + shfl_xor(x, 1); x = x + shfl_xor(x, 2); x = x + half_mirror(x); x = x + row_mirror(x);
  return (x.v[0] + x.v[16]) + (x.v[32] + x.v[48]);
}
template <class T> NM_FN V<T> hsum32(V<T> x) {
  x = x + shfl_xor(x, 1); x = x + shfl_xor(x, 2); x = x + half_mirror(x); x = x + row_mirror(x);
  const T s0 = x.v[0] + x.v[16], s1 = x.v[32] + x.v[48];
  V<T> r; for (int i = 0; i < NM_WAVE; i++) r.v[i] = i < 32 ? s0 : s1;
  return r;
}
NM_FN bool wany(const VB& c) { for (int i = 0; i < NM_WAVE; i++) if (c.v[i]) return true; return false; }
NM_FN V<int> lane_rank(uint64_t m) { V<int> r; for (int i = 0; i < NM_WAVE; i++) r.v[i] = __builtin_popcountll(m & ((1ull << i) - 1ull)); return r; }
NM_FN int popc64(uint64_t m) { return __builtin_popcountll(m); }
NM_FN uint64_t ballot(const VB& c) { uint64_t m = 0; for (int i = 0; i < NM_WAVE; i++) if (c.v[i]) m |= 1ull << i; return m; }
NM_FN VB in_mask(uint64_t m) { VB r; for (int i = 0; i < NM_WAVE; i++) r.v[i] = (m >> i) & 1; return r; }
template <class T> NM_FN void order_after(V<int>&, const V<T>&) {}
template <class T> NM_FN void wargmax(V<T> val, V<int> idx, T* best, int* ibest) {
  T bv = val.v[0]; int bi = idx.v[0];
  for (int i = 1; i < NM_WAVE; i++)
    if (val.v[i] > bv || (val.v[i] == bv && idx.v[i] < bi)) { bv = val.v[i]; bi = idx.v[i]; }
  *best = bv; *ibest = bi;
}
template <class T> NM_FN void wmaxfirst(const V<T>& val, T* best, int* lane_of_best) {
  T bv = val.v[0]; int bi = 0;
  for (int i = 1; i < NM_WAVE; i++) if (val.v[i] > bv) { bv = val.v[i]; bi = i; }
  *best = bv; *lane_of_best = bi;
}
template <class T> NM_FN V<T> ldsv(const T* a, const V<int>& i) { V<T> r; for (int k = 0; k < NM_WAVE; k++) r.v[k] = a[i.v[k]]; return r; }
template <class T> NM_FN T ldsv(const T* a, int i) { return a[i]; }
template <class T> NM_FN void stsv(T* a, const V<int>& i, const V<T>& v, const VB& m) { for (int k = 0; k < NM_WAVE; k++) if (m.v[k]) a[i.v[k]] = v.v[k]; }
template <class T> NM_FN void stsv(T* a, const V<int>& i, T v, const VB& m) { for (int k = 0; k < NM_WAVE; k++) if (m.v[k]) a[i.v[k]] = v; }
template <class T, class S> NM_FN void stsu(T* a, const V<int>& i, const V<T>& v, const VB& m, S*) { stsv(a, i, v, m); }
template <class T, class S> NM_FN void stsu(T* a, const V<int>& i, T v, const VB& m, S*) { stsv(a, i, v, m); }
template <class T> NM_FN T gld1(const T* p, size_t i) { return p[i]; }
template <class T> NM_FN void gst1(T* p, size_t i, T v) { p[i] = v; }
NM_FN void gadd1(float* p, size_t i, float v) { p[i] += v; }
template <class T> NM_FN V<T> gldv(const T* p, const V<int>& i) { return ldsv(p, i); }
template <class T> NM_FN void gstv(T* p, const V<int>& i, const V<T>& v, const VB& m) { stsv(p, i, v, m); }
template <class T> NM_FN void gstv(T* p, const V<int>& i, T v, const VB& m) { stsv(p, i, v, m); }
template <class T> NM_FN void gld4(const T* p, const V<int>& i, V<T>* o) { for (int k = 0; k < NM_WAVE; k++) for (int c = 0; c < 4; c++) o[c].v[k] = p[i.v[k] + c]; }
template <class T> NM_FN V<int> to_int(const V<T>& a) { V<int> r; for (int i = 0; i < NM_WAVE; i++) r.v[i] = (int)a.v[i]; return r; }
template <class T> NM_FN void gld3(const T* p, const V<int>& i, V<T>* o) { for (int k = 0; k < NM_WAVE; k++) for (int c = 0; c < 3; c++) o[c].v[k] = p[i.v[k] + c]; }
template <class T> NM_FN void gld3(const T* p, int i, T* o) { o[0] = p[i]; o[1] = p[i + 1]; o[2] = p[i + 2]; }
NM_FN void wave_sync() {}
NM_FN void sched_fence() {}
}
#endif
```

Baseline: 83.99 million env-steps/s.

## Pack per-env state into 128-byte-aligned records with wide staged load/store

Replaces the separate per-field state arrays (qpos, qvel, qwarm, cmd, epsum, act, dofvel, dofpos, rngctr, hullcache, feet data) with one aligned struct-of-records per env. In the paired-env wave path, the records for both envs are fetched with 16-byte vector loads into the LDS row buffer, unpacked from LDS, then written back through LDS with 16-byte stores. The aim is to replace many small scattered global transactions with a few coalesced whole-line ones. In exchange it adds LDS staging and wave syncs, reuses the jrow buffer, and makes host state get/set pull and push the whole record array.

```diff
diff --git a/nightmare_rl_amd/csrc/nm_core.h b/nightmare_rl_amd/csrc/nm_core.h
--- a/nightmare_rl_amd/csrc/nm_core.h
+++ b/nightmare_rl_amd/csrc/nm_core.h
@@ -52,17 +52,39 @@
   real tibia_max, body_max, base_h_target, max_contact_force;
 };
 
+template <class real> struct alignas(128) EnvRec {
+  real qpos[kNQ], qvel[kNV], qwarm[kNV];
+  int hullcache[8];
+  real cmd[3], epsum[kNREW], act[kNU], dofvel[kNU], dofpos[kNU];
+  uint32_t rngctr;
+  alignas(16) real feetair[kNLEG];
+  int feetflags;
+};
+template <class real> struct RecLayout {
+  typedef EnvRec<real> R;
+  static constexpr int kBytes = (int)sizeof(R);
+  static constexpr int kWide = (int)offsetof(R, feetair);
+  static constexpr int kPieces = kWide / 16;
+  static constexpr int kRW = kBytes / (int)sizeof(real), kRI = kBytes / 4;
+  static constexpr int kStB = (kWide + 32 * (int)sizeof(real) + 15) & ~15;
+  static constexpr int kSW = kStB / (int)sizeof(real), kSI = kStB / 4;
+  static_assert(sizeof(R) % 128 == 0 && alignof(R) == 128, "records are whole 128-byte lines");
+  static_assert(kWide % 16 == 0 && offsetof(R, rngctr) + 4 <= (size_t)kWide, "the wide part is whole 16-byte pieces");
+};
+#define NM_ROFS(field) ((int)(offsetof(EnvRec<real>, field) / sizeof(real)))
+#define NM_RIOFS(field) ((int)(offsetof(EnvRec<real>, field) / sizeof(int)))
+
 template <class real> struct Args {
   int N;
   uint64_t seed;
   int64_t env_offset;
-  real *qpos, *qvel, *qwarm;
-  real *dofpos, *dofvel, *act, *cmd, *epsum;
-  real* feetair;
-  int* feetflags;
+  EnvRec<real>* st;
   int64_t* eplen;
+#ifdef NM_EMUL
+  real *qpos, *qvel, *qwarm, *dofpos, *dofvel, *act, *cmd, *epsum, *feetair;
+  int *feetflags, *hullcache;
   uint32_t* rngctr;
-  int* hullcache;
+#endif
   const float* actions;
   const real* cmd_u;
   float *obs, *rew, *timeout_now;
@@ -2557,22 +2579,23 @@
   const V<int> lane = opaque_lane();
   const VB l18 = lane < kNU;
   const V<int> l18c = sel(l18, lane, V<int>(0));
-  const vr q_in = gldv(A.qpos, sel(lane < kNQ, lane, V<int>(0)) + env * kNQ);
-  const vr v_in = gldv(A.qvel, sel(lane < kNV, lane, V<int>(0)) + env * kNV);
-  const vr w_in = gldv(A.qwarm, sel(lane < kNV, lane, V<int>(0)) + env * kNV);
-  const V<int> hc_in = gldv(A.hullcache, sel(lane < 8, lane, V<int>(0)) + env * 8);
+  constexpr int kRW = RecLayout<real>::kRW, kRI = RecLayout<real>::kRI;
+  const vr q_in = gldv(A.st->qpos, sel(lane < kNQ, lane, V<int>(0)) + env * kRW);
+  const vr v_in = gldv(A.st->qvel, sel(lane < kNV, lane, V<int>(0)) + env * kRW);
+  const vr w_in = gldv(A.st->qwarm, sel(lane < kNV, lane, V<int>(0)) + env * kRW);
+  const V<int> hc_in = gldv(A.st->hullcache, sel(lane < 8, lane, V<int>(0)) + env * kRI);
   const V<float> a_in = gldv(A.actions, l18c + env * kNU);
   vr cmd_in = vr(real(0)), eps_in = vr(real(0)), prev_act = vr(real(0)), prev_dofvel = vr(real(0)), dofpos_old = vr(real(0));
   int64_t ep = 0;
   uint32_t ctr_in = 0;
   if (!A.physics_only) {
-    cmd_in = gldv(A.cmd, sel(lane < 3, lane, V<int>(0)) + env * 3);
-    eps_in = gldv(A.epsum, sel(lane < kNREW, lane, V<int>(0)) + env * kNREW);
+    cmd_in = gldv(A.st->cmd, sel(lane < 3, lane, V<int>(0)) + env * kRW);
+    eps_in = gldv(A.st->epsum, sel(lane < kNREW, lane, V<int>(0)) + env * kRW);
     ep = gld1(A.eplen, env);
-    ctr_in = gld1(A.rngctr, env);
-    prev_act = gldv(A.act, l18c + env * kNU);
-    prev_dofvel = gldv(A.dofvel, l18c + env * kNU);
-    dofpos_old = gldv(A.dofpos, l18c + env * kNU);
+    ctr_in = gld1(&A.st->rngctr, (size_t)env * kRI);
+    prev_act = gldv(A.st->act, l18c + env * kRW);
+    prev_dofvel = gldv(A.st->dofvel, l18c + env * kRW);
+    dofpos_old = gldv(A.st->dofpos, l18c + env * kRW);
   }
   stsv(sh.qpos, lane, q_in, lane < kNQ);
   stsv(sh.qvel, lane, v_in, lane < kNV);
@@ -2648,6 +2671,7 @@
   const VB l18 = lane < kNU;
   const V<int> l18c = sel(l18, lane, V<int>(0));
   const vr act = ldsv(sh.eact, l18c), prev_act = ldsv(sh.epact, l18c), prev_dofvel = ldsv(sh.epdv, l18c);
+  constexpr int kRW = RecLayout<real>::kRW, kRI = RecLayout<real>::kRI;
   vr defp;
   {
     V<int> m3 = lane % 3;
@@ -2657,10 +2681,10 @@
     const V<int> hc = ldsv(sh.hcache, sel(lane < 8, lane, V<int>(0)));
     const vr q = ldsv(sh.qpos, sel(lane < kNQ, lane, V<int>(0))), v = ldsv(sh.qvel, sel(lane < kNV, lane, V<int>(0))),
              w = ldsv(sh.warm, sel(lane < kNV, lane, V<int>(0)));
-    gstv(A.hullcache, lane + env * 8, hc, lane < 8);
-    gstv(A.qpos, lane + env * kNQ, q, lane < kNQ);
-    gstv(A.qvel, lane + env * kNV, v, lane < kNV);
-    gstv(A.qwarm, lane + env * kNV, w, lane < kNV);
+    gstv(A.st->hullcache, lane + env * kRI, hc, lane < 8);
+    gstv(A.st->qpos, lane + env * kRW, q, lane < kNQ);
+    gstv(A.st->qvel, lane + env * kRW, v, lane < kNV);
+    gstv(A.st->qwarm, lane + env * kRW, w, lane < kNV);
   }
   if (A.rec && env == A.rec_env) {
     gstv(A.rec, lane, ldsv(sh.qpos, sel(lane < kNQ, lane, V<int>(0))), lane < kNQ);
@@ -2747,8 +2771,8 @@
   V<int> l8c = sel(lane < kNREW, lane, V<int>(0));
   epsum[0] = ldsv(sh.eepsum, l8c);
   if (reset) {
-    gstv(A.qpos, lane + env * kNQ, ldsv(M.qpos0, sel(lane < kNQ, lane, V<int>(0))), lane < kNQ);
-    gstv(A.qvel, lane + env * kNV, real(0), lane < kNV);
+    gstv(A.st->qpos, lane + env * kRW, ldsv(M.qpos0, sel(lane < kNQ, lane, V<int>(0))), lane < kNQ);
+    gstv(A.st->qvel, lane + env * kRW, real(0), lane < kNV);
     resample(1);
     eplen = 0;
 #ifdef NM_EMUL
@@ -2800,8 +2824,8 @@
       vr over = sel(ff > vr(M.max_contact_force), ff - M.max_contact_force, vr(real(0)));
       rt[R_FEET_CONTACT] = wsum<real>(sel(l6, over * over, vr(real(0)))) * M.rew_scale[R_FEET_CONTACT];
       if (M.rew_scale[R_FEET_AIR_TIME] != real(0)) {
-        vr air = gldv(A.feetair, l6c + env * kNLEG);
-        const V<int> fl = V<int>(gld1(A.feetflags, env));
+        vr air = gldv(A.st->feetair, l6c + env * kRW);
+        const V<int> fl = V<int>(gld1(&A.st->feetflags, (size_t)env * kRI));
         if (reset) air = vr(real(0));
         const VB contact = ff > vr(real(1));
         const VB filt = contact | (((fl >> l6c) & 1) != 0);
@@ -2810,12 +2834,12 @@
         air = sel(filt == lastf, air, vr(real(0)));
         const vr single = sel(air > vr(real(1)), air - real(1), vr(real(0))) + sel(air < vr(real(0.5)), real(0.5) - air, vr(real(0)));
         rt[R_FEET_AIR_TIME] = wsum<real>(sel(l6, single * single, vr(real(0)))) * M.rew_scale[R_FEET_AIR_TIME];
-        gstv(A.feetair, l6c + env * kNLEG, air, l6);
+        gstv(A.st->feetair, l6c + env * kRW, air, l6);
         const int nf = (int)(ballot(l6 & contact) | (ballot(l6 & filt) << kNLEG));
 #ifdef NM_EMUL
-        A.feetflags[env] = nf;
+        A.st[env].feetflags = nf;
 #else
-        if (NM_TID == 0) gst1(A.feetflags, env, nf);
+        if (NM_TID == 0) gst1(&A.st->feetflags, (size_t)env * kRI, nf);
 #endif
       }
     }
@@ -2827,7 +2851,7 @@
     vr add = vr(real(0));
 #pragma unroll
     for (int k = 0; k < kNREW; k++) add = wrlane(add, rt[k], k);
-    gstv(A.epsum, lane + env * kNREW, epsum[0] + add, lane < kNREW);
+    gstv(A.st->epsum, lane + env * kRW, epsum[0] + add, lane < kNREW);
   }
   NM_ESTAMP(14);
   {
@@ -2863,12 +2887,12 @@
     put(act, lane + 48, l18);
   }
   NM_ESTAMP(15);
-  gstv(A.dofpos, lane + env * kNU, dofpos, l18);
-  gstv(A.dofvel, lane + env * kNU, dofvel, l18);
-  gstv(A.act, lane + env * kNU, act, l18);
+  gstv(A.st->dofpos, lane + env * kRW, dofpos, l18);
+  gstv(A.st->dofvel, lane + env * kRW, dofvel, l18);
+  gstv(A.st->act, lane + env * kRW, act, l18);
   {
     vr cv = sel(lane == 0, vr(cmd[0]), sel(lane == 1, vr(cmd[1]), vr(cmd[2])));
-    gstv(A.cmd, lane + env * 3, cv, lane < 3);
+    gstv(A.st->cmd, lane + env * kRW, cv, lane < 3);
   }
 #ifdef NM_EMUL
   const bool lane0 = true;
@@ -2877,7 +2901,7 @@
 #endif
   if (lane0) {
     gst1(A.eplen, env, eplen);
-    gst1(A.rngctr, env, ctr);
+    gst1(&A.st->rngctr, (size_t)env * kRI, ctr);
     gst1(A.rew, env, (float)rew);
     if (A.ret_acc) gadd1(A.ret_acc, env, (float)rew);
     gst1(A.done, env, (int64_t)(reset ? 1 : 0));
@@ -2898,28 +2922,38 @@
   const V<int> ho = h * kSR, hoi = h * kSI;
   const VB l18 = hl < kNU;
   const V<int> l18c = sel(l18, hl, V<int>(0));
-  const vr q_in = gldv(A.qpos, sel(hl < kNQ, hl, V<int>(0)) + env * kNQ);
-  const vr v_in = gldv(A.qvel, sel(hl < kNV, hl, V<int>(0)) + env * kNV);
-  const vr w_in = gldv(A.qwarm, sel(hl < kNV, hl, V<int>(0)) + env * kNV);
-  const V<int> hc_in = gldv(A.hullcache, sel(hl < 8, hl, V<int>(0)) + env * 8);
+  typedef RecLayout<real> RL;
+  constexpr int kNLd = (2 * RL::kPieces + 63) / 64;
+  static_assert((size_t)2 * RL::kStB <= sizeof(w.jrow), "the staged records fit the row buffer");
+  W16 pc[kNLd];
+  V<int> slot[kNLd];
+#pragma unroll
+  for (int k = 0; k < kNLd; k++) {
+    const V<int> p0 = lane + 64 * k;
+    const V<int> p = sel(p0 < V<int>(2 * RL::kPieces), p0, V<int>(0));
+    const V<int> r = sel(p < V<int>(RL::kPieces), V<int>(0), V<int>(1));
+    const V<int> er0 = r + wave * 2;
+    const V<int> er = sel(er0 < V<int>(A.N), er0, V<int>(A.N - 1));
+    pc[k] = gld16(A.st, er * RL::kBytes + (p - r * RL::kPieces) * 16);
+    slot[k] = r * RL::kStB + (p - r * RL::kPieces) * 16;
+  }
   const V<float> a_in = gldv(A.actions, l18c + env * kNU);
-  vr cmd_in = vr(real(0)), eps_in = vr(real(0)), prev_act = vr(real(0)), prev_dofvel = vr(real(0)), dofpos_old = vr(real(0));
 #ifndef NM_EMUL
   int64_t ep = 0;
-  uint32_t ctr_in = 0;
+  if (!A.physics_only) ep = gld1(A.eplen, (size_t)env);
 #endif
-  if (!A.physics_only) {
-    cmd_in = gldv(A.cmd, sel(hl < 3, hl, V<int>(0)) + env * 3);
-    eps_in = gldv(A.epsum, sel(hl < kNREW, hl, V<int>(0)) + env * kNREW);
-#ifndef NM_EMUL
-    ep = gld1(A.eplen, (size_t)env);
-    ctr_in = gld1(A.rngctr, (size_t)env);
-#endif
-    prev_act = gldv(A.act, l18c + env * kNU);
-    prev_dofvel = gldv(A.dofvel, l18c + env * kNU);
-    dofpos_old = gldv(A.dofpos, l18c + env * kNU);
-  }
   mid();
+#pragma unroll
+  for (int k = 0; k < kNLd; k++) sts16(w.jrow, slot[k], pc[k]);
+  wave_sync();
+  const real* stg = w.jrow;
+  const int* stgi = reinterpret_cast<const int*>(w.jrow);
+  const V<int> hs = h * RL::kSW + hl, hsi = h * RL::kSI + hl;
+  const vr q_in = ldsv(stg, hs + NM_ROFS(qpos)), v_in = ldsv(stg, hs + NM_ROFS(qvel)), w_in = ldsv(stg, hs + NM_ROFS(qwarm));
+  const V<int> hc_in = ldsv(stgi, hsi + NM_RIOFS(hullcache));
+  const vr cmd_in = ldsv(stg, hs + NM_ROFS(cmd)), eps_in = ldsv(stg, hs + NM_ROFS(epsum)), prev_act = ldsv(stg, hs + NM_ROFS(act)),
+           prev_dofvel = ldsv(stg, hs + NM_ROFS(dofvel)), dofpos_old = ldsv(stg, hs + NM_ROFS(dofpos));
+  const V<int> ctr_in = ldsv(stgi, hsi + NM_RIOFS(rngctr));
   stsv(rb, ho + (hl + NM_OFS(qpos)), q_in, hl < kNQ);
   stsv(rb, ho + (hl + NM_OFS(qvel)), v_in, hl < kNV);
   stsv(rb, ho + (hl + NM_OFS(warm)), w_in, hl < kNV);
@@ -2950,13 +2984,12 @@
       const int64_t ep = A.eplen[e];
       w.e[hh].eplen_lo = (int)(uint32_t)(ep & 0xffffffffll);
       w.e[hh].eplen_hi = (int)(ep >> 32);
-      w.e[hh].ectr = A.rngctr[e];
     }
 #else
     stsv(ib, hoi + NM_IOFS(eplen_lo), (int)(uint32_t)(ep & 0xffffffffll), hl == 0);
     stsv(ib, hoi + NM_IOFS(eplen_hi), (int)(ep >> 32), hl == 0);
-    stsv(ib, hoi + NM_IOFS(ectr), (int)ctr_in, hl == 0);
 #endif
+    stsv(ib, hoi + NM_IOFS(ectr), ctr_in, hl == 0);
     stsv(rb, ho + (hl + NM_OFS(ctrl)), ((act - defp) - dofpos_old) * M.p_gain, l18);
   } else {
     wave_sync();
@@ -2981,6 +3014,12 @@
   const V<int> ho = h * kSR, hoi = h * kSI;
 #define SHR(field, idx) ldsv(rb, ho + ((idx) + NM_OFS(field)))
 #define SHI(field, idx) ldsv(ib, hoi + ((idx) + NM_IOFS(field)))
+  typedef RecLayout<real> RL;
+  constexpr int kRW = RL::kRW, kRI = RL::kRI;
+  const bool narrow = A.physics_only || (NM_ABLATE(A.ablate) & 128);
+  real* stg = w.jrow;
+  int* stgi = reinterpret_cast<int*>(w.jrow);
+  const V<int> hs = h * RL::kSW + hl, hsi = h * RL::kSI + hl;
   const VB l18 = hl < kNU;
   const V<int> l18c = sel(l18, hl, V<int>(0));
   const vr act = SHR(eact, l18c), prev_act = SHR(epact, l18c), prev_dofvel = SHR(epdv, l18c);
@@ -2994,10 +3033,17 @@
     V<int> hc = SHI(hcache, sel(hl < 8, hl, V<int>(0)));
     hc = sel(hl == 0, hc | (SHI(ncon, V<int>(0)) << 16), hc);
     const vr q = SHR(qpos, sel(hl < kNQ, hl, V<int>(0))), v = SHR(qvel, sel(hl < kNV, hl, V<int>(0))), wq = SHR(warm, sel(hl < kNV, hl, V<int>(0)));
-    gstv(A.hullcache, hl + env * 8, hc, live & (hl < 8));
-    gstv(A.qpos, hl + env * kNQ, q, live & (hl < kNQ));
-    gstv(A.qvel, hl + env * kNV, v, live & (hl < kNV));
-    gstv(A.qwarm, hl + env * kNV, wq, live & (hl < kNV));
+    if (narrow) {
+      gstv(A.st->hullcache, hl + env * kRI, hc, live & (hl < 8));
+      gstv(A.st->qpos, hl + env * kRW, q, live & (hl < kNQ));
+      gstv(A.st->qvel, hl + env * kRW, v, live & (hl < kNV));
+      gstv(A.st->qwarm, hl + env * kRW, wq, live & (hl < kNV));
+    } else {
+      stsv(stg, hs + NM_ROFS(qpos), q, VB(true));
+      stsv(stg, hs + NM_ROFS(qvel), v, VB(true));
+      stsv(stg, hs + NM_ROFS(qwarm), wq, VB(true));
+      stsv(stgi, hsi + NM_RIOFS(hullcache), hc, VB(true));
+    }
     if (A.rec) {
       const VB r = live & (env == V<int>(A.rec_env));
       gstv(A.rec, hl, q, r & (hl < kNQ));
@@ -3101,8 +3147,8 @@
   const VB resetL = reset & live;
   const uint64_t rmask = ballot(resetL);
   if (rmask) {
-    gstv(A.qpos, hl + env * kNQ, ldsv(M.qpos0, sel(hl < kNQ, hl, V<int>(0))), resetL & (hl < kNQ));
-    gstv(A.qvel, hl + env * kNV, real(0), resetL & (hl < kNV));
+    stsv(stg, hs + NM_ROFS(qpos), ldsv(M.qpos0, sel(hl < kNQ, hl, V<int>(0))), resetL & (hl < kNQ));
+    stsv(stg, hs + NM_ROFS(qvel), vr(real(0)), resetL & (hl < kNV));
 #pragma unroll
     for (int hh = 0; hh < 2; hh++)
       if ((rmask >> (32 * hh)) & 1) { resample(hh, 1); ep[hh] = 0; }
@@ -3159,8 +3205,8 @@
       vr over = sel(ff > vr(M.max_contact_force), ff - M.max_contact_force, vr(real(0)));
       rt[R_FEET_CONTACT] = hsum32(sel(l6, over * over, vr(real(0)))) * M.rew_scale[R_FEET_CONTACT];
       if (M.rew_scale[R_FEET_AIR_TIME] != real(0)) {
-        vr air = gldv(A.feetair, l6c + envc * kNLEG);
-        const V<int> fl = gldv(A.feetflags, envc);
+        vr air = gldv(A.st->feetair, l6c + envc * kRW);
+        const V<int> fl = gldv(&A.st->feetflags, envc * kRI);
         air = sel(reset, vr(real(0)), air);
         const VB contact = ff > vr(real(1));
         const VB filt = contact | (((fl >> l6c) & 1) != 0);
@@ -3169,10 +3215,10 @@
         air = sel(filt == lastf, air, vr(real(0)));
         const vr single = sel(air > vr(real(1)), air - real(1), vr(real(0))) + sel(air < vr(real(0.5)), real(0.5) - air, vr(real(0)));
         rt[R_FEET_AIR_TIME] = hsum32(sel(l6, single * single, vr(real(0)))) * M.rew_scale[R_FEET_AIR_TIME];
-        gstv(A.feetair, l6c + env * kNLEG, air, live & l6);
+        gstv(A.st->feetair, l6c + env * kRW, air, live & l6);
         const uint64_t bc = ballot(l6 & contact), bf = ballot(l6 & filt);
         const int nf0 = (int)((bc & 63) | ((bf & 63) << kNLEG)), nf1 = (int)(((bc >> 32) & 63) | (((bf >> 32) & 63) << kNLEG));
-        gstv(A.feetflags, env, sel(h1, V<int>(nf1), V<int>(nf0)), live & (hl == 0));
+        gstv(&A.st->feetflags, env * kRI, sel(h1, V<int>(nf1), V<int>(nf0)), live & (hl == 0));
       }
     }
   }
@@ -3183,7 +3229,9 @@
     vr add = vr(real(0));
 #pragma unroll
     for (int k = 0; k < kNREW; k++) add = sel(hl == k, rt[k], add);
-    gstv(A.epsum, hl + env * kNREW, epsum + add, live & (hl < kNREW));
+    const vr cv = sel(hl == 0, cmd[0], sel(hl == 1, cmd[1], cmd[2]));
+    stsv(stg, hs + NM_ROFS(cmd), cv, VB(true));
+    stsv(stg, hs + NM_ROFS(epsum), epsum + add, VB(true));
   }
   published(1);
   NM_ESTAMP(14);
@@ -3221,25 +3269,41 @@
     put(act, hl + 48, l18);
   }
   NM_ESTAMP(15);
-  gstv(A.dofpos, hl + env * kNU, dofpos, live & l18);
-  gstv(A.dofvel, hl + env * kNU, dofvel, live & l18);
-  gstv(A.act, hl + env * kNU, act, live & l18);
-  {
-    vr cv = sel(hl == 0, cmd[0], sel(hl == 1, cmd[1], cmd[2]));
-    gstv(A.cmd, hl + env * 3, cv, live & (hl < 3));
+  stsv(stg, hs + NM_ROFS(act), act, VB(true));
+  stsv(stg, hs + NM_ROFS(dofvel), dofvel, VB(true));
+  stsv(stg, hs + NM_ROFS(dofpos), dofpos, VB(true));
+  stsv(stgi, hsi + NM_RIOFS(rngctr), sel(h1, V<int>((int)ctr[1]), V<int>((int)ctr[0])), VB(true));
+  wave_sync();
+  {
+    constexpr int kNSt = (2 * RL::kPieces + 63) / 64;
+    W16 pc[kNSt];
+    V<int> dst[kNSt];
+#pragma unroll
+    for (int k = 0; k < kNSt; k++) {
+      const V<int> p0 = lane + 64 * k;
+      const V<int> p = sel(p0 < V<int>(2 * RL::kPieces), p0, V<int>(0));
+      const V<int> r = sel(p < V<int>(RL::kPieces), V<int>(0), V<int>(1));
+      pc[k] = lds16(stg, r * RL::kStB + (p - r * RL::kPieces) * 16);
+      dst[k] = (r + wave * 2) * RL::kBytes + (p - r * RL::kPieces) * 16;
+    }
+#pragma unroll
+    for (int k = 0; k < kNSt; k++) {
+      const V<int> p0 = lane + 64 * k;
+      const V<int> er = sel(p0 < V<int>(RL::kPieces), V<int>(0), V<int>(1)) + wave * 2;
+      gst16(A.st, dst[k], pc[k], (p0 < V<int>(2 * RL::kPieces)) & (er < V<int>(A.N)));
+    }
   }
 #ifdef NM_EMUL
   for (int hh = 0; hh < 2; hh++)
     if (lives[hh]) {
       const int e = wave * 2 + hh, l0 = 32 * hh;
-      A.eplen[e] = ep[hh]; A.rngctr[e] = ctr[hh]; A.rew[e] = (float)rew.v[l0];
+      A.eplen[e] = ep[hh]; A.rew[e] = (float)rew.v[l0];
       if (A.ret_acc) A.ret_acc[e] += (float)rew.v[l0];
       A.done[e] = (int64_t)(reset.v[l0] ? 1 : 0); A.timeout_now[e] = time_out.v[l0] ? 1.0f : 0.0f;
     }
 #else
   if (hl == 0 && live) {
     gst1(A.eplen, (size_t)env, h1 ? ep[1] : ep[0]);
-    gst1(A.rngctr, (size_t)env, h1 ? ctr[1] : ctr[0]);
     gst1(A.rew, (size_t)env, (float)rew);
     if (A.ret_acc) gadd1(A.ret_acc, (size_t)env, (float)rew);
     gst1(A.done, (size_t)env, (int64_t)(reset ? 1 : 0));
@@ -3251,7 +3315,7 @@
 }
 
 template <class real, int G, class Mid = NoMid, class Pub = NoMid>
-NM_FN void wave_step(ShW<real, G>& w, const Model<real>& M, const Args<real>& A, int wave, Mid&& mid = Mid(), Pub&& published = Pub()) {
+NM_FN void wave_step_rec(ShW<real, G>& w, const Model<real>& M, const Args<real>& A, int wave, Mid&& mid = Mid(), Pub&& published = Pub()) {
   nm_stamp(-1);
   if constexpr (G == 2) {
     env_load2(w, M, A, wave, mid);
@@ -3280,4 +3344,33 @@
   nm_stamp(10);
 }
 
-}
+#ifndef NM_EMUL
+template <class real, int G, class Mid = NoMid, class Pub = NoMid>
+NM_FN void wave_step(ShW<real, G>& w, const Model<real>& M, const Args<real>& A, int wave, Mid&& mid = Mid(), Pub&& published = Pub()) {
+  wave_step_rec<real, G>(w, M, A, wave, mid, published);
+}
+#else
+template <class real, int G, class Mid = NoMid, class Pub = NoMid>
+inline void wave_step(ShW<real, G>& w, const Model<real>& M, const Args<real>& A, int wave, Mid&& mid = Mid(), Pub&& published = Pub()) {
+  if (A.st) { wave_step_rec<real, G>(w, M, A, wave, mid, published); return; }
+  static thread_local EnvRec<real>* recs = nullptr;
+  static thread_local int cap = 0;
+  if (cap < A.N) { delete[] recs; recs = new EnvRec<real>[A.N](); cap = A.N; }
+  auto move = [&](int e, bool pack) {
+    EnvRec<real>& R = recs[e];
+    auto f = [&](real* rec, real* arr, int K) { for (int k = 0; k < K; k++) { if (pack) rec[k] = arr[(size_t)e * K + k]; else arr[(size_t)e * K + k] = rec[k]; } };
+    f(R.qpos, A.qpos, kNQ); f(R.qvel, A.qvel, kNV); f(R.qwarm, A.qwarm, kNV); f(R.cmd, A.cmd, 3); f(R.epsum, A.epsum, kNREW);
+    f(R.act, A.act, kNU); f(R.dofvel, A.dofvel, kNU); f(R.dofpos, A.dofpos, kNU); f(R.feetair, A.feetair, kNLEG);
+    for (int k = 0; k < 8; k++) { if (pack) R.hullcache[k] = A.hullcache[(size_t)e * 8 + k]; else A.hullcache[(size_t)e * 8 + k] = R.hullcache[k]; }
+    if (pack) { R.rngctr = A.rngctr[e]; R.feetflags = A.feetflags[e]; } else { A.rngctr[e] = R.rngctr; A.feetflags[e] = R.feetflags; }
+  };
+  for (int g = 0; g < G; g++) if (wave * G + g < A.N) move(wave * G + g, true);
+  move(A.N - 1, true);
+  Args<real> B = A;
+  B.st = recs;
+  wave_step_rec<real, G>(w, M, B, wave, mid, published);
+  for (int g = 0; g < G; g++) if (wave * G + g < A.N) move(wave * G + g, false);
+}
+#endif
+
+}
diff --git a/nightmare_rl_amd/csrc/nm_hip.hip b/nightmare_rl_amd/csrc/nm_hip.hip
--- a/nightmare_rl_amd/csrc/nm_hip.hip
+++ b/nightmare_rl_amd/csrc/nm_hip.hip
@@ -152,10 +152,11 @@
   int j = blockIdx.x * blockDim.x + threadIdx.x;
   if (j >= n) return;
   int env = ids ? ids[j] : j;
-  for (int k = 0; k < nm::kNQ; k++) A.qpos[env * nm::kNQ + k] = M.qpos0[k];
-  for (int k = 0; k < nm::kNV; k++) A.qvel[env * nm::kNV + k] = real(0);
+  nm::EnvRec<real>& R = A.st[env];
+  for (int k = 0; k < nm::kNQ; k++) R.qpos[k] = M.qpos0[k];
+  for (int k = 0; k < nm::kNV; k++) R.qvel[k] = real(0);
   real ux, uy;
-  uint32_t ctr = A.rngctr[env];
+  uint32_t ctr = R.rngctr;
   if (A.cmd_u) { ux = A.cmd_u[env * 4 + 2]; uy = A.cmd_u[env * 4 + 3]; }
   else {
     ux = (real)nm::rand_u24_bits(A.seed, (uint64_t)(A.env_offset + env), ctr) * real(1.0 / 16777216.0);
@@ -164,13 +165,13 @@
   }
   real c0 = ux * real(2) * M.max_lin_x - M.max_lin_x, c2 = uy * real(2) * M.max_ang - M.max_ang;
   real keep = sqrt(c0 * c0) > real(0.02) ? real(1) : real(0);
-  A.cmd[env * 3] = c0 * keep; A.cmd[env * 3 + 1] = real(0); A.cmd[env * 3 + 2] = c2;
-  A.rngctr[env] = ctr;
+  R.cmd[0] = c0 * keep; R.cmd[1] = real(0); R.cmd[2] = c2;
+  R.rngctr = ctr;
   A.eplen[env] = 0;
-  for (int k = 0; k < nm::kNLEG; k++) A.feetair[env * nm::kNLEG + k] = real(0);
+  for (int k = 0; k < nm::kNLEG; k++) R.feetair[k] = real(0);
   for (int k = 0; k < nm::kNREW; k++) {
-    atomicAdd(A.stat_sum + k, A.epsum[env * nm::kNREW + k]);
-    A.epsum[env * nm::kNREW + k] = real(0);
+    atomicAdd(A.stat_sum + k, R.epsum[k]);
+    R.epsum[k] = real(0);
   }
   atomicAdd(A.stat_cnt, 1);
 }
@@ -304,18 +305,16 @@
       A.nxcd = nx;
     }
     size_t n_ = (size_t)N;
-    if (dalloc(&A.qpos, n_ * 25) || dalloc(&A.qvel, n_ * 24) || dalloc(&A.qwarm, n_ * 24) || dalloc(&A.dofpos, n_ * 18) ||
-        dalloc(&A.dofvel, n_ * 18) || dalloc(&A.act, n_ * 18) || dalloc(&A.cmd, n_ * 3) || dalloc(&A.epsum, n_ * nm::kNREW) || dalloc(&A.feetair, n_ * nm::kNLEG) || dalloc(&A.feetflags, n_) ||
-        dalloc(&A.rngctr, n_) || dalloc(&A.hullcache, n_ * 8) || dalloc(&A.stat_sum, nm::kNREW) || dalloc(&A.stat_cnt, 4) || dalloc(&cmd_u_dev, n_ * 4) ||
+    if (dalloc(&A.st, n_) || dalloc(&A.stat_sum, nm::kNREW) || dalloc(&A.stat_cnt, 4) || dalloc(&cmd_u_dev, n_ * 4) ||
         dalloc(&timeout_now, n_) || dalloc(&ids_dev, n_) || dalloc(&counters_dev, 4) || dalloc(&A.wave_done, ((n_ + nm::kTicketGroup - 1) / nm::kTicketGroup + 2) * nm::kTicketStride) || dalloc(&A.nto, 1) || dalloc(&A.to_list, n_) || dalloc(&A.nprev, 1) || dalloc(&A.to_prev, n_) || dalloc(&A.to_owner, 1))
       return 1;
     if (dalloc(&M_dev, 1)) return 1;
     HIPCHK(hipMemcpy(M_dev, &M, sizeof M, hipMemcpyHostToDevice));
-    std::vector<real> q0(n_ * 25);
+    if (((uintptr_t)A.st & 127) != 0) return fail("nm_create: the state records are not 128-byte aligned");
+    hst.assign(n_, Rec{});
     for (size_t i = 0; i < n_; i++)
-      for (int k = 0; k < 25; k++) q0[i * 25 + k] = T.qpos0[k];
-    HIPCHK(hipMemcpy(A.qpos, q0.data(), q0.size() * sizeof(real), hipMemcpyHostToDevice));
-    return 0;
+      for (int k = 0; k < 25; k++) hst[i].qpos[k] = T.qpos0[k];
+    return push();
   }
   ~Env() override {
     (void)hipSetDevice(device);
@@ -398,56 +397,70 @@
     HIPCHK(hipMemcpy(dev, tmp.data(), n * sizeof(real), hipMemcpyHostToDevice));
     return 0;
   }
+  typedef nm::EnvRec<real> Rec;
+  std::vector<Rec> hst;
+  int pull() {
+    HIPCHK(hipSetDevice(device));
+    HIPCHK(hipDeviceSynchronize());
+    hst.resize((size_t)N);
+    HIPCHK(hipMemcpy(hst.data(), A.st, (size_t)N * sizeof(Rec), hipMemcpyDeviceToHost));
+    return 0;
+  }
+  int push() {
+    HIPCHK(hipMemcpy(A.st, hst.data(), (size_t)N * sizeof(Rec), hipMemcpyHostToDevice));
+    return 0;
+  }
+  template <int K> void fget(real (Rec::*f)[K], double* host) const {
+    if (!host) return;
+    for (size_t i = 0; i < (size_t)N; i++)
+      for (int k = 0; k < K; k++) host[i * K + k] = (double)(hst[i].*f)[k];
+  }
+  template <int K> void fset(real (Rec::*f)[K], const double* host) {
+    if (!host) return;
+    for (size_t i = 0; i < (size_t)N; i++)
+      for (int k = 0; k < K; k++) (hst[i].*f)[k] = (real)host[i * K + k];
+  }
   int get_state(double* qpos, double* qvel, double* qw) override {
-    HIPCHK(hipSetDevice(device));
-    HIPCHK(hipDeviceSynchronize());
-    return d2h(A.qpos, qpos, (size_t)N * 25) || d2h(A.qvel, qvel, (size_t)N * 24) || d2h(A.qwarm, qw, (size_t)N * 24);
+    if (pull()) return 1;
+    fget(&Rec::qpos, qpos); fget(&Rec::qvel, qvel); fget(&Rec::qwarm, qw);
+    return 0;
   }
   int set_state(const double* qpos, const double* qvel, const double* qw) override {
-    HIPCHK(hipSetDevice(device));
-    HIPCHK(hipDeviceSynchronize());
-    return h2d(A.qpos, qpos, (size_t)N * 25) || h2d(A.qvel, qvel, (size_t)N * 24) || h2d(A.qwarm, qw, (size_t)N * 24);
+    if (pull()) return 1;
+    fset(&Rec::qpos, qpos); fset(&Rec::qvel, qvel); fset(&Rec::qwarm, qw);
+    return push();
   }
   int get_buffers(double* dp, double* dv, double* act, double* cmd, double* es) override {
-    HIPCHK(hipSetDevice(device));
-    HIPCHK(hipDeviceSynchronize());
-    return d2h(A.dofpos, dp, (size_t)N * 18) || d2h(A.dofvel, dv, (size_t)N * 18) || d2h(A.act, act, (size_t)N * 18) ||
-           d2h(A.cmd, cmd, (size_t)N * 3) || d2h(A.epsum, es, (size_t)N * nm::kNREW);
+    if (pull()) return 1;
+    fget(&Rec::dofpos, dp); fget(&Rec::dofvel, dv); fget(&Rec::act, act); fget(&Rec::cmd, cmd); fget(&Rec::epsum, es);
+    return 0;
   }
   int set_buffers(const double* dp, const double* dv, const double* act, const double* cmd, const double* es) override {
-    HIPCHK(hipSetDevice(device));
-    HIPCHK(hipDeviceSynchronize());
-    return h2d(A.dofpos, dp, (size_t)N * 18) || h2d(A.dofvel, dv, (size_t)N * 18) || h2d(A.act, act, (size_t)N * 18) ||
-           h2d(A.cmd, cmd, (size_t)N * 3) || h2d(A.epsum, es, (size_t)N * nm::kNREW);
+    if (pull()) return 1;
+    fset(&Rec::dofpos, dp); fset(&Rec::dofvel, dv); fset(&Rec::act, act); fset(&Rec::cmd, cmd); fset(&Rec::epsum, es);
+    return push();
   }
   int get_feet(double* air, unsigned char* last, unsigned char* filt) override {
-    HIPCHK(hipSetDevice(device));
-    HIPCHK(hipDeviceSynchronize());
-    if (d2h(A.feetair, air, (size_t)N * 6)) return 1;
-    std::vector<int> fl(N);
-    HIPCHK(hipMemcpy(fl.data(), A.feetflags, sizeof(int) * N, hipMemcpyDeviceToHost));
+    if (pull()) return 1;
+    fget(&Rec::feetair, air);
     for (int i = 0; i < N; i++)
       for (int k = 0; k < 6; k++) {
-        if (last) last[i * 6 + k] = (fl[i] >> k) & 1;
-        if (filt) filt[i * 6 + k] = (fl[i] >> (6 + k)) & 1;
+        const int fl = hst[i].feetflags;
+        if (last) last[i * 6 + k] = (fl >> k) & 1;
+        if (filt) filt[i * 6 + k] = (fl >> (6 + k)) & 1;
       }
     return 0;
   }
   int set_feet(const double* air, const unsigned char* last, const unsigned char* filt) override {
-    HIPCHK(hipSetDevice(device));
-    HIPCHK(hipDeviceSynchronize());
-    if (h2d(A.feetair, air, (size_t)N * 6)) return 1;
-    if (last || filt) {
-      std::vector<int> fl(N);
-      HIPCHK(hipMemcpy(fl.data(), A.feetflags, sizeof(int) * N, hipMemcpyDeviceToHost));
-      for (int i = 0; i < N; i++)
-        for (int k = 0; k < 6; k++) {
-          if (last) fl[i] = (fl[i] & ~(1 << k)) | ((last[i * 6 + k] ? 1 : 0) << k);
-          if (filt) fl[i] = (fl[i] & ~(1 << (6 + k))) | ((filt[i * 6 + k] ? 1 : 0) << (6 + k));
-        }
-      HIPCHK(hipMemcpy(A.feetflags, fl.data(), sizeof(int) * N, hipMemcpyHostToDevice));
-    }
-    return 0;
+    if (pull()) return 1;
+    fset(&Rec::feetair, air);
+    for (int i = 0; i < N; i++)
+      for (int k = 0; k < 6; k++) {
+        int& fl = hst[i].feetflags;
+        if (last) fl = (fl & ~(1 << k)) | ((last[i * 6 + k] ? 1 : 0) << k);
+        if (filt) fl = (fl & ~(1 << (6 + k))) | ((filt[i * 6 + k] ? 1 : 0) << (6 + k));
+      }
+    return push();
   }
   int set_cmd_u(const double* u) override {
     HIPCHK(hipSetDevice(device));
@@ -460,10 +473,9 @@
     HIPCHK(hipDeviceSynchronize());
     long long c[3];
     HIPCHK(hipMemcpy(c, counters_dev, sizeof c, hipMemcpyDeviceToHost));
-    std::vector<int> hc((size_t)N * 8);
-    HIPCHK(hipMemcpy(hc.data(), A.hullcache, hc.size() * sizeof(int), hipMemcpyDeviceToHost));
+    if (pull()) return 1;
     long long fb = 0;
-    for (int i = 0; i < N; i++) fb += hc[(size_t)i * 8 + 7];
+    for (int i = 0; i < N; i++) fb += hst[i].hullcache[7];
     out[0] = c[0]; out[1] = c[1]; out[2] = fb;
     return 0;
   }
diff --git a/nightmare_rl_amd/csrc/simt.h b/nightmare_rl_amd/csrc/simt.h
--- a/nightmare_rl_amd/csrc/simt.h
+++ b/nightmare_rl_amd/csrc/simt.h
@@ -190,6 +190,12 @@
 NM_FN void gld4(const double* p, int i, double* o) { const nm_d4 t = *(const NM_GLOBAL(nm_d4)*)((const NM_GLOBAL(double)*)p + i); o[0] = t.x; o[1] = t.y; o[2] = t.z; o[3] = t.w; }
 NM_FN int to_int(float x) { return (int)x; }
 NM_FN int to_int(double x) { return (int)x; }
+typedef unsigned int nm_u4_ __attribute__((ext_vector_type(4)));
+typedef nm_u4_ W16 __attribute__((may_alias));
+NM_FN W16 gld16(const void* p, int off) { return *(const NM_GLOBAL(W16)*)((const NM_GLOBAL(char)*)p + off); }
+NM_FN void gst16(void* p, int off, W16 v, bool m) { if (m) *(NM_GLOBAL(W16)*)((NM_GLOBAL(char)*)p + off) = v; }
+NM_FN W16 lds16(const void* a, int off) { return *(const W16*)((const char*)a + off); }
+NM_FN void sts16(void* a, int off, W16 v) { *(W16*)((char*)a + off) = v; }
 NM_FN void wave_sync() {
   __builtin_amdgcn_fence(__ATOMIC_RELEASE, "wavefront");
   __builtin_amdgcn_wave_barrier();
@@ -334,6 +340,11 @@
 template <class T> NM_FN V<int> to_int(const V<T>& a) { V<int> r; for (int i = 0; i < NM_WAVE; i++) r.v[i] = (int)a.v[i]; return r; }
 template <class T> NM_FN void gld3(const T* p, const V<int>& i, V<T>* o) { for (int k = 0; k < NM_WAVE; k++) for (int c = 0; c < 3; c++) o[c].v[k] = p[i.v[k] + c]; }
 template <class T> NM_FN void gld3(const T* p, int i, T* o) { o[0] = p[i]; o[1] = p[i + 1]; o[2] = p[i + 2]; }
+struct W16 { uint32_t w[NM_WAVE][4]; };
+NM_FN W16 gld16(const void* p, const V<int>& off) { W16 r; for (int k = 0; k < NM_WAVE; k++) std::memcpy(r.w[k], (const char*)p + off.v[k], 16); return r; }
+NM_FN void gst16(void* p, const V<int>& off, const W16& v, const VB& m) { for (int k = 0; k < NM_WAVE; k++) if (m.v[k]) std::memcpy((char*)p + off.v[k], v.w[k], 16); }
+NM_FN W16 lds16(const void* a, const V<int>& off) { return gld16(a, off); }
+NM_FN void sts16(void* a, const V<int>& off, const W16& v) { for (int k = 0; k < NM_WAVE; k++) std::memcpy((char*)a + off.v[k], v.w[k], 16); }
 NM_FN void wave_sync() {}
 NM_FN void sched_fence() {}
 }
```

Result: slower. 27.74 million env-steps/s (-67.0%).
